# george-gca/sr-pytorch-lightning

Measured on AMD Instinct MI355X. Metric: SR training throughput, LR patches/s (48x48 LR x4, fwd+bwd+Adam), higher is better.
Workload: dtype bf16; 1 GPU; edsr_baseline x4, 48x48 LR patches, batch 256/GPU, train step (L1 + Adam); global_batch=256, parallelism=dp1, hip_graph=full

## Files before the change

### include/srk.h

```cpp
#ifndef SRK_H
#define SRK_H

#include <stdint.h>

#ifdef __cplusplus
extern "C" {
#endif

typedef void* srk_stream_t;

enum { SRK_BF16 = 0, SRK_F16 = 1, SRK_F32 = 2 };

enum {
  SRK_E_BADARG = -1,
  SRK_E_NODEV = -2
};

enum {
  SRK_OUT_NHWC = 0,
  SRK_OUT_NHWC_PS = 1,
  SRK_OUT_PLANAR = 2
};

typedef struct {
  const float* w;
  const float* bias;
  void* wpk;
  float* bias_pk;
  int Cout, Cin, KH, KW;
  int KinP;
  int CoutP;
  int dgrad;
  int ps_r;
  int dtype;
  int rows_layout;
} srk_pack_args;
int srk_pack_conv_weights(const srk_pack_args* a, srk_stream_t stream);
int srk_pack_conv_weights_group(const srk_pack_args* table, int n, srk_stream_t stream);
int srk_pack_group_tiles(const srk_pack_args* host_table, int n, int* tile_begin);
int srk_pack_conv_weights_group_tiled(const srk_pack_args* table, const int* tile_begin, int n, int total_tiles, srk_stream_t stream);

typedef struct {
  const void* x; int x_pitch, x_coff;
  int x_ps;
  int N, H, W;
  int Cin;
  const void* wpk; const float* bias;
  int CoutP;
  int Cout;
  int KH, KW;
  int relu; float scale;
  const void* res; int res_pitch, res_coff;
  const void* mask; int mask_pitch, mask_coff; int mask_from;
  void* out; int out_pitch, out_coff; int out_mode; int ps_r;
  const float* post_add;
  int dtype;
  int cout_real;
  void* relu_bits; const void* mask_bits;
} srk_conv_args;
int srk_conv_bits_ok(const srk_conv_args* a);
int srk_conv2d(const srk_conv_args* a, srk_stream_t stream);
int srk_conv_tile(int Cout);

int srk_conv_trunk_ok(const srk_conv_args* layers_host, int nlayers);
int srk_conv_trunk(const srk_conv_args* layers_host, const void* table_dev, int nlayers, srk_stream_t stream);

typedef struct {
  const void* x; int x_pitch, x_coff;
  int N, H, W;
  const void* w1; const float* b1;
  const void* w2; const float* b2;
  int relu_mid; float scale_mid;
  const void* mask; int mask_pitch, mask_coff;
  void* mid; int mid_pitch, mid_coff;
  float scale_out;
  const void* res; int res_pitch, res_coff; int res_from_x;
  void* out; int out_pitch, out_coff;
  int dtype;
  float* pool; const void* pool_aux; int pool_aux_pitch, pool_aux_coff;
  int ca_mode; int ca_cr;
  const float* ca_gsum; int ca_gsum_rows; const float* ca_sums; int ca_sums_rows;
  const float* ca_s; const float* ca_z; const float* ca_w1; const float* ca_w2;
  float* ca_slots;
  void* xo; int xo_pitch, xo_coff;
  const void* ca_x2; int ca_x2_pitch, ca_x2_coff;
  const float* ca_b1; const float* ca_b2; float* ca_s_out; float* ca_z_out;
} srk_conv_pair_args;
int srk_conv_pair(const srk_conv_pair_args* a, srk_stream_t stream);
int srk_conv_pair_tiles(int N, int H, int W);

typedef struct {
  const float* w1; const float* b1;
  const float* w2; const float* b2;
  int Cin, Chid, Cmid, CoutP;
  void* fwd; void* bwd;
  int dtype;
} srk_pw_pack_args;
int srk_pw_shape_ok(int Cin, int Chid, int CoutP);
long long srk_pw_pack_bytes(int Cin, int Chid, int CoutP, int bwd);
int srk_pw_pack(const srk_pw_pack_args* a, srk_stream_t stream);

typedef struct {
  const float* v; const float* g;
  float* w; float* inv;
  const float* dw;
  float* dv; float* dg;
  int rows, cols, row0, pad_;
} srk_wn_job;
int srk_weight_norm_group(const srk_wn_job* table_dev, int njobs, int total_rows, int backward, srk_stream_t stream);

int srk_pw_pack_group(const srk_pw_pack_args* table_dev, int n, srk_stream_t stream);

typedef struct {
  const void* x; int x_pitch, x_coff;
  long long P;
  int Cin, Chid, CoutP;
  int Cout;
  const void* wpk;
  void* out; int out_pitch, out_coff;
  int dtype;
} srk_pw_args;
int srk_pw_forward(const srk_pw_args* a, srk_stream_t stream);

typedef struct {
  const void* x; int x_pitch, x_coff;
  const void* gz; int gz_pitch, gz_coff; int Cz;
  long long P;
  int Cin, Chid, CoutP;
  const void* wpk;
  const void* res; int res_pitch, res_coff;
  void* gx; int gx_pitch, gx_coff;
  void* h_out; void* gh_out;
  int dtype;
} srk_pw_bwd_args;
int srk_pw_backward(const srk_pw_bwd_args* a, srk_stream_t stream);

typedef struct {
  const void* x; int x_pitch, x_coff;
  const void* gz; int gz_pitch, gz_coff; int Cz;
  long long P;
  int Cin, Chid, Cmid, CoutP;
  const void* wpk;
  float* dw1p; float* dw2p; float* db1p; float* db2p; int nranges;
  float* dw1; float* db1; float* dw2; float* db2;
  int dtype;
} srk_pw_wgrad_args;
int srk_pw_wgrad_ranges(long long P, int Chid);
int srk_pw_wgrad(const srk_pw_wgrad_args* a, srk_stream_t stream);

typedef struct {
  const void* x; int x_pitch, x_coff; int x_ps;
  const void* dy; int dy_pitch, dy_coff; int dy_ps;
  int N, H, W;
  int Cin, Cout;
  int KH, KW;
  float* dwp;
  float* dbp;
  int nslabs;
  int dtype;
  int cout_real;
} srk_wgrad_args;
int srk_conv2d_wgrad(const srk_wgrad_args* a, srk_stream_t stream);
int srk_wgrad_slabs(const srk_wgrad_args* a);
int srk_wgrad_slab_cout(const srk_wgrad_args* a);

typedef struct {
  const float* dwp; const float* dbp;
  int nslabs;
  float* dw; float* db;
  int Cout, Cin, KH, KW;
  int CinP, CoutP;
  int ps_r;
  float scale;
  int accumulate;
} srk_wgrad_fin_args;
int srk_wgrad_finalize(const srk_wgrad_fin_args* a, srk_stream_t stream);

int srk_wgrad_group_ok(const srk_wgrad_args* a);
int srk_wgrad_group_job_bytes(void);
int srk_wgrad_group_plan(srk_wgrad_args* jobs, int n, float* scratch, void* table_host, int* block_job_host,
                         int* nblocks, long long* scratch_floats);
int srk_conv2d_wgrad_group(const void* table_dev, const int* block_job_dev, int nblocks, int dtype, srk_stream_t stream);
int srk_wgrad_finalize_group(const srk_wgrad_fin_args* table_dev, int n, int blocks_per_job, srk_stream_t stream);
int srk_upload_small(void* dst_dev, const void* src_host, long long nbytes, srk_stream_t stream);
int srk_upload_prepare(void);
int srk_upload_eager(void* dst_dev, const void* src_host, long long nbytes);
int srk_upload_fence(void);

typedef struct {
  const float* x;
  const float* sub;
  void* dst; int dst_pitch, dst_coff;
  int N, Cin, H, W, KH, KW;
  int Kstore;
  int dtype;
} srk_unfold_args;
int srk_unfold_nchw(const srk_unfold_args* a, srk_stream_t stream);

typedef struct {
  const float* src; void* dst; int dst_pitch, dst_coff;
  int N, C, H, W;
  int Cstore; int ps_r; float scale; int dtype;
} srk_to_nhwc_args;
int srk_nchw_to_nhwc(const srk_to_nhwc_args* a, srk_stream_t stream);

typedef struct {
  const void* src; int src_pitch, src_coff; float* dst;
  int N, C, H, W; int dtype;
} srk_to_nchw_args;
int srk_nhwc_to_nchw(const srk_to_nchw_args* a, srk_stream_t stream);

int srk_ca_splits(int N, int HW);
typedef struct {
  const void* t; int t_pitch, t_coff;
  const void* u; int u_pitch, u_coff;
  float* sums;
  int N, HW, C; int dtype;
} srk_ca_pool_args;
int srk_ca_pool(const srk_ca_pool_args* a, srk_stream_t stream);

typedef struct {
  const void* t; int t_pitch, t_coff;
  const void* res; int res_pitch, res_coff;
  const float* sums;
  const float* w1; const float* b1; const float* w2; const float* b2;
  float* s_out; float* z_out;
  void* out; int out_pitch, out_coff;
  int N, HW, C, Cr; int dtype;
  int sums_rows;
} srk_ca_apply_args;
int srk_ca_apply(const srk_ca_apply_args* a, srk_stream_t stream);

typedef struct {
  const void* g; int g_pitch, g_coff;
  const float* gsum;
  const float* sums; const float* s; const float* z;
  const float* w1; const float* w2;
  float* dw1; float* db1; float* dw2; float* db2;
  void* gt; int gt_pitch, gt_coff;
  int N, HW, C, Cr; int dtype;
  int sums_rows, gsum_rows;
} srk_ca_bwd_args;
int srk_ca_bwd_apply(const srk_ca_bwd_args* a, srk_stream_t stream);
typedef struct { const float* src; float* dst; int n; int k; } srk_rowsum_job;
int srk_rowsum_group(const srk_rowsum_job* table_dev, int njobs, int max_k, srk_stream_t stream);

typedef struct {
  const uint8_t* lr; const uint8_t* hr;
  int lr_h, lr_w, hr_h, hr_w;
  int top, left;
  int rot;
  int hflip, vflip;
} srk_patch_desc;
typedef struct {
  const srk_patch_desc* table; int N; int C; int patch_lr; int scale;
  float* lr_out;
  float* hr_out;
} srk_patch_args;
int srk_sample_patches(const srk_patch_args* a, srk_stream_t stream);

typedef struct {
  const float* sr; const float* hr;
  int N, C, H, W;
  int luma;
  int shave;
  double* sse;
} srk_sse_args;
int srk_image_sse(const srk_sse_args* a, srk_stream_t stream);

typedef struct srk_l1_args {
  const float* sr;
  const float* hr;
  long long n;
  signed char* sign;
  double* partial;
  const float* gout;
  float scale;
  float* grad;
} srk_l1_args;
int srk_l1_blocks(long long n);
int srk_l1_loss_fwd(const srk_l1_args* a, srk_stream_t stream);
int srk_l1_loss_bwd(const srk_l1_args* a, srk_stream_t stream);
int srk_l1_loss_mean(const double* partial, int nb, long long n, float* out, srk_stream_t stream);

#define SRK_FLIP_TABLE_FLOATS 176
#define SRK_FLIP_ADJ_CHANNELS 7
typedef struct srk_flip_args {
  const float* sr;
  const float* hr;
  int N, H, W;
  const float* table;
  double* partial;
  float* err;
  float* adj;
  const float* gout;
  float scale;
  float* grad;
} srk_flip_args;
int srk_flip_blocks(int N, int H, int W);
int srk_flip_fwd(const srk_flip_args* a, srk_stream_t stream);
int srk_flip_bwd(const srk_flip_args* a, srk_stream_t stream);
int srk_flip_mean(const double* partial, int nb, long long n, float* out, srk_stream_t stream);

typedef struct srk_ssim_args {
  const float* x;
  const float* y;
  int N, C, H, W;
  int pool;
  float sigma, k1, k2;
  double* sums;
} srk_ssim_args;
int srk_image_ssim(const srk_ssim_args* a, srk_stream_t stream);

typedef struct srk_ms_ssim_args {
  const float* x;
  const float* y;
  float* workspace;
  double* partials;
  float* out;
  int N, C, H, W;
  float sigma, k1, k2;
  float w0, w1, w2, w3, w4;
} srk_ms_ssim_args;
long long srk_ms_ssim_workspace_bytes(int N, int C, int H, int W);
int srk_ms_ssim_tiles(int H, int W, int* first);
int srk_ms_ssim(const srk_ms_ssim_args* a, srk_stream_t stream);

typedef struct {
  const void* x; int x_pitch, x_coff;
  void* cols; int cols_pitch;
  int N, H, W, C;
  int K, stride, pad;
  int Ho, Wo;
  int dtype;
} srk_unfold_nhwc_args;
int srk_unfold_nhwc(const srk_unfold_nhwc_args* a, srk_stream_t stream);

typedef struct {
  const void* cols; int cols_pitch;
  const float* bias;
  void* out; int out_pitch, out_coff;
  int N, Hi, Wi, C;
  int K, stride, pad;
  int Ho, Wo;
  int dtype;
} srk_fold_nhwc_args;
int srk_fold_nhwc(const srk_fold_nhwc_args* a, srk_stream_t stream);

typedef struct {
  const void* x; int x_pitch;
  void* out; int out_pitch;
  const void* wpk;
  const float* bias;
  int N, H, W;
  int dtype;
  const float* slope; int slope_stride;
  void* pre; int pre_pitch;
} srk_proj_args;
long long srk_proj_pack_bytes(void);
int srk_proj_pack(const float* w4, void* wpk, int dtype, srk_stream_t stream);
typedef struct { const float* w4; void* wpk; } srk_proj_pack_job;
int srk_proj_pack_group(const srk_proj_pack_job* table_dev, int n, int dtype, srk_stream_t stream);
int srk_proj_down(const srk_proj_args* a, srk_stream_t stream);
int srk_proj_up(const srk_proj_args* a, srk_stream_t stream);
typedef struct {
  const void* xh; int xh_pitch;
  const void* g; int g_pitch;
  float* scratch;
  float* dw;
  int accumulate;
  int N, H, W;
  int dtype;
  float* db;
  int bias_side;
  int db_accumulate;
} srk_proj_wgrad_args;
long long srk_proj_wgrad_scratch_floats(int N, int H, int W);
int srk_proj_wgrad(const srk_proj_wgrad_args* a, srk_stream_t stream);

typedef struct {
  const void* x; int x_pitch, x_coff;
  const void* y; int y_pitch, y_coff;
  long long P; int C;
  int mode;
  float* partial;
  int dtype;
  const float* shift;
  float* shift_out;
  void* gate_out; int gate_pitch;
  const float* slope; int slope_stride;
  const float* gate_a; const float* gate_d;
  float* partial2;
} srk_chan_stats_args;
int srk_chan_stats_blocks(long long P);
int srk_chan_stats(const srk_chan_stats_args* a, srk_stream_t stream);
typedef struct {
  const float* partial; int nblocks; int C; int Creal;
  int mode; int total;
  float M, eps, momentum;
  const float* mean; const float* invstd; const float* gamma;
  const float* weight; const float* bias;
  float* running_mean; float* running_var;
  float* out;
  long long* nbt;
  float* dgamma_acc; float* dbeta_acc;
  const float* partial2; int total2;
  float* dslope_acc;
} srk_chan_finalize_args;
int srk_chan_finalize(const srk_chan_finalize_args* a, srk_stream_t stream);
int srk_chan_stats_finalize(const srk_chan_stats_args* a, const srk_chan_finalize_args* f, int* counter, srk_stream_t stream);

typedef struct {
  const void* x; int x_pitch, x_coff;
  const void* y; int y_pitch, y_coff;
  const void* z; int z_pitch, z_coff;
  const float* a; const float* b; const float* d;
  const float* slope; int slope_stride;
  int post_prelu;
  void* out; int out_pitch, out_coff;
  long long P; int C;
  int dtype;
  const float* gate_a; const float* gate_d;
} srk_chan_apply_args;
int srk_chan_apply(const srk_chan_apply_args* a, srk_stream_t stream);

typedef struct {
  const float* wt; const float* bt;
  const float* wu; const float* bu;
  int O, C, Ci;
  float* weff; float* beff;
  float* wedge; float* bedge; float* wcor; float* bcor;
  const void* x; int x_pitch;
  int N, H, W; int dtype;
  float* out;
  const float* g;
  void* dx; int dx_pitch;
  float* eedge; float* e0; float* ecor; float* k0;
  float* scratch;
  const float* r; const float* r0;
  float* dwt; float* dbt; float* dwu; float* dbu;
} srk_hrtail_args;
int srk_hrtail_collapse(const srk_hrtail_args* a, srk_stream_t stream);
int srk_hrtail_edge_fwd(const srk_hrtail_args* a, srk_stream_t stream);
int srk_hrtail_edge_bwd_x(const srk_hrtail_args* a, srk_stream_t stream);
long long srk_hrtail_scratch_floats(int N, int Ci);
int srk_hrtail_edge_bwd_w(const srk_hrtail_args* a, srk_stream_t stream);
int srk_hrtail_expand(const srk_hrtail_args* a, srk_stream_t stream);

typedef struct { float* p; const float* g; long long state_off; long long n; long long step_idx; } srk_adam_slot;
typedef struct { int slot; int count; long long start; } srk_adam_block;
typedef struct {
  const srk_adam_slot* slots; const srk_adam_block* blocks; int nslots, nblocks;
  float* m; float* v;
  float* steps; unsigned int* ticket;
  float lr, beta1, beta2, eps, weight_decay; int maximize;
  float one_minus_beta1, one_minus_beta2;
} srk_adam_args;
int srk_adam_step(const srk_adam_args* a, srk_stream_t stream);
int srk_adam_step_scaled(const srk_adam_args* a, float* scaler_state, srk_stream_t stream);
int srk_adam_check_scaled(const srk_adam_args* a, float* scaler_state, srk_stream_t stream);
int srk_adam_update_scaled(const srk_adam_args* a, const float* scaler_state, srk_stream_t stream);
int srk_loss_scale_update(float* scaler_state, srk_stream_t stream);

const char* srk_last_error(void);
int srk_version(void);
int srk_device_cus(void);

#ifdef __cplusplus
}
#endif
#endif
```

### sr-pytorch-lightning_amd/_lib.py

```python
import ctypes as C
import os

_HERE = os.path.dirname(os.path.abspath(__file__))
EXACT_RELU = os.environ.get("SRK_EXACT_RELU") == "1"
LIB_PATH = os.environ.get("SRK_LIB_PATH") or os.path.join(_HERE, "libsrk_gfx950_exact.so" if EXACT_RELU else "libsrk_gfx950.so")

SRK_BF16, SRK_F16, SRK_F32 = 0, 1, 2
OUT_NHWC, OUT_NHWC_PS, OUT_PLANAR = 0, 1, 2

_p, _i, _f = C.c_void_p, C.c_int, C.c_float


class PackArgs(C.Structure):
    _fields_ = [("w", _p), ("bias", _p), ("wpk", _p), ("bias_pk", _p),
                ("Cout", _i), ("Cin", _i), ("KH", _i), ("KW", _i),
                ("KinP", _i), ("CoutP", _i), ("dgrad", _i), ("ps_r", _i), ("dtype", _i), ("rows_layout", _i)]


class ConvArgs(C.Structure):
    _fields_ = [("x", _p), ("x_pitch", _i), ("x_coff", _i), ("x_ps", _i),
                ("N", _i), ("H", _i), ("W", _i), ("Cin", _i),
                ("wpk", _p), ("bias", _p), ("CoutP", _i), ("Cout", _i), ("KH", _i), ("KW", _i),
                ("relu", _i), ("scale", _f),
                ("res", _p), ("res_pitch", _i), ("res_coff", _i),
                ("mask", _p), ("mask_pitch", _i), ("mask_coff", _i), ("mask_from", _i),
                ("out", _p), ("out_pitch", _i), ("out_coff", _i), ("out_mode", _i), ("ps_r", _i),
                ("post_add", _p), ("dtype", _i), ("cout_real", _i), ("relu_bits", _p), ("mask_bits", _p)]


class ConvPairArgs(C.Structure):
    _fields_ = [("x", _p), ("x_pitch", _i), ("x_coff", _i), ("N", _i), ("H", _i), ("W", _i),
                ("w1", _p), ("b1", _p), ("w2", _p), ("b2", _p),
                ("relu_mid", _i), ("scale_mid", _f),
                ("mask", _p), ("mask_pitch", _i), ("mask_coff", _i),
                ("mid", _p), ("mid_pitch", _i), ("mid_coff", _i),
                ("scale_out", _f),
                ("res", _p), ("res_pitch", _i), ("res_coff", _i), ("res_from_x", _i),
                ("out", _p), ("out_pitch", _i), ("out_coff", _i), ("dtype", _i),
                ("pool", _p), ("pool_aux", _p), ("pool_aux_pitch", _i), ("pool_aux_coff", _i),
                ("ca_mode", _i), ("ca_cr", _i), ("ca_gsum", _p), ("ca_gsum_rows", _i), ("ca_sums", _p), ("ca_sums_rows", _i),
                ("ca_s", _p), ("ca_z", _p), ("ca_w1", _p), ("ca_w2", _p), ("ca_slots", _p),
                ("xo", _p), ("xo_pitch", _i), ("xo_coff", _i),
                ("ca_x2", _p), ("ca_x2_pitch", _i), ("ca_x2_coff", _i), ("ca_b1", _p), ("ca_b2", _p), ("ca_s_out", _p), ("ca_z_out", _p)]


class PwPackArgs(C.Structure):
    _fields_ = [("w1", _p), ("b1", _p), ("w2", _p), ("b2", _p), ("Cin", _i), ("Chid", _i), ("Cmid", _i), ("CoutP", _i),
                ("fwd", _p), ("bwd", _p), ("dtype", _i)]


class WnJob(C.Structure):
    _fields_ = [("v", _p), ("g", _p), ("w", _p), ("inv", _p), ("dw", _p), ("dv", _p), ("dg", _p),
                ("rows", _i), ("cols", _i), ("row0", _i), ("pad_", _i)]


class PwArgs(C.Structure):
    _fields_ = [("x", _p), ("x_pitch", _i), ("x_coff", _i), ("P", C.c_longlong), ("Cin", _i), ("Chid", _i), ("CoutP", _i), ("Cout", _i),
                ("wpk", _p), ("out", _p), ("out_pitch", _i), ("out_coff", _i), ("dtype", _i)]


class PwBwdArgs(C.Structure):
    _fields_ = [("x", _p), ("x_pitch", _i), ("x_coff", _i), ("gz", _p), ("gz_pitch", _i), ("gz_coff", _i), ("Cz", _i),
                ("P", C.c_longlong), ("Cin", _i), ("Chid", _i), ("CoutP", _i), ("wpk", _p),
                ("res", _p), ("res_pitch", _i), ("res_coff", _i), ("gx", _p), ("gx_pitch", _i), ("gx_coff", _i),
                ("h_out", _p), ("gh_out", _p), ("dtype", _i)]


class PwWgradArgs(C.Structure):
    _fields_ = [("x", _p), ("x_pitch", _i), ("x_coff", _i), ("gz", _p), ("gz_pitch", _i), ("gz_coff", _i), ("Cz", _i),
                ("P", C.c_longlong), ("Cin", _i), ("Chid", _i), ("Cmid", _i), ("CoutP", _i), ("wpk", _p),
                ("dw1p", _p), ("dw2p", _p), ("db1p", _p), ("db2p", _p), ("nranges", _i), ("dw1", _p), ("db1", _p), ("dw2", _p), ("db2", _p),
                ("dtype", _i)]


class ChanFinalizeArgs(C.Structure):
    _fields_ = [("partial", _p), ("nblocks", _i), ("C", _i), ("Creal", _i), ("mode", _i), ("total", _i),
                ("M", _f), ("eps", _f), ("momentum", _f), ("mean", _p), ("invstd", _p), ("gamma", _p),
                ("weight", _p), ("bias", _p), ("running_mean", _p), ("running_var", _p), ("out", _p),
                ("nbt", _p), ("dgamma_acc", _p), ("dbeta_acc", _p), ("partial2", _p), ("total2", _i), ("dslope_acc", _p)]


class RowsumJob(C.Structure):
    _fields_ = [("src", _p), ("dst", _p), ("n", _i), ("k", _i)]


class AdamSlot(C.Structure):
    _fields_ = [("p", _p), ("g", _p), ("state_off", C.c_longlong), ("n", C.c_longlong), ("step_idx", C.c_longlong)]


class AdamBlock(C.Structure):
    _fields_ = [("slot", _i), ("count", _i), ("start", C.c_longlong)]


class AdamArgs(C.Structure):
    _fields_ = [("slots", _p), ("blocks", _p), ("nslots", _i), ("nblocks", _i), ("m", _p), ("v", _p), ("steps", _p), ("ticket", _p),
                ("lr", _f), ("beta1", _f), ("beta2", _f), ("eps", _f), ("weight_decay", _f), ("maximize", _i),
                ("one_minus_beta1", _f), ("one_minus_beta2", _f)]


class WgradArgs(C.Structure):
    _fields_ = [("x", _p), ("x_pitch", _i), ("x_coff", _i), ("x_ps", _i),
                ("dy", _p), ("dy_pitch", _i), ("dy_coff", _i), ("dy_ps", _i),
                ("N", _i), ("H", _i), ("W", _i), ("Cin", _i), ("Cout", _i), ("KH", _i), ("KW", _i),
                ("dwp", _p), ("dbp", _p), ("nslabs", _i), ("dtype", _i), ("cout_real", _i)]


class WgradFinArgs(C.Structure):
    _fields_ = [("dwp", _p), ("dbp", _p), ("nslabs", _i), ("dw", _p), ("db", _p),
                ("Cout", _i), ("Cin", _i), ("KH", _i), ("KW", _i), ("CinP", _i), ("CoutP", _i),
                ("ps_r", _i), ("scale", _f), ("accumulate", _i)]


class ProjArgs(C.Structure):
    _fields_ = [("x", _p), ("x_pitch", _i), ("out", _p), ("out_pitch", _i), ("wpk", _p), ("bias", _p),
                ("N", _i), ("H", _i), ("W", _i), ("dtype", _i), ("slope", _p), ("slope_stride", _i), ("pre", _p), ("pre_pitch", _i)]


class ProjPackJob(C.Structure):
    _fields_ = [("w4", _p), ("wpk", _p)]


class ProjWgradArgs(C.Structure):
    _fields_ = [("xh", _p), ("xh_pitch", _i), ("g", _p), ("g_pitch", _i), ("scratch", _p), ("dw", _p), ("accumulate", _i),
                ("N", _i), ("H", _i), ("W", _i), ("dtype", _i), ("db", _p), ("bias_side", _i), ("db_accumulate", _i)]


class UnfoldArgs(C.Structure):
    _fields_ = [("x", _p), ("sub", _p), ("dst", _p), ("dst_pitch", _i), ("dst_coff", _i),
                ("N", _i), ("Cin", _i), ("H", _i), ("W", _i), ("KH", _i), ("KW", _i), ("Kstore", _i), ("dtype", _i)]


class ToNhwcArgs(C.Structure):
    _fields_ = [("src", _p), ("dst", _p), ("dst_pitch", _i), ("dst_coff", _i),
                ("N", _i), ("C", _i), ("H", _i), ("W", _i), ("Cstore", _i), ("ps_r", _i), ("scale", _f), ("dtype", _i)]


class ToNchwArgs(C.Structure):
    _fields_ = [("src", _p), ("src_pitch", _i), ("src_coff", _i), ("dst", _p),
                ("N", _i), ("C", _i), ("H", _i), ("W", _i), ("dtype", _i)]


class CaPoolArgs(C.Structure):
    _fields_ = [("t", _p), ("t_pitch", _i), ("t_coff", _i), ("u", _p), ("u_pitch", _i), ("u_coff", _i),
                ("sums", _p), ("N", _i), ("HW", _i), ("C", _i), ("dtype", _i)]


class CaApplyArgs(C.Structure):
    _fields_ = [("t", _p), ("t_pitch", _i), ("t_coff", _i), ("res", _p), ("res_pitch", _i), ("res_coff", _i),
                ("sums", _p), ("w1", _p), ("b1", _p), ("w2", _p), ("b2", _p), ("s_out", _p), ("z_out", _p),
                ("out", _p), ("out_pitch", _i), ("out_coff", _i),
                ("N", _i), ("HW", _i), ("C", _i), ("Cr", _i), ("dtype", _i), ("sums_rows", _i)]


class CaBwdArgs(C.Structure):
    _fields_ = [("g", _p), ("g_pitch", _i), ("g_coff", _i), ("gsum", _p), ("sums", _p), ("s", _p), ("z", _p),
                ("w1", _p), ("w2", _p), ("dw1", _p), ("db1", _p), ("dw2", _p), ("db2", _p),
                ("gt", _p), ("gt_pitch", _i), ("gt_coff", _i),
                ("N", _i), ("HW", _i), ("C", _i), ("Cr", _i), ("dtype", _i), ("sums_rows", _i), ("gsum_rows", _i)]


class PatchDesc(C.Structure):
    _fields_ = [("lr", _p), ("hr", _p), ("lr_h", _i), ("lr_w", _i), ("hr_h", _i), ("hr_w", _i),
                ("top", _i), ("left", _i), ("rot", _i), ("hflip", _i), ("vflip", _i)]


class PatchArgs(C.Structure):
    _fields_ = [("table", _p), ("N", _i), ("C", _i), ("patch_lr", _i), ("scale", _i), ("lr_out", _p), ("hr_out", _p)]


class SseArgs(C.Structure):
    _fields_ = [("sr", _p), ("hr", _p), ("N", _i), ("C", _i), ("H", _i), ("W", _i), ("luma", _i), ("shave", _i), ("sse", _p)]


class SsimArgs(C.Structure):
    _fields_ = [("x", _p), ("y", _p), ("N", _i), ("C", _i), ("H", _i), ("W", _i), ("pool", _i),
                ("sigma", _f), ("k1", _f), ("k2", _f), ("sums", _p)]


class MsSsimArgs(C.Structure):
    _fields_ = [("x", _p), ("y", _p), ("workspace", _p), ("partials", _p), ("out", _p), ("N", _i), ("C", _i), ("H", _i), ("W", _i),
                ("sigma", _f), ("k1", _f), ("k2", _f), ("w0", _f), ("w1", _f), ("w2", _f), ("w3", _f), ("w4", _f)]


class L1Args(C.Structure):
    _fields_ = [("sr", _p), ("hr", _p), ("n", C.c_longlong), ("sign", _p), ("partial", _p), ("gout", _p),
                ("scale", _f), ("grad", _p)]


class FlipArgs(C.Structure):
    _fields_ = [("sr", _p), ("hr", _p), ("N", _i), ("H", _i), ("W", _i), ("table", _p), ("partial", _p), ("err", _p), ("adj", _p),
                ("gout", _p), ("scale", _f), ("grad", _p)]


class UnfoldNhwcArgs(C.Structure):
    _fields_ = [("x", _p), ("x_pitch", _i), ("x_coff", _i), ("cols", _p), ("cols_pitch", _i),
                ("N", _i), ("H", _i), ("W", _i), ("C", _i), ("K", _i), ("stride", _i), ("pad", _i), ("Ho", _i), ("Wo", _i), ("dtype", _i)]


class FoldNhwcArgs(C.Structure):
    _fields_ = [("cols", _p), ("cols_pitch", _i), ("bias", _p), ("out", _p), ("out_pitch", _i), ("out_coff", _i),
                ("N", _i), ("Hi", _i), ("Wi", _i), ("C", _i), ("K", _i), ("stride", _i), ("pad", _i), ("Ho", _i), ("Wo", _i), ("dtype", _i)]


class ChanStatsArgs(C.Structure):
    _fields_ = [("x", _p), ("x_pitch", _i), ("x_coff", _i), ("y", _p), ("y_pitch", _i), ("y_coff", _i),
                ("P", C.c_longlong), ("C", _i), ("mode", _i), ("partial", _p), ("dtype", _i), ("shift", _p), ("shift_out", _p),
                ("gate_out", _p), ("gate_pitch", _i), ("slope", _p), ("slope_stride", _i),
                ("gate_a", _p), ("gate_d", _p), ("partial2", _p)]


class ChanApplyArgs(C.Structure):
    _fields_ = [("x", _p), ("x_pitch", _i), ("x_coff", _i), ("y", _p), ("y_pitch", _i), ("y_coff", _i),
                ("z", _p), ("z_pitch", _i), ("z_coff", _i), ("a", _p), ("b", _p), ("d", _p),
                ("slope", _p), ("slope_stride", _i), ("post_prelu", _i), ("out", _p), ("out_pitch", _i), ("out_coff", _i),
                ("P", C.c_longlong), ("C", _i), ("dtype", _i), ("gate_a", _p), ("gate_d", _p)]


class HrTailArgs(C.Structure):
    _fields_ = [("wt", _p), ("bt", _p), ("wu", _p), ("bu", _p), ("O", _i), ("C", _i), ("Ci", _i),
                ("weff", _p), ("beff", _p), ("wedge", _p), ("bedge", _p), ("wcor", _p), ("bcor", _p),
                ("x", _p), ("x_pitch", _i), ("N", _i), ("H", _i), ("W", _i), ("dtype", _i),
                ("out", _p), ("g", _p), ("dx", _p), ("dx_pitch", _i),
                ("eedge", _p), ("e0", _p), ("ecor", _p), ("k0", _p), ("scratch", _p),
                ("r", _p), ("r0", _p), ("dwt", _p), ("dbt", _p), ("dwu", _p), ("dbu", _p)]


LAUNCHERS = {
    "srk_pack_conv_weights": PackArgs,
    "srk_conv2d": ConvArgs,
    "srk_conv_pair": ConvPairArgs,
    "srk_pw_pack": PwPackArgs,
    "srk_pw_forward": PwArgs,
    "srk_pw_backward": PwBwdArgs,
    "srk_pw_wgrad": PwWgradArgs,
    "srk_adam_step": AdamArgs,
    "srk_chan_finalize": ChanFinalizeArgs,
    "srk_conv2d_wgrad": WgradArgs,
    "srk_wgrad_finalize": WgradFinArgs,
    "srk_unfold_nchw": UnfoldArgs,
    "srk_nchw_to_nhwc": ToNhwcArgs,
    "srk_nhwc_to_nchw": ToNchwArgs,
    "srk_ca_pool": CaPoolArgs,
    "srk_ca_apply": CaApplyArgs,
    "srk_ca_bwd_apply": CaBwdArgs,
    "srk_sample_patches": PatchArgs,
    "srk_image_sse": SseArgs,
    "srk_image_ssim": SsimArgs,
    "srk_ms_ssim": MsSsimArgs,
    "srk_l1_loss_fwd": L1Args,
    "srk_l1_loss_bwd": L1Args,
    "srk_flip_fwd": FlipArgs,
    "srk_flip_bwd": FlipArgs,
    "srk_unfold_nhwc": UnfoldNhwcArgs,
    "srk_fold_nhwc": FoldNhwcArgs,
    "srk_chan_stats": ChanStatsArgs,
    "srk_chan_apply": ChanApplyArgs,
    "srk_proj_down": ProjArgs,
    "srk_proj_up": ProjArgs,
    "srk_proj_wgrad": ProjWgradArgs,
    "srk_hrtail_collapse": HrTailArgs,
    "srk_hrtail_edge_fwd": HrTailArgs,
    "srk_hrtail_edge_bwd_x": HrTailArgs,
    "srk_hrtail_edge_bwd_w": HrTailArgs,
    "srk_hrtail_expand": HrTailArgs,
}
OTHER_SYMBOLS = ("srk_conv_tile", "srk_last_error", "srk_version", "srk_device_cus", "srk_wgrad_slabs",
                 "srk_pack_conv_weights_group", "srk_l1_blocks", "srk_wgrad_group_ok", "srk_wgrad_group_job_bytes",
                 "srk_wgrad_group_plan", "srk_conv2d_wgrad_group", "srk_wgrad_finalize_group", "srk_upload_small", "srk_upload_prepare", "srk_upload_eager", "srk_upload_fence", "srk_ca_splits", "srk_chan_stats_blocks",
                 "srk_conv_pair_tiles", "srk_rowsum_group", "srk_pw_shape_ok", "srk_pw_pack_bytes", "srk_pw_pack_group", "srk_weight_norm_group", "srk_pw_wgrad_ranges", "srk_l1_loss_mean", "srk_chan_stats_finalize", "srk_pack_group_tiles", "srk_pack_conv_weights_group_tiled",
                 "srk_proj_pack", "srk_proj_pack_bytes", "srk_proj_wgrad_scratch_floats", "srk_proj_pack_group", "srk_wgrad_slab_cout",
                 "srk_hrtail_scratch_floats", "srk_adam_step_scaled", "srk_adam_check_scaled", "srk_adam_update_scaled", "srk_loss_scale_update", "srk_conv_bits_ok",
                 "srk_conv_trunk", "srk_conv_trunk_ok", "srk_flip_blocks", "srk_flip_mean",
                 "srk_ms_ssim_workspace_bytes", "srk_ms_ssim_tiles")

_lib = None


def load():
    global _lib
    if _lib is not None:
        return _lib
    if not os.path.exists(LIB_PATH):
        raise RuntimeError(
            f"{LIB_PATH} is missing: build it with `python __graft_entry__.py` "
            "(hipcc --offload-arch=gfx950).  There is no CPU fallback for the HIP path.")
    lib = C.CDLL(LIB_PATH)
    older = bool(os.environ.get("SRK_LIB_PATH"))

    class _Absent:
        def __init__(self, name):
            self.name = name
            self.argtypes = self.restype = None

        def __call__(self, *a, **k):
            raise RuntimeError(f"{self.name} is not exported by {LIB_PATH} (an older build loaded through SRK_LIB_PATH)")

    if older:
        for name in list(LAUNCHERS) + list(OTHER_SYMBOLS):
            if not hasattr(lib, name):
                setattr(lib, name, _Absent(name))
    for name, st in LAUNCHERS.items():
        fn = getattr(lib, name)
        fn.argtypes = [C.POINTER(st), C.c_void_p]
        fn.restype = C.c_int
    lib.srk_conv_tile.argtypes = [C.c_int]
    lib.srk_conv_tile.restype = C.c_int
    lib.srk_conv_pair_tiles.argtypes = [C.c_int, C.c_int, C.c_int]
    lib.srk_conv_pair_tiles.restype = C.c_int
    lib.srk_wgrad_slabs.argtypes = [C.POINTER(WgradArgs)]
    lib.srk_wgrad_slabs.restype = C.c_int
    lib.srk_wgrad_slab_cout.argtypes = [C.POINTER(WgradArgs)]
    lib.srk_wgrad_slab_cout.restype = C.c_int
    lib.srk_pack_conv_weights_group.argtypes = [C.c_void_p, C.c_int, C.c_void_p]
    lib.srk_pack_conv_weights_group.restype = C.c_int
    lib.srk_pack_group_tiles.argtypes = [C.c_void_p, C.c_int, C.c_void_p]
    lib.srk_pack_group_tiles.restype = C.c_int
    lib.srk_pack_conv_weights_group_tiled.argtypes = [C.c_void_p, C.c_void_p, C.c_int, C.c_int, C.c_void_p]
    lib.srk_pack_conv_weights_group_tiled.restype = C.c_int
    lib.srk_wgrad_group_ok.argtypes = [C.POINTER(WgradArgs)]
    lib.srk_wgrad_group_ok.restype = C.c_int
    lib.srk_wgrad_group_job_bytes.restype = C.c_int
    lib.srk_wgrad_group_plan.argtypes = [C.POINTER(WgradArgs), C.c_int, C.c_void_p, C.c_void_p, C.c_void_p,
                                         C.POINTER(C.c_int), C.POINTER(C.c_longlong)]
    lib.srk_wgrad_group_plan.restype = C.c_int
    lib.srk_conv2d_wgrad_group.argtypes = [C.c_void_p, C.c_void_p, C.c_int, C.c_int, C.c_void_p]
    lib.srk_conv2d_wgrad_group.restype = C.c_int
    lib.srk_wgrad_finalize_group.argtypes = [C.c_void_p, C.c_int, C.c_int, C.c_void_p]
    lib.srk_wgrad_finalize_group.restype = C.c_int
    lib.srk_rowsum_group.argtypes = [C.c_void_p, C.c_int, C.c_int, C.c_void_p]
    lib.srk_rowsum_group.restype = C.c_int
    lib.srk_upload_small.argtypes = [C.c_void_p, C.c_void_p, C.c_longlong, C.c_void_p]
    lib.srk_upload_small.restype = C.c_int
    if not isinstance(getattr(lib, "srk_upload_eager", None), _Absent):
        lib.srk_upload_prepare.argtypes = []
        lib.srk_upload_prepare.restype = C.c_int
        lib.srk_upload_eager.argtypes = [C.c_void_p, C.c_void_p, C.c_longlong]
        lib.srk_upload_eager.restype = C.c_int
        lib.srk_upload_fence.argtypes = []
        lib.srk_upload_fence.restype = C.c_int
    lib.srk_chan_stats_finalize.argtypes = [C.POINTER(ChanStatsArgs), C.POINTER(ChanFinalizeArgs), C.c_void_p, C.c_void_p]
    lib.srk_chan_stats_finalize.restype = C.c_int
    lib.srk_chan_stats_blocks.argtypes = [C.c_longlong]
    lib.srk_chan_stats_blocks.restype = C.c_int
    lib.srk_ca_splits.argtypes = [C.c_int, C.c_int]
    lib.srk_ca_splits.restype = C.c_int
    lib.srk_l1_loss_mean.argtypes = [C.c_void_p, C.c_int, C.c_longlong, C.c_void_p, C.c_void_p]
    lib.srk_l1_loss_mean.restype = C.c_int
    lib.srk_l1_blocks.argtypes = [C.c_longlong]
    if not isinstance(getattr(lib, "srk_flip_mean", None), _Absent):
        lib.srk_flip_mean.argtypes = [C.c_void_p, C.c_int, C.c_longlong, C.c_void_p, C.c_void_p]
        lib.srk_flip_mean.restype = C.c_int
        lib.srk_flip_blocks.argtypes = [C.c_int, C.c_int, C.c_int]
        lib.srk_flip_blocks.restype = C.c_int
    lib.srk_l1_blocks.restype = C.c_int
    if not isinstance(getattr(lib, "srk_ms_ssim_tiles", None), _Absent):
        lib.srk_ms_ssim_workspace_bytes.argtypes = [C.c_int, C.c_int, C.c_int, C.c_int]
        lib.srk_ms_ssim_workspace_bytes.restype = C.c_longlong
        lib.srk_ms_ssim_tiles.argtypes = [C.c_int, C.c_int, C.c_void_p]
        lib.srk_ms_ssim_tiles.restype = C.c_int
    lib.srk_pw_shape_ok.argtypes = [C.c_int, C.c_int, C.c_int]
    lib.srk_pw_shape_ok.restype = C.c_int
    lib.srk_pw_pack_bytes.argtypes = [C.c_int, C.c_int, C.c_int, C.c_int]
    lib.srk_pw_pack_bytes.restype = C.c_longlong
    lib.srk_pw_wgrad_ranges.argtypes = [C.c_longlong, C.c_int]
    lib.srk_pw_wgrad_ranges.restype = C.c_int
    lib.srk_pw_pack_group.argtypes = [C.c_void_p, C.c_int, C.c_void_p]
    lib.srk_pw_pack_group.restype = C.c_int
    lib.srk_weight_norm_group.argtypes = [C.c_void_p, C.c_int, C.c_int, C.c_int, C.c_void_p]
    lib.srk_weight_norm_group.restype = C.c_int
    lib.srk_proj_pack.argtypes = [C.c_void_p, C.c_void_p, C.c_int, C.c_void_p]
    lib.srk_proj_pack.restype = C.c_int
    lib.srk_proj_pack_group.argtypes = [C.c_void_p, C.c_int, C.c_int, C.c_void_p]
    lib.srk_proj_pack_group.restype = C.c_int
    lib.srk_proj_pack_bytes.restype = C.c_longlong
    lib.srk_proj_wgrad_scratch_floats.argtypes = [C.c_int, C.c_int, C.c_int]
    lib.srk_proj_wgrad_scratch_floats.restype = C.c_longlong
    lib.srk_hrtail_scratch_floats.argtypes = [C.c_int, C.c_int]
    lib.srk_hrtail_scratch_floats.restype = C.c_longlong
    lib.srk_conv_bits_ok.argtypes = [C.POINTER(ConvArgs)]
    lib.srk_conv_bits_ok.restype = C.c_int
    lib.srk_conv_trunk_ok.argtypes = [C.POINTER(ConvArgs), C.c_int]
    lib.srk_conv_trunk_ok.restype = C.c_int
    lib.srk_conv_trunk.argtypes = [C.POINTER(ConvArgs), C.c_void_p, C.c_int, C.c_void_p]
    lib.srk_conv_trunk.restype = C.c_int
    lib.srk_adam_step_scaled.argtypes = [C.POINTER(AdamArgs), C.c_void_p, C.c_void_p]
    lib.srk_adam_step_scaled.restype = C.c_int
    for fn in (lib.srk_adam_check_scaled, lib.srk_adam_update_scaled):
        fn.argtypes = [C.POINTER(AdamArgs), C.c_void_p, C.c_void_p]
        fn.restype = C.c_int
    lib.srk_loss_scale_update.argtypes = [C.c_void_p, C.c_void_p]
    lib.srk_loss_scale_update.restype = C.c_int
    lib.srk_last_error.restype = C.c_char_p
    lib.srk_version.restype = C.c_int
    lib.srk_device_cus.restype = C.c_int
    _lib = lib
    return lib


def call(name, args, stream):
    lib = load()
    if getattr(args, "N", 1) == 0:
        return
    rc = getattr(lib, name)(C.byref(args), C.c_void_p(stream))
    if rc != 0:
        raise RuntimeError(f"{name} failed (rc={rc}): {lib.srk_last_error().decode(errors='replace')}")


def check(rc, what):
    if rc != 0:
        raise RuntimeError(f"{what} failed (rc={rc}): {load().srk_last_error().decode(errors='replace')}")


def conv_tile(cout):
    return load().srk_conv_tile(int(cout))
```

### sr-pytorch-lightning_amd/csrc/hr_tail.hip

```cpp
#include "srk_common.h"

namespace {

SRK_DEV void sub_of(int a, int d, int& i, int& s) {
  const int ap = a + d;
  i = ap & 1;
  s = (ap - i) >> 1;
}

struct Wts {
  const float* wt; const float* bt; const float* wu; const float* bu;
  int O, C, Ci;
};

SRK_DEV float sum16(float v) {
  v += __shfl_xor(v, 8, 64);
  v += __shfl_xor(v, 4, 64);
  v += __shfl_xor(v, 2, 64);
  v += __shfl_xor(v, 1, 64);
  return v;
}

SRK_DEV float collapse_w(const Wts& p, int sub, int o, int a, int b, int ci, int dy0, int dy1, int dx0, int dx1, int fy, int fx) {
  float acc = 0.f;
  for (int dy = dy0; dy <= dy1; ++dy) {
    int i, sy; sub_of(a, dy, i, sy);
    const int ey = fy - sy;
    if (ey < -1 || ey > 1) continue;
    for (int dx = dx0; dx <= dx1; ++dx) {
      int j, sx; sub_of(b, dx, j, sx);
      const int ex = fx - sx;
      if (ex < -1 || ex > 1) continue;
      const float* wt = p.wt + (size_t)o * p.C * 9 + (dy + 1) * 3 + (dx + 1);
      const float* wu = p.wu + ((size_t)(i * 2 + j) * p.Ci + ci) * 9 + (ey + 1) * 3 + (ex + 1);
      for (int c0 = sub; c0 < p.C; c0 += 64) {
        float x[4], y[4];
#pragma unroll
        for (int k = 0; k < 4; ++k) {
          const int c = c0 + 16 * k;
          const bool ok = c < p.C;
          x[k] = ok ? wt[(size_t)c * 9] : 0.f;
          y[k] = ok ? wu[(size_t)c * 4 * p.Ci * 9] : 0.f;
        }
#pragma unroll
        for (int k = 0; k < 4; ++k)
          if (c0 + 16 * k < p.C) acc += x[k] * y[k];
      }
    }
  }
  return sum16(acc);
}
SRK_DEV float collapse_b(const Wts& p, int sub, int o, int a, int b, int dy0, int dy1, int dx0, int dx1) {
  float acc = 0.f;
  if (p.bu) {
    for (int dy = dy0; dy <= dy1; ++dy) {
      int i, sy; sub_of(a, dy, i, sy);
      for (int dx = dx0; dx <= dx1; ++dx) {
        int j, sx; sub_of(b, dx, j, sx);
        const float* wt = p.wt + (size_t)o * p.C * 9 + (dy + 1) * 3 + (dx + 1);
        for (int c = sub; c < p.C; c += 16) acc += wt[(size_t)c * 9] * p.bu[c * 4 + i * 2 + j];
      }
    }
  }
  return sum16(acc);
}

__global__ __launch_bounds__(256) void hrtail_collapse_kernel(const srk_hrtail_args a) {
  const Wts p{a.wt, a.bt, a.wu, a.bu, a.O, a.C, a.Ci};
  const int O = a.O, Ci = a.Ci;
  const int n_eff = 4 * O * Ci * 25, n_edge = 4 * 2 * O * Ci * 5, n_cor = 4 * O * Ci;
  const int n_b = 4 * O + 4 * 2 * O + 4 * O;
  const int sub = threadIdx.x & 15;
  int t = blockIdx.x * 16 + (threadIdx.x >> 4);
  if (t >= n_eff + n_edge + n_cor + n_b) t = n_eff + n_edge + n_cor + n_b;
  float v = 0.f;
  float* dst = nullptr;
  if (t < n_eff) {
    const int f = t % 25, ci = (t / 25) % Ci, k = t / (25 * Ci);
    v = collapse_w(p, sub, k >> 2, (k >> 1) & 1, k & 1, ci, -1, 1, -1, 1, f / 5 - 2, f % 5 - 2);
    dst = a.weff + t;
  } else if (t < n_eff + n_edge) {
    const int u = t - n_eff;
    const int tt = u % 5, ci = (u / 5) % Ci, kk = (u / (5 * Ci)) % (2 * O), ty = u / (5 * Ci * 2 * O);
    const int o = kk >> 1, q = kk & 1;
    if (ty == 0) v = collapse_w(p, sub, o, 0, q, ci, -1, -1, -1, 1, 0, tt - 2);
    else if (ty == 1) v = collapse_w(p, sub, o, 1, q, ci, 1, 1, -1, 1, 0, tt - 2);
    else if (ty == 2) v = collapse_w(p, sub, o, q, 0, ci, -1, 1, -1, -1, tt - 2, 0);
    else v = collapse_w(p, sub, o, q, 1, ci, -1, 1, 1, 1, tt - 2, 0);
    dst = a.wedge + u;
  } else if (t < n_eff + n_edge + n_cor) {
    const int u = t - n_eff - n_edge;
    const int ci = u % Ci, o = (u / Ci) % O, c = u / (Ci * O);
    const int ca = c >> 1, cb = c & 1;
    v = collapse_w(p, sub, o, ca, cb, ci, ca ? 1 : -1, ca ? 1 : -1, cb ? 1 : -1, cb ? 1 : -1, 0, 0);
    dst = a.wcor + u;
  } else if (t < n_eff + n_edge + n_cor + n_b) {
    const int w = t - n_eff - n_edge - n_cor;
    if (w < 4 * O) {
      const int k = w;
      v = (a.bt ? a.bt[k >> 2] : 0.f) + collapse_b(p, sub, k >> 2, (k >> 1) & 1, k & 1, -1, 1, -1, 1);
      dst = a.beff + k;
    } else if (w < 4 * O + 8 * O) {
      const int u = w - 4 * O, kk = u % (2 * O), ty = u / (2 * O), o = kk >> 1, q = kk & 1;
      if (ty == 0) v = collapse_b(p, sub, o, 0, q, -1, -1, -1, 1);
      else if (ty == 1) v = collapse_b(p, sub, o, 1, q, 1, 1, -1, 1);
      else if (ty == 2) v = collapse_b(p, sub, o, q, 0, -1, 1, -1, -1);
      else v = collapse_b(p, sub, o, q, 1, -1, 1, 1, 1);
      dst = a.bedge + u;
    } else {
      const int u = w - 12 * O, o = u % O, c = u / O, ca = c >> 1, cb = c & 1;
      v = collapse_b(p, sub, o, ca, cb, ca ? 1 : -1, ca ? 1 : -1, cb ? 1 : -1, cb ? 1 : -1);
      dst = a.bcor + u;
    }
  }
  if (dst && sub == 0) *dst = v;
}

template <int DT> SRK_DEV float ld_act(const void* base, size_t idx) {
  return DTraits<DT>::to_f32(reinterpret_cast<const typename DTraits<DT>::elem*>(base)[idx]);
}

constexpr int MAXO = 4;
SRK_DEV float wave_total(float v) {
#pragma unroll
  for (int m = 32; m >= 1; m >>= 1) v += __shfl_xor(v, m, 64);
  return v;
}
struct EdgeGeo {
  int ty, len; bool row;
  int fix_lr, fix_hr;
};
SRK_DEV EdgeGeo edge_geo(int ty, int H, int W) {
  EdgeGeo e;
  e.ty = ty; e.row = ty < 2; e.len = e.row ? W : H;
  e.fix_lr = ty == 0 ? 0 : ty == 1 ? H - 1 : ty == 2 ? 0 : W - 1;
  e.fix_hr = ty == 0 ? 0 : ty == 1 ? 2 * H - 1 : ty == 2 ? 0 : 2 * W - 1;
  return e;
}
SRK_DEV void stage_copy256(float* __restrict__ dst, const float* __restrict__ src, int n) {
  int i = threadIdx.x;
  for (; i + 256 * 7 < n; i += 256 * 8) {
    float v[8];
#pragma unroll
    for (int k = 0; k < 8; ++k) v[k] = src[i + 256 * k];
#pragma unroll
    for (int k = 0; k < 8; ++k) dst[i + 256 * k] = v[k];
  }
  float v[8];
#pragma unroll
  for (int k = 0; k < 8; ++k) v[k] = i + 256 * k < n ? src[i + 256 * k] : 0.f;
#pragma unroll
  for (int k = 0; k < 8; ++k)
    if (i + 256 * k < n) dst[i + 256 * k] = v[k];
}
template <int DT>
SRK_DEV void stage_line(const srk_hrtail_args& a, const EdgeGeo& e, int n, float* Xl, int pitch) {
  typedef DTraits<DT> Tr;
  const int Ci = a.Ci;
  if ((Ci & 7) == 0 && (a.x_pitch & 7) == 0) {
    const int nch = Ci >> 3, total = (e.len + 4) * nch;
    for (int i0 = threadIdx.x; i0 < total; i0 += 256 * 4) {
      i32x4 raw[4];
#pragma unroll
      for (int u = 0; u < 4; ++u) {
        const int i = i0 + 256 * u;
        const int sp = i / nch, c8 = i - sp * nch, s = sp - 2;
        raw[u] = i32x4{0, 0, 0, 0};
        if (i < total && s >= 0 && s < e.len) {
          const int yy = e.row ? e.fix_lr : s, xx = e.row ? s : e.fix_lr;
          raw[u] = gload16(reinterpret_cast<const typename Tr::elem*>(a.x) + ((size_t)(n * a.H + yy) * a.W + xx) * a.x_pitch + c8 * 8);
        }
      }
#pragma unroll
      for (int u = 0; u < 4; ++u) {
        const int i = i0 + 256 * u;
        if (i >= total) continue;
        const int sp = i / nch, c8 = i - sp * nch;
        const int w4[4] = {raw[u].x, raw[u].y, raw[u].z, raw[u].w};
        float v[8];
#pragma unroll
        for (int k = 0; k < 4; ++k) unpack2<DT>((uint32_t)w4[k], v[2 * k], v[2 * k + 1]);
#pragma unroll
        for (int k = 0; k < 8; ++k) Xl[sp * pitch + c8 * 8 + k] = v[k];
      }
    }
    return;
  }
  for (int i = threadIdx.x; i < (e.len + 4) * Ci; i += 256) {
    const int s = i / Ci - 2, ci = i % Ci;
    float v = 0.f;
    if (s >= 0 && s < e.len) {
      const int yy = e.row ? e.fix_lr : s, xx = e.row ? s : e.fix_lr;
      v = ld_act<DT>(a.x, ((size_t)(n * a.H + yy) * a.W + xx) * a.x_pitch + ci);
    }
    Xl[(s + 2) * pitch + ci] = v;
  }
}

template <int DT>
__global__ __launch_bounds__(256) void hrtail_edge_fwd_kernel(const srk_hrtail_args a, int phase) {
  const int H = a.H, W = a.W, O = a.O, Ci = a.Ci, H2 = 2 * H, W2 = 2 * W;
  const int n = blockIdx.x;
  const EdgeGeo e = edge_geo(2 * phase + blockIdx.y, H, W);
  extern __shared__ __attribute__((aligned(16))) char smem_raw[];
  const int pitch = Ci + 1;
  float* const Xl = reinterpret_cast<float*>(smem_raw);
  float* const Wl = Xl + (size_t)(e.len + 4) * pitch;
  stage_line<DT>(a, e, n, Xl, pitch);
  stage_copy256(Wl, a.wedge + (size_t)e.ty * 2 * O * Ci * 5, 2 * O * Ci * 5);
  __syncthreads();
  const size_t oplane = (size_t)H2 * W2;
  float* const out = a.out + (size_t)n * O * oplane;
  for (int idx = threadIdx.x + 256 * blockIdx.z; idx < 2 * e.len * O; idx += 256 * gridDim.z) {
    const int p = idx % (2 * e.len), o = idx / (2 * e.len);
    const int s = p >> 1, q = p & 1;
    const float* const w = Wl + (size_t)(o * 2 + q) * Ci * 5;
    const float* const x = Xl + (size_t)s * pitch;
    float a0 = a.bedge[e.ty * 2 * O + o * 2 + q], a1 = 0.f, a2 = 0.f, a3 = 0.f, a4 = 0.f;
    for (int ci = 0; ci < Ci; ++ci) {
      a0 += w[ci * 5 + 0] * x[0 * pitch + ci]; a1 += w[ci * 5 + 1] * x[1 * pitch + ci]; a2 += w[ci * 5 + 2] * x[2 * pitch + ci];
      a3 += w[ci * 5 + 3] * x[3 * pitch + ci]; a4 += w[ci * 5 + 4] * x[4 * pitch + ci];
    }
    float acc = ((a0 + a1) + (a2 + a3)) + a4;
    if (!e.row && (p == 0 || p == 2 * e.len - 1)) {
      const int ca = p == 0 ? 0 : 1, cb = e.ty == 2 ? 0 : 1, c = ca * 2 + cb;
      float cc = a.bcor[c * O + o];
      const float* const xc = Xl + (size_t)(s + 2) * pitch;
      for (int ci = 0; ci < Ci; ++ci) cc += a.wcor[((size_t)c * O + o) * Ci + ci] * xc[ci];
      acc -= cc;
    }
    const size_t at = e.row ? (size_t)e.fix_hr * W2 + p : (size_t)p * W2 + e.fix_hr;
    out[(size_t)o * oplane + at] -= acc;
  }
}

template <int DT>
__global__ __launch_bounds__(256) void hrtail_edge_bwd_x_kernel(const srk_hrtail_args a, int phase) {
  typedef DTraits<DT> Tr;
  const int H = a.H, W = a.W, O = a.O, Ci = a.Ci, H2 = 2 * H, W2 = 2 * W;
  const int n = blockIdx.x;
  const bool shared_line = phase == 0 ? H == 1 : W == 1;
  if (shared_line && blockIdx.y == 1) return;
  extern __shared__ __attribute__((aligned(16))) char smem_raw[];
  const size_t gplane = (size_t)H2 * W2;
  const float* const g = a.g + (size_t)n * O * gplane;
  for (int rep = 0; rep < (shared_line ? 2 : 1); ++rep) {
  const EdgeGeo e = edge_geo(2 * phase + (shared_line ? rep : (int)blockIdx.y), H, W);
  float* const Gl = reinterpret_cast<float*>(smem_raw);
  float* const Wl = Gl + (size_t)2 * O * (e.len + 4);
  __syncthreads();
  for (int i0 = threadIdx.x; i0 < 2 * O * (e.len + 4); i0 += 256 * 4) {
    float v[4];
#pragma unroll
    for (int u = 0; u < 4; ++u) {
      const int i = i0 + 256 * u;
      const int kk = i / (e.len + 4), s = i % (e.len + 4) - 2, o = kk >> 1, q = kk & 1;
      v[u] = 0.f;
      if (i < 2 * O * (e.len + 4) && s >= 0 && s < e.len)
        v[u] = e.row ? g[(size_t)o * gplane + (size_t)e.fix_hr * W2 + 2 * s + q] : g[(size_t)o * gplane + (size_t)(2 * s + q) * W2 + e.fix_hr];
    }
#pragma unroll
    for (int u = 0; u < 4; ++u)
      if (i0 + 256 * u < 2 * O * (e.len + 4)) Gl[i0 + 256 * u] = v[u];
  }
  stage_copy256(Wl, a.wedge + (size_t)e.ty * 2 * O * Ci * 5, 2 * O * Ci * 5);
  __syncthreads();
  const int nch = (Ci + 7) >> 3;
  const bool vec = (Ci & 7) == 0 && (a.dx_pitch & 7) == 0;
  for (int idx = threadIdx.x + 256 * blockIdx.z; idx < e.len * nch; idx += 256 * gridDim.z) {
    const int c8 = idx % nch, s = idx / nch;
    float corr[8];
#pragma unroll
    for (int k = 0; k < 8; ++k) corr[k] = 0.f;
    for (int kk = 0; kk < 2 * O; ++kk) {
      const float* const gl = Gl + (size_t)kk * (e.len + 4) + s + 2;
      float gv[5];
#pragma unroll
      for (int tt = 0; tt < 5; ++tt) gv[tt] = gl[2 - tt];
#pragma unroll
      for (int k = 0; k < 8; ++k) {
        const int ci = c8 * 8 + k;
        if (ci < Ci) {
          const float* const w = Wl + ((size_t)kk * Ci + ci) * 5;
#pragma unroll
          for (int tt = 0; tt < 5; ++tt) corr[k] += w[tt] * gv[tt];
        }
      }
    }
    if (!e.row && (s == 0 || s == e.len - 1)) {
      for (int ca = 0; ca < 2; ++ca) {
        if (!(ca ? s == e.len - 1 : s == 0)) continue;
        const int cb = e.ty == 2 ? 0 : 1, c = ca * 2 + cb;
        const size_t at = (size_t)(ca ? H2 - 1 : 0) * W2 + e.fix_hr;
        for (int o = 0; o < O; ++o) {
          const float gc = g[(size_t)o * gplane + at];
#pragma unroll
          for (int k = 0; k < 8; ++k)
            if (c8 * 8 + k < Ci) corr[k] -= a.wcor[((size_t)c * O + o) * Ci + c8 * 8 + k] * gc;
        }
      }
    }
    const int yy = e.row ? e.fix_lr : s, xx = e.row ? s : e.fix_lr;
    typename Tr::elem* const d = reinterpret_cast<typename Tr::elem*>(a.dx) + ((size_t)(n * H + yy) * W + xx) * a.dx_pitch + c8 * 8;
    if (vec) {
      const i32x4 raw = *reinterpret_cast<const i32x4*>(d);
      const int w4[4] = {raw.x, raw.y, raw.z, raw.w};
      int o4[4];
#pragma unroll
      for (int k = 0; k < 4; ++k) {
        float f0, f1;
        unpack2<DT>((uint32_t)w4[k], f0, f1);
        o4[k] = (int)pack2<DT>(f0 - corr[2 * k], f1 - corr[2 * k + 1]);
      }
      *reinterpret_cast<i32x4*>(d) = i32x4{o4[0], o4[1], o4[2], o4[3]};
    } else {
#pragma unroll
      for (int k = 0; k < 8; ++k)
        if (c8 * 8 + k < Ci) d[k] = Tr::from_f32(Tr::to_f32(d[k]) - corr[k]);
    }
  }
  }
}

constexpr int EW_MAXLEN = 512;
template <int DT>
__global__ __launch_bounds__(256) void hrtail_edge_bwd_w_kernel(const srk_hrtail_args a, int nchunks, int ew_chunk) {
  const int H = a.H, W = a.W, O = a.O, Ci = a.Ci, H2 = 2 * H, W2 = 2 * W;
  const int ty = blockIdx.y, chunk = blockIdx.x;
  const int n0 = chunk * ew_chunk, n1 = min(a.N, n0 + ew_chunk);
  const int ncombo = ty < 4 ? 2 * O * 5 : O;
  const size_t gplane = (size_t)H2 * W2;
  float* const dst = a.scratch + ((size_t)ty * nchunks + chunk) * (size_t)(2 * MAXO * 5) * (Ci + 1);
  extern __shared__ __attribute__((aligned(16))) char smem_raw[];
  float* const Xl = reinterpret_cast<float*>(smem_raw);
  if (ty >= 4) {
    if (blockIdx.z != 0) return;
    const int c = ty - 4, ca = c >> 1, cbb = c & 1;
    const int Py = ca ? H2 - 1 : 0, Px = cbb ? W2 - 1 : 0, yy = ca ? H - 1 : 0, xx = cbb ? W - 1 : 0;
    for (int item = threadIdx.x; item < ncombo * (Ci + 1); item += 256) {
      const int ci = item % (Ci + 1), o = item / (Ci + 1);
      float acc = 0.f;
      for (int n = n0; n < n1; ++n) {
        const float gv = a.g[((size_t)n * O + o) * gplane + (size_t)Py * W2 + Px];
        const float xv = ci < Ci ? ld_act<DT>(a.x, ((size_t)(n * H + yy) * W + xx) * a.x_pitch + ci) : 1.f;
        acc += gv * xv;
      }
      dst[item] = acc;
    }
    return;
  }
  const bool rowedge = ty < 2;
  const int len = rowedge ? W : H;
  float* const Gl = Xl + (size_t)(len + 4) * Ci;
  constexpr int MAXIT = (2 * MAXO * 5 * 65 + 255) / 256;
  const int nitems = ncombo * (Ci + 1);
  const int ipb = (nitems + gridDim.z - 1) / gridDim.z, item0 = blockIdx.z * ipb, item1 = min(nitems, item0 + ipb);
  float acc[MAXIT];
#pragma unroll
  for (int k = 0; k < MAXIT; ++k) acc[k] = 0.f;
  for (int n = n0; n < n1; ++n) {
    __syncthreads();
    stage_line<DT>(a, edge_geo(ty, H, W), n, Xl, Ci);
    for (int i = threadIdx.x; i < 2 * O * len; i += 256) {
      const int kk = i / len, s = i % len, o = kk >> 1, q = kk & 1;
      const float* const g = a.g + ((size_t)n * O + o) * gplane;
      Gl[i] = rowedge ? g[(size_t)(ty == 0 ? 0 : H2 - 1) * W2 + 2 * s + q] : g[(size_t)(2 * s + q) * W2 + (ty == 2 ? 0 : W2 - 1)];
    }
    __syncthreads();
#pragma unroll
    for (int k = 0; k < MAXIT; ++k) {
      const int item = item0 + threadIdx.x + k * 256;
      if (item >= item1) break;
      const int ci = item % (Ci + 1), cb = item / (Ci + 1), tt = cb % 5, kk = cb / 5;
      const float* const gr = Gl + kk * len;
      float t0 = 0.f, t1 = 0.f, t2 = 0.f, t3 = 0.f;
      int p = 0;
      if (ci < Ci) {
        const float* const xr = Xl + (size_t)tt * Ci + ci;
        for (; p + 3 < len; p += 4) {
          t0 += gr[p] * xr[(size_t)p * Ci]; t1 += gr[p + 1] * xr[(size_t)(p + 1) * Ci];
          t2 += gr[p + 2] * xr[(size_t)(p + 2) * Ci]; t3 += gr[p + 3] * xr[(size_t)(p + 3) * Ci];
        }
        for (; p < len; ++p) t0 += gr[p] * xr[(size_t)p * Ci];
      } else if (tt == 2) {
        for (; p + 3 < len; p += 4) { t0 += gr[p]; t1 += gr[p + 1]; t2 += gr[p + 2]; t3 += gr[p + 3]; }
        for (; p < len; ++p) t0 += gr[p];
      }
      acc[k] += (t0 + t1) + (t2 + t3);
    }
  }
#pragma unroll
  for (int k = 0; k < MAXIT; ++k) {
    const int item = item0 + threadIdx.x + k * 256;
    if (item < item1) dst[item] = acc[k];
  }
}

__global__ __launch_bounds__(256) void hrtail_edge_reduce_kernel(const srk_hrtail_args a, int nchunks) {
  const int O = a.O, Ci = a.Ci;
  const int per = 2 * MAXO * 5 * (Ci + 1);
  const int t = blockIdx.x * 256 + threadIdx.x;
  const int n_edge = 4 * 2 * O * 5 * (Ci + 1), n_cor = 4 * O * (Ci + 1);
  if (t >= n_edge + n_cor) return;
  int ty, item;
  if (t < n_edge) { ty = t / (2 * O * 5 * (Ci + 1)); item = t % (2 * O * 5 * (Ci + 1)); }
  else { const int u = t - n_edge; ty = 4 + u / (O * (Ci + 1)); item = u % (O * (Ci + 1)); }
  const float* const src = a.scratch + (size_t)ty * nchunks * per + item;
  float s0 = 0.f, s1 = 0.f, s2 = 0.f, s3 = 0.f;
  int c = 0;
  for (; c + 3 < nchunks; c += 4) {
    s0 += src[(size_t)c * per]; s1 += src[(size_t)(c + 1) * per]; s2 += src[(size_t)(c + 2) * per]; s3 += src[(size_t)(c + 3) * per];
  }
  for (; c < nchunks; ++c) s0 += src[(size_t)c * per];
  const float s = (s0 + s1) + (s2 + s3);
  const int ci = item % (Ci + 1), cb = item / (Ci + 1);
  if (ty < 4) {
    const int tt = cb % 5, kk = cb / 5;
    if (ci < Ci) a.eedge[(((size_t)ty * 2 * O + kk) * Ci + ci) * 5 + tt] = s;
    else if (tt == 2) a.e0[ty * 2 * O + kk] = s;
  } else {
    if (ci < Ci) a.ecor[((size_t)(ty - 4) * O + cb) * Ci + ci] = s;
    else a.k0[(ty - 4) * O + cb] = s;
  }
}

struct Gr {
  const float* r; const float* r0; const float* ee; const float* e0; const float* ec; const float* k0;
  int O, Ci;
};
SRK_DEV int row_type(int a, int dy) { return (a == 0 && dy == -1) ? 0 : ((a == 1 && dy == 1) ? 1 : -1); }
SRK_DEV int col_type(int b, int dx) { return (b == 0 && dx == -1) ? 2 : ((b == 1 && dx == 1) ? 3 : -1); }
SRK_DEV float g_w(const Gr& q, int o, int a, int b, int dy, int dx, int ci, int fy, int fx) {
  float v = q.r[(((size_t)(o * 4 + a * 2 + b)) * q.Ci + ci) * 25 + (fy + 2) * 5 + (fx + 2)];
  const int rt = row_type(a, dy), ct = col_type(b, dx);
  if (rt >= 0 && fy == 0) v -= q.ee[(((size_t)rt * 2 * q.O + o * 2 + b) * q.Ci + ci) * 5 + fx + 2];
  if (ct >= 0 && fx == 0) v -= q.ee[(((size_t)ct * 2 * q.O + o * 2 + a) * q.Ci + ci) * 5 + fy + 2];
  if (rt >= 0 && ct >= 0 && fy == 0 && fx == 0) v += q.ec[((size_t)(a * 2 + b) * q.O + o) * q.Ci + ci];
  return v;
}
SRK_DEV float g_b(const Gr& q, int o, int a, int b, int dy, int dx) {
  float v = q.r0[o * 4 + a * 2 + b];
  const int rt = row_type(a, dy), ct = col_type(b, dx);
  if (rt >= 0) v -= q.e0[rt * 2 * q.O + o * 2 + b];
  if (ct >= 0) v -= q.e0[ct * 2 * q.O + o * 2 + a];
  if (rt >= 0 && ct >= 0) v += q.k0[(a * 2 + b) * q.O + o];
  return v;
}

__global__ __launch_bounds__(256) void hrtail_expand_kernel(const srk_hrtail_args a) {
  const Gr q{a.r, a.r0, a.eedge, a.e0, a.ecor, a.k0, a.O, a.Ci};
  const int O = a.O, C = a.C, Ci = a.Ci;
  const int n_wu = 4 * C * Ci * 9, n_bu = 4 * C, n_bt = O;
  const int nb_thread = (n_wu + n_bu + n_bt + 255) / 256;
  if ((int)blockIdx.x >= nb_thread) {
    const int t = ((int)blockIdx.x - nb_thread) * 4 + (threadIdx.x >> 6), lane = threadIdx.x & 63;
    if (t >= O * C * 9) return;
    const int d = t % 9, c = (t / 9) % C, o = t / (9 * C);
    const int dy = d / 3 - 1, dx = d % 3 - 1;
    float acc = 0.f;
    for (int pa = 0; pa < 2; ++pa) {
      int i, sy; sub_of(pa, dy, i, sy);
      for (int pb = 0; pb < 2; ++pb) {
        int j, sx; sub_of(pb, dx, j, sx);
        const int cu = c * 4 + i * 2 + j;
        if (a.bu && lane == 0) acc += g_b(q, o, pa, pb, dy, dx) * a.bu[cu];
        for (int ci = lane; ci < Ci; ci += 64)
#pragma unroll
          for (int e = 0; e < 9; ++e)
            acc += g_w(q, o, pa, pb, dy, dx, ci, sy + e / 3 - 1, sx + e % 3 - 1) * a.wu[((size_t)cu * Ci + ci) * 9 + e];
      }
    }
    acc = wave_total(acc);
    if (lane == 0) a.dwt[t] = acc;
    return;
  }
  int t = blockIdx.x * 256 + threadIdx.x;
  if (t < n_wu) {
    const int e = t % 9, ci = (t / 9) % Ci, cu = t / (9 * Ci), c = cu >> 2, i = (cu >> 1) & 1, j = cu & 1;
    const int ey = e / 3 - 1, ex = e % 3 - 1;
    float acc = 0.f;
    for (int pa = 0; pa < 2; ++pa)
      for (int dy = -1; dy <= 1; ++dy) {
        int ii, sy; sub_of(pa, dy, ii, sy);
        if (ii != i) continue;
        for (int pb = 0; pb < 2; ++pb)
          for (int dx = -1; dx <= 1; ++dx) {
            int jj, sx; sub_of(pb, dx, jj, sx);
            if (jj != j) continue;
            for (int o = 0; o < O; ++o)
              acc += a.wt[((size_t)o * C + c) * 9 + (dy + 1) * 3 + dx + 1] * g_w(q, o, pa, pb, dy, dx, ci, sy + ey, sx + ex);
          }
      }
    a.dwu[t] = acc;
    return;
  }
  t -= n_wu;
  if (t < n_bu) {
    if (!a.dbu) return;
    const int cu = t, c = cu >> 2, i = (cu >> 1) & 1, j = cu & 1;
    float acc = 0.f;
    for (int pa = 0; pa < 2; ++pa)
      for (int dy = -1; dy <= 1; ++dy) {
        int ii, sy; sub_of(pa, dy, ii, sy);
        if (ii != i) continue;
        for (int pb = 0; pb < 2; ++pb)
          for (int dx = -1; dx <= 1; ++dx) {
            int jj, sx; sub_of(pb, dx, jj, sx);
            if (jj != j) continue;
            for (int o = 0; o < O; ++o) acc += a.wt[((size_t)o * C + c) * 9 + (dy + 1) * 3 + dx + 1] * g_b(q, o, pa, pb, dy, dx);
          }
      }
    a.dbu[cu] = acc;
    return;
  }
  t -= n_bu;
  if (t < n_bt && a.dbt) a.dbt[t] = a.r0[t * 4] + a.r0[t * 4 + 1] + a.r0[t * 4 + 2] + a.r0[t * 4 + 3];
}

int check_common(const srk_hrtail_args* a, const char* who) {
  SRK_CHECK_ARG(a, "%s: null argument", who);
  SRK_CHECK_ARG(a->O >= 1 && a->O <= MAXO && a->C >= 1 && a->Ci >= 1, "%s: O=%d (1..%d) C=%d Ci=%d", who, a->O, MAXO, a->C, a->Ci);
  return 0;
}
int check_act(const srk_hrtail_args* a, const char* who) {
  SRK_CHECK_ARG(a->N > 0 && a->H > 0 && a->W > 0, "%s: bad dims N=%d H=%d W=%d", who, a->N, a->H, a->W);
  SRK_CHECK_ARG(a->dtype == SRK_BF16 || a->dtype == SRK_F16, "%s: 16-bit activations only", who);
  SRK_CHECK_ARG((long long)a->N * a->O * 4 * a->H * a->W < (1ll << 31), "%s: output too large", who);
  return 0;
}

}

extern "C" int srk_hrtail_collapse(const srk_hrtail_args* a, srk_stream_t stream) {
  if (int rc = check_common(a, "srk_hrtail_collapse")) return rc;
  SRK_CHECK_ARG(a->wt && a->wu && a->weff && a->beff && a->wedge && a->bedge && a->wcor && a->bcor, "srk_hrtail_collapse: null pointer");
  const int total = 4 * a->O * a->Ci * 25 + 4 * 2 * a->O * a->Ci * 5 + 4 * a->O * a->Ci + 16 * a->O;
  hipLaunchKernelGGL(hrtail_collapse_kernel, dim3((unsigned)((total + 15) / 16)), dim3(256), 0, reinterpret_cast<hipStream_t>(stream), *a);
  SRK_LAUNCH_CHECK();
  return 0;
}

static unsigned edge_split(int N) {
  const int z = (512 + 2 * N - 1) / (2 * N);
  return (unsigned)(z < 1 ? 1 : (z > 8 ? 8 : z));
}

template <typename K> static int edge_lds_attr(K kernel, const char* who) {
  const hipError_t e = hipFuncSetAttribute(reinterpret_cast<const void*>(kernel), hipFuncAttributeMaxDynamicSharedMemorySize, 160 * 1024);
  if (e != hipSuccess) { srk_set_error("%s: cannot reserve LDS: %s", who, hipGetErrorString(e)); return (int)e; }
  return 0;
}

extern "C" int srk_hrtail_edge_fwd(const srk_hrtail_args* a, srk_stream_t stream) {
  if (int rc = check_common(a, "srk_hrtail_edge_fwd")) return rc;
  if (int rc = check_act(a, "srk_hrtail_edge_fwd")) return rc;
  SRK_CHECK_ARG(a->x && a->out && a->wedge && a->bedge && a->wcor && a->bcor, "srk_hrtail_edge_fwd: null pointer");
  const int len = a->H > a->W ? a->H : a->W;
  const size_t lds = ((size_t)(len + 4) * (a->Ci + 1) + (size_t)2 * a->O * a->Ci * 5) * 4;
  SRK_CHECK_ARG(lds <= 160 * 1024, "srk_hrtail_edge_fwd: edge of %d pixels x %d channels does not fit the LDS", len, a->Ci);
  static const int rc0 = edge_lds_attr(&hrtail_edge_fwd_kernel<SRK_BF16>, "srk_hrtail_edge_fwd");
  static const int rc1 = edge_lds_attr(&hrtail_edge_fwd_kernel<SRK_F16>, "srk_hrtail_edge_fwd");
  if (rc0 || rc1) return rc0 ? rc0 : rc1;
  hipStream_t st = reinterpret_cast<hipStream_t>(stream);
  for (int phase = 0; phase < 2; ++phase) {
    if (a->dtype == SRK_BF16) hipLaunchKernelGGL(hrtail_edge_fwd_kernel<SRK_BF16>, dim3((unsigned)a->N, 2, edge_split(a->N)), dim3(256), lds, st, *a, phase);
    else hipLaunchKernelGGL(hrtail_edge_fwd_kernel<SRK_F16>, dim3((unsigned)a->N, 2, edge_split(a->N)), dim3(256), lds, st, *a, phase);
    SRK_LAUNCH_CHECK();
  }
  return 0;
}

extern "C" int srk_hrtail_edge_bwd_x(const srk_hrtail_args* a, srk_stream_t stream) {
  if (int rc = check_common(a, "srk_hrtail_edge_bwd_x")) return rc;
  if (int rc = check_act(a, "srk_hrtail_edge_bwd_x")) return rc;
  SRK_CHECK_ARG(a->g && a->dx && a->wedge && a->wcor, "srk_hrtail_edge_bwd_x: null pointer");
  const int len = a->H > a->W ? a->H : a->W;
  const size_t lds = ((size_t)2 * a->O * (len + 4) + (size_t)2 * a->O * a->Ci * 5) * 4;
  SRK_CHECK_ARG(lds <= 160 * 1024, "srk_hrtail_edge_bwd_x: edge of %d pixels does not fit the LDS", len);
  static const int rc0 = edge_lds_attr(&hrtail_edge_bwd_x_kernel<SRK_BF16>, "srk_hrtail_edge_bwd_x");
  static const int rc1 = edge_lds_attr(&hrtail_edge_bwd_x_kernel<SRK_F16>, "srk_hrtail_edge_bwd_x");
  if (rc0 || rc1) return rc0 ? rc0 : rc1;
  hipStream_t st = reinterpret_cast<hipStream_t>(stream);
  for (int phase = 0; phase < 2; ++phase) {
    if (a->dtype == SRK_BF16) hipLaunchKernelGGL(hrtail_edge_bwd_x_kernel<SRK_BF16>, dim3((unsigned)a->N, 2, edge_split(a->N)), dim3(256), lds, st, *a, phase);
    else hipLaunchKernelGGL(hrtail_edge_bwd_x_kernel<SRK_F16>, dim3((unsigned)a->N, 2, edge_split(a->N)), dim3(256), lds, st, *a, phase);
    SRK_LAUNCH_CHECK();
  }
  return 0;
}

static int ew_chunk_of(int N) { return N <= 64 ? 1 : (N + 63) / 64; }

extern "C" long long srk_hrtail_scratch_floats(int N, int Ci) {
  const int ewc = ew_chunk_of(N);
  const long long nchunks = (N + ewc - 1) / ewc;
  return 8 * nchunks * (long long)(2 * MAXO * 5) * (Ci + 1);
}

extern "C" int srk_hrtail_edge_bwd_w(const srk_hrtail_args* a, srk_stream_t stream) {
  if (int rc = check_common(a, "srk_hrtail_edge_bwd_w")) return rc;
  if (int rc = check_act(a, "srk_hrtail_edge_bwd_w")) return rc;
  SRK_CHECK_ARG(a->x && a->g && a->scratch && a->eedge && a->e0 && a->ecor && a->k0, "srk_hrtail_edge_bwd_w: null pointer");
  const int ewc = ew_chunk_of(a->N);
  const int nchunks = (a->N + ewc - 1) / ewc;
  const unsigned nz = nchunks * 8 >= 512 ? 2 : (nchunks * 8 >= 256 ? 4 : 8);
  const int len = a->H > a->W ? a->H : a->W;
  SRK_CHECK_ARG(a->Ci <= 64 && len <= EW_MAXLEN, "srk_hrtail_edge_bwd_w: Ci=%d (<= 64) edge length %d (<= %d)", a->Ci, len, EW_MAXLEN);
  const size_t lds = ((size_t)(len + 4) * a->Ci + (size_t)2 * a->O * len) * 4;
  hipStream_t st = reinterpret_cast<hipStream_t>(stream);
  static const hipError_t attr0 = hipFuncSetAttribute(reinterpret_cast<const void*>(&hrtail_edge_bwd_w_kernel<SRK_BF16>), hipFuncAttributeMaxDynamicSharedMemorySize, 160 * 1024);
  static const hipError_t attr1 = hipFuncSetAttribute(reinterpret_cast<const void*>(&hrtail_edge_bwd_w_kernel<SRK_F16>), hipFuncAttributeMaxDynamicSharedMemorySize, 160 * 1024);
  if (attr0 != hipSuccess || attr1 != hipSuccess) { srk_set_error("srk_hrtail_edge_bwd_w: cannot reserve LDS"); return (int)(attr0 != hipSuccess ? attr0 : attr1); }
  if (a->dtype == SRK_BF16) hipLaunchKernelGGL(hrtail_edge_bwd_w_kernel<SRK_BF16>, dim3((unsigned)nchunks, 8, nz), dim3(256), lds, st, *a, nchunks, ewc);
  else hipLaunchKernelGGL(hrtail_edge_bwd_w_kernel<SRK_F16>, dim3((unsigned)nchunks, 8, nz), dim3(256), lds, st, *a, nchunks, ewc);
  SRK_LAUNCH_CHECK();
  const int total = (4 * 2 * a->O * 5 + 4 * a->O) * (a->Ci + 1);
  hipLaunchKernelGGL(hrtail_edge_reduce_kernel, dim3((unsigned)((total + 255) / 256)), dim3(256), 0, st, *a, nchunks);
  SRK_LAUNCH_CHECK();
  return 0;
}

extern "C" int srk_hrtail_expand(const srk_hrtail_args* a, srk_stream_t stream) {
  if (int rc = check_common(a, "srk_hrtail_expand")) return rc;
  SRK_CHECK_ARG(a->wt && a->wu && a->r && a->r0 && a->eedge && a->e0 && a->ecor && a->k0 && a->dwt && a->dwu, "srk_hrtail_expand: null pointer");
  const int per_thread = 4 * a->C * a->Ci * 9 + 4 * a->C + a->O, per_wave = a->O * a->C * 9;
  const int nblocks = (per_thread + 255) / 256 + (per_wave + 3) / 4;
  hipLaunchKernelGGL(hrtail_expand_kernel, dim3((unsigned)nblocks), dim3(256), 0, reinterpret_cast<hipStream_t>(stream), *a);
  SRK_LAUNCH_CHECK();
  return 0;
}
```

### sr-pytorch-lightning_amd/ops.py

```python
import weakref

import torch

from . import _lib as L
from .packing import *
from .packing import _DT, _TLS, _f32c, _group_for, _knob, _need_gpu, _ptr, _roundup, _stream, _tok


def _pitch(t):
    n, h, w, c = t.shape
    p = t.stride(2) if w > 1 else (t.stride(1) if h > 1 else (t.stride(0) if n > 1 else c))
    if w > 1 and h > 1:
        assert t.stride(1) == w * p, "NHWC view must be dense in W"
    if h > 1 and n > 1:
        assert t.stride(0) == h * w * p, "NHWC view must be dense in H"
    assert c == 1 or t.stride(3) == 1, "channels must be innermost"
    return p


_ADDR_LIMIT = 0x7fff0000


def _batch_chunks(n, *tensors):
    worst = 0
    for t in tensors:
        if t is not None and t.dim() > 0 and t.shape[0] > 0:
            worst = max(worst, t.shape[0] * t.stride(0) * t.element_size())
    if worst < _ADDR_LIMIT or n <= 1:
        return 1
    return min(n, -(-worst // (_ADDR_LIMIT // 2)))


_SIGN_BITS = _knob("SRK_NO_SIGN_BITS") != "1"


def _conv_args(x, pk, out, *, res=None, mask=None, post_add=None, relu_bits=None, mask_bits=None, use_bias=True, **fields):
    n, h, w, c = x.shape
    planar = fields.get("out_mode") == L.OUT_PLANAR
    a = dict(x=x.data_ptr(), x_pitch=_pitch(x), N=n, H=h, W=w, Cin=c, scale=1.0,
             res=_ptr(res), res_pitch=0 if (res is None or planar) else _pitch(res),
             mask=_ptr(mask), mask_pitch=0 if mask is None else _pitch(mask),
             out=out.data_ptr(), out_pitch=0 if planar else _pitch(out), post_add=_ptr(post_add), dtype=_DT[x.dtype],
             relu_bits=_ptr(relu_bits), mask_bits=_ptr(mask_bits))
    if pk is not None:
        a.update(wpk=pk.wpk.data_ptr(), bias=_ptr(pk.bias) if use_bias else 0, CoutP=pk.CoutP, KH=pk.k, KW=pk.k,
                 cout_real=getattr(pk, "cr", 0) or 0)
    a.update(fields)
    args = L.ConvArgs(**a)
    args.pk = pk
    return args


def conv_raw(x, pk, *, N, H, W, Cin, Cout, out, out_mode=L.OUT_NHWC, ps_r=0, relu=False, scale=1.0,
             res=None, mask=None, mask_from=0, post_add=None, x_ps=0, use_bias=True, relu_bits=None, mask_bits=None):
    _need_gpu(x)
    if relu_bits is not None or mask_bits is not None:
        ok = _SIGN_BITS and _batch_chunks(N, x, out, res, mask) == 1 and mask_from == 0 and out_mode == L.OUT_NHWC and int(ps_r) <= 1 and post_add is None
        bits_t = None
        if ok:
            bits_t = mask_bits if mask_bits is not None else torch.empty((N * H * W, 2), dtype=torch.int32, device=x.device)
            a = _conv_args(x, pk, out, N=N, H=H, W=W, Cin=Cin, Cout=Cout, x_ps=int(x_ps), relu=int(relu), scale=float(scale), res=res,
                           out_mode=out_mode, ps_r=int(ps_r), relu_bits=bits_t if relu_bits is not None else None,
                           mask_bits=bits_t if mask_bits is not None else None, bias=0, cout_real=0)
            ok = bool(L.load().srk_conv_bits_ok(a))
        if not ok:
            conv_raw(x, pk, N=N, H=H, W=W, Cin=Cin, Cout=Cout, out=out, out_mode=out_mode, ps_r=ps_r, relu=relu, scale=scale, res=res, mask=mask,
                     mask_from=mask_from, post_add=post_add, x_ps=x_ps, use_bias=use_bias)
            out.__dict__["_srk_bits"] = None
            return out
        a.bias = _ptr(pk.bias) if use_bias else 0
        a.cout_real = getattr(pk, "cr", 0) or 0
        L.call("srk_conv2d", a, _stream())
        out.__dict__["_srk_bits"] = bits_t if relu_bits is not None else None
        return out
    nck = _batch_chunks(N, x, out, res, mask)
    if nck > 1:
        step = -(-N // nck)
        for n0 in range(0, N, step):
            n1 = min(N, n0 + step)
            conv_raw(x[n0:n1], pk, N=n1 - n0, H=H, W=W, Cin=Cin, Cout=Cout, out=out[n0:n1], out_mode=out_mode, ps_r=ps_r,
                     relu=relu, scale=scale, res=None if res is None else res[n0:n1], mask=None if mask is None else mask[n0:n1],
                     mask_from=mask_from, post_add=post_add, x_ps=x_ps, use_bias=use_bias)
        return out
    a = _conv_args(x, pk, out, N=N, H=H, W=W, Cin=Cin, Cout=Cout, x_ps=int(x_ps), relu=int(relu), scale=float(scale), res=res, mask=mask,
                   mask_from=int(mask_from), out_mode=out_mode, ps_r=int(ps_r), post_add=post_add, use_bias=use_bias)
    L.call("srk_conv2d", a, _stream())
    return out


_PAIR_OFF = _knob("SRK_NO_PAIR", "0") == "1"
_CA_UNFUSED = _knob("SRK_CA_UNFUSED", "0") == "1"
_PAIR_MAX_TILES = int(_knob("SRK_PAIR_MAX_TILES", "0"))


def pair_ok(x, w1, w2):
    if _PAIR_OFF or x.dtype not in (torch.bfloat16, torch.float16) or x.shape[3] != 64:
        return False
    if tuple(w1.shape) != (64, 64, 3, 3) or tuple(w2.shape) != (64, 64, 3, 3):
        return False
    n, h, wd, _ = x.shape
    if n == 0 or x.numel() * 2 >= _ADDR_LIMIT:
        return False
    lim = _PAIR_MAX_TILES or 2 * L.load().srk_device_cus()
    return L.load().srk_conv_pair_tiles(n, h, wd) <= lim


def conv_pair_raw(x, pk1, pk2, *, out, relu_mid=False, scale_mid=1.0, mask=None, mid=None, scale_out=1.0, res=None,
                  use_bias=True, pool=None, pool_aux=None, ca_bwd=None, ca_fwd=None, xo=None):
    _need_gpu(x)
    n, h, wd, _ = x.shape
    from_x = res is not None and res.data_ptr() == x.data_ptr() and _pitch(res) == _pitch(x) and ca_bwd is None and ca_fwd is None
    ca = ca_bwd or ca_fwd or {}
    x2 = ca.get("x2")
    a = L.ConvPairArgs(
        x=x.data_ptr(), x_pitch=_pitch(x), x_coff=0, N=n, H=h, W=wd,
        w1=pk1.wpk.data_ptr(), b1=_ptr(pk1.bias) if use_bias else 0, w2=pk2.wpk.data_ptr(), b2=_ptr(pk2.bias) if use_bias else 0,
        relu_mid=int(relu_mid), scale_mid=float(scale_mid),
        mask=_ptr(mask), mask_pitch=0 if mask is None else _pitch(mask), mask_coff=0,
        mid=_ptr(mid), mid_pitch=0 if mid is None else _pitch(mid), mid_coff=0,
        scale_out=float(scale_out),
        res=_ptr(res), res_pitch=0 if res is None else _pitch(res), res_coff=0, res_from_x=int(from_x),
        out=out.data_ptr(), out_pitch=_pitch(out), out_coff=0, dtype=_DT[x.dtype],
        pool=_ptr(pool), pool_aux=_ptr(pool_aux), pool_aux_pitch=0 if pool_aux is None else _pitch(pool_aux), pool_aux_coff=0,
        ca_mode=1 if ca_bwd is not None else (2 if ca_fwd is not None else 0), ca_cr=ca["w1"].shape[0] if ca else 0,
        ca_gsum=_ptr(ca.get("gsum")), ca_gsum_rows=ca["gsum"].shape[1] if ca_bwd else 0,
        ca_sums=_ptr(ca.get("sums")), ca_sums_rows=ca["sums"].shape[1] if ca else 0,
        ca_s=_ptr(ca.get("s")), ca_z=_ptr(ca.get("z")), ca_w1=_ptr(ca.get("w1")), ca_w2=_ptr(ca.get("w2")), ca_slots=_ptr(ca.get("slots")),
        xo=_ptr(xo), xo_pitch=0 if xo is None else _pitch(xo), xo_coff=0,
        ca_x2=_ptr(x2), ca_x2_pitch=0 if x2 is None else _pitch(x2), ca_x2_coff=0,
        ca_b1=_ptr(ca.get("b1")), ca_b2=_ptr(ca.get("b2")), ca_s_out=_ptr(ca.get("s_out")), ca_z_out=_ptr(ca.get("z_out")))
    L.call("srk_conv_pair", a, _stream())
    PAIR_LAUNCHES[a.ca_mode] += 1
    return out


_ONES = {}


def backward(loss):
    key = (loss.device, loss.dtype)
    one = _ONES.get(key)
    if one is None:
        if loss.is_cuda and torch.cuda.is_current_stream_capturing():
            loss.backward()
            return
        one = _ONES[key] = torch.ones((), dtype=loss.dtype, device=loss.device)
    loss.backward(gradient=one if loss.dim() == 0 else one.expand_as(loss))


def unfold_raw(x, sub, k, dtype):
    _need_gpu(x)
    n, c, h, w = x.shape
    xs = x.detach()
    if xs.dtype != torch.float32 or not xs.is_contiguous():
        xs = xs.float().contiguous()
    ks = pad16(c * k * k)
    dst = torch.empty((n, h, w, ks), dtype=dtype, device=x.device)
    a = L.UnfoldArgs(x=xs.data_ptr(), sub=_ptr(sub), dst=dst.data_ptr(), dst_pitch=ks, dst_coff=0,
                     N=n, Cin=c, H=h, W=w, KH=k, KW=k, Kstore=ks, dtype=_DT[dtype])
    L.call("srk_unfold_nchw", a, _stream())
    return dst


def to_nhwc(src, dtype, *, ps_r=0, scale=1.0):
    _need_gpu(src)
    r = ps_r if ps_r > 1 else 1
    n, cs, hs, ws = src.shape
    c, h, w = cs * r * r, hs // r, ws // r
    s = src.detach()
    if s.dtype != torch.float32 or not s.is_contiguous():
        s = s.float().contiguous()
    dst = torch.empty((n, h, w, pad16(c)), dtype=dtype, device=src.device)
    a = L.ToNhwcArgs(src=s.data_ptr(), dst=dst.data_ptr(), dst_pitch=dst.shape[3], dst_coff=0,
                     N=n, C=c, H=h, W=w, Cstore=dst.shape[3], ps_r=int(ps_r), scale=float(scale), dtype=_DT[dtype])
    L.call("srk_nchw_to_nhwc", a, _stream())
    return dst


def to_nchw(src, C=None):
    _need_gpu(src)
    n, h, w, cp = src.shape
    C = cp if C is None else C
    dst = torch.empty((n, C, h, w), dtype=torch.float32, device=src.device)
    a = L.ToNchwArgs(src=src.data_ptr(), src_pitch=_pitch(src), src_coff=0, dst=dst.data_ptr(),
                     N=n, C=C, H=h, W=w, dtype=_DT[src.dtype])
    L.call("srk_nhwc_to_nchw", a, _stream())
    return dst


class ToNhwcFn(torch.autograd.Function):

    @staticmethod
    def forward(ctx, x, dtype):
        ctx.c = x.shape[1]
        return to_nhwc(x, dtype)

    @staticmethod
    def backward(ctx, g):
        return to_nchw(g.contiguous(), ctx.c), None


class ToNchwFn(torch.autograd.Function):

    @staticmethod
    def forward(ctx, x, C):
        ctx.dt = x.dtype
        return to_nchw(x, C)

    @staticmethod
    def backward(ctx, g):
        return to_nhwc(g, ctx.dt), None


def nchw_to_nhwc(x, dtype):
    return ToNhwcFn.apply(x, dtype)


def nhwc_to_nchw(x, C):
    return ToNchwFn.apply(x, int(C))


_RES_LINK = _knob("SRK_NO_RES_LINK", "0") != "1"


class ResLink:
    __slots__ = ("armed", "g")

    def __init__(self):
        self.armed, self.g = False, None


class ConvFn(torch.autograd.Function):

    @staticmethod
    def forward(ctx, x, w, b, res, scale, ps_r, link=None):
        _need_gpu(x)
        n, h, wd, cinp = x.shape
        cout, cin, k, _ = w.shape
        assert cinp == pad16(cin), f"input has {cinp} channels, conv expects pad16({cin})"
        ctx.link = link
        if link is not None:
            link.armed = bool(ctx.needs_input_grad[0]) and int(ps_r) <= 1
        pk = pack_conv(w, b, x.dtype, ps_r=ps_r)
        if ps_r > 1:
            c = cout // (ps_r * ps_r)
            assert c % 16 == 0, "fused PixelShuffle store needs C % 16 == 0"
            out = torch.empty((n, h * ps_r, wd * ps_r, c), dtype=x.dtype, device=x.device)
            conv_raw(x, pk, N=n, H=h, W=wd, Cin=cinp, Cout=cout, out=out, out_mode=L.OUT_NHWC_PS, ps_r=ps_r,
                     scale=scale, res=res)
        else:
            out = torch.empty((n, h, wd, pad16(cout)), dtype=x.dtype, device=x.device)
            conv_raw(x, pk, N=n, H=h, W=wd, Cin=cinp, Cout=out.shape[3], out=out, scale=scale, res=res)
        ctx.save_for_backward(x, w)
        ctx.cfg = (scale, ps_r, b is not None, res is not None)
        ctx.wb = (w, b)
        ctx.pg = _tok()
        ctx.gacc = x.__dict__.get("_srk_gacc")
        return out

    @staticmethod
    def backward(ctx, g):
        x, w = ctx.saved_tensors
        scale, ps_r, has_b, has_res = ctx.cfg
        g = g.contiguous()
        n, h, wd, cinp = x.shape
        cout, cin, k, _ = w.shape
        coutp = pad16(cout)
        gx = gw = gb = None
        if ctx.needs_input_grad[0]:
            pkd = pack_conv(w, None, x.dtype, dgrad=True, ps_r=ps_r, token=ctx.pg)
            if ctx.gacc is not None and ps_r <= 1:
                gx, add = ctx.gacc[0].grad_dest(ctx.gacc[1])
                conv_raw(g, pkd, N=n, H=h, W=wd, Cin=coutp, Cout=cinp, out=gx, scale=scale, use_bias=False, res=gx if add else None)
            else:
                gx = torch.empty_like(x)
                parked = None
                if ctx.link is not None and ctx.link.g is not None:
                    parked, ctx.link.g = ctx.link.g, None
                conv_raw(g, pkd, N=n, H=h, W=wd, Cin=coutp, Cout=cinp, out=gx, scale=scale, x_ps=ps_r, use_bias=False, res=parked)
        if ctx.needs_input_grad[1] or ctx.needs_input_grad[2]:
            gw, gb = wgrad(x, g, wparam=ctx.wb[0], bparam=ctx.wb[1], N=n, H=h, W=wd, Cin=cinp, Cout=coutp, k=k,
                           w_shape=tuple(w.shape), ps_r=ps_r, scale=scale, dy_ps=ps_r, want_bias=has_b)
            gw = gw if ctx.needs_input_grad[1] else None
        return gx, gw, gb, (g if has_res else None), None, None, None


def conv(x, w, b, *, res=None, scale=1.0, ps_r=0, link=None):
    return ConvFn.apply(x, w, b, res, float(scale), int(ps_r), link)


class HeadConvFn(torch.autograd.Function):

    @staticmethod
    def forward(ctx, x, w, b, sub, dtype):
        _need_gpu(x)
        cout, cin, k, _ = w.shape
        n, c, h, wd = x.shape
        assert c == cin
        xu = unfold_raw(x, sub, k, dtype)
        pk = _pack_head(w, b, dtype)
        out = torch.empty((n, h, wd, pad16(cout)), dtype=dtype, device=x.device)
        conv_raw(xu, pk, N=n, H=h, W=wd, Cin=xu.shape[3], Cout=out.shape[3], out=out)
        ctx.save_for_backward(xu, w)
        ctx.has_b = b is not None
        return out

    @staticmethod
    def backward(ctx, g):
        xu, w = ctx.saved_tensors
        g = g.contiguous()
        n, h, wd, kp = xu.shape
        gw = gb = None
        if ctx.needs_input_grad[1] or ctx.needs_input_grad[2]:
            gw, gb = wgrad_raw(xu, g, N=n, H=h, W=wd, Cin=kp, Cout=g.shape[3], k=1, w_shape=tuple(w.shape),
                               want_bias=ctx.has_b)
            gw = gw if ctx.needs_input_grad[1] else None
        return None, gw, gb, None, None


def _pack_head(w, b, dtype):
    return pack_conv(w, b, dtype, as_1x1=True)


def head_conv(x, w, b, sub, dtype):
    return HeadConvFn.apply(x, w, b, sub, dtype)


class TailConvFn(torch.autograd.Function):

    @staticmethod
    def forward(ctx, x, w, b, res, post_add, ps_r):
        _need_gpu(x)
        n, h, wd, cinp = x.shape
        cout, cin, k, _ = w.shape
        r = ps_r if ps_r > 1 else 1
        pk = pack_conv(w, b, x.dtype)
        out = torch.empty((n, cout // (r * r), h * r, wd * r), dtype=torch.float32, device=x.device)
        resc = None if res is None else _f32c(res)
        conv_raw(x, pk, N=n, H=h, W=wd, Cin=cinp, Cout=cout, out=out, out_mode=L.OUT_PLANAR, ps_r=ps_r,
                 res=resc, post_add=post_add)
        ctx.save_for_backward(x, w)
        ctx.cfg = (ps_r, b is not None, res is not None)
        ctx.wb = (w, b)
        ctx.pg = _tok()
        return out

    @staticmethod
    def backward(ctx, g):
        x, w = ctx.saved_tensors
        ps_r, has_b, has_res = ctx.cfg
        n, h, wd, cinp = x.shape
        cout, cin, k, _ = w.shape
        dy = to_nhwc(g, x.dtype, ps_r=ps_r)
        gx = gw = gb = None
        if ctx.needs_input_grad[0]:
            pkd = pack_conv(w, None, x.dtype, dgrad=True, token=ctx.pg)
            gx = torch.empty_like(x)
            conv_raw(dy, pkd, N=n, H=h, W=wd, Cin=dy.shape[3], Cout=cinp, out=gx, use_bias=False)
        if ctx.needs_input_grad[1] or ctx.needs_input_grad[2]:
            gw, gb = wgrad(x, dy, wparam=ctx.wb[0], bparam=ctx.wb[1], N=n, H=h, W=wd, Cin=cinp, Cout=dy.shape[3], k=k,
                           w_shape=tuple(w.shape), want_bias=has_b)
            gw = gw if ctx.needs_input_grad[1] else None
        return gx, gw, gb, (g if has_res else None), None, None


def tail_conv(x, w, b, *, res=None, post_add=None, ps_r=0):
    return TailConvFn.apply(x, w, b, res, post_add, int(ps_r))


class SkipConvFn(torch.autograd.Function):

    @staticmethod
    def forward(ctx, x, w, b, sub, ps_r, dtype):
        _need_gpu(x)
        cout, cin, k, _ = w.shape
        n, c, h, wd = x.shape
        r = ps_r if ps_r > 1 else 1
        xu = unfold_raw(x, sub, k, dtype)
        pk = _pack_head(w, b, dtype)
        out = torch.empty((n, cout // (r * r), h * r, wd * r), dtype=torch.float32, device=x.device)
        conv_raw(xu, pk, N=n, H=h, W=wd, Cin=xu.shape[3], Cout=cout, out=out, out_mode=L.OUT_PLANAR, ps_r=ps_r)
        ctx.save_for_backward(xu, w)
        ctx.cfg = (ps_r, b is not None)
        return out

    @staticmethod
    def backward(ctx, g):
        xu, w = ctx.saved_tensors
        ps_r, has_b = ctx.cfg
        n, h, wd, kp = xu.shape
        gw = gb = None
        if ctx.needs_input_grad[1] or ctx.needs_input_grad[2]:
            dy = to_nhwc(g, xu.dtype, ps_r=ps_r)
            gw, gb = wgrad_raw(xu, dy, N=n, H=h, W=wd, Cin=kp, Cout=dy.shape[3], k=1, w_shape=tuple(w.shape),
                               want_bias=has_b)
            gw = gw if ctx.needs_input_grad[1] else None
        return None, gw, gb, None, None, None


def skip_conv(x, w, b, sub, ps_r, dtype):
    return SkipConvFn.apply(x, w, b, sub, int(ps_r), dtype)


_HR_COLLAPSE = _knob("SRK_NO_HR_COLLAPSE", "0") != "1"


def hr_tail_ok(x, wu, wt, ps_r):
    if not _HR_COLLAPSE or int(ps_r) != 2 or x.dtype not in (torch.bfloat16, torch.float16):
        return False
    cu, ci, ku, _ = wu.shape
    o, c, kt, _ = wt.shape
    if ku != 3 or kt != 3 or cu != 4 * c or ci != 64 or x.shape[3] != 64 or not 1 <= o <= 4:
        return False
    n, h, w, _ = x.shape
    return n > 0 and max(h, w) <= 512 and x.numel() * 2 < _ADDR_LIMIT and n * o * 4 * h * w < (1 << 31)


def _hr_bufs(o, ci, dev):
    f32 = torch.float32
    return dict(weff=torch.empty((4 * o, ci, 5, 5), dtype=f32, device=dev), beff=torch.empty(4 * o, dtype=f32, device=dev),
                wedge=torch.empty((4, 2 * o, ci, 5), dtype=f32, device=dev), bedge=torch.empty((4, 2 * o), dtype=f32, device=dev),
                wcor=torch.empty((4, o, ci), dtype=f32, device=dev), bcor=torch.empty((4, o), dtype=f32, device=dev))


class HrTailFn(torch.autograd.Function):

    @staticmethod
    def _args(x, wu, bu, wt, bt, bufs, **kw):
        n, h, w, _ = x.shape
        o, c = wt.shape[0], wt.shape[1]
        return L.HrTailArgs(wt=wt.data_ptr(), bt=_ptr(bt), wu=wu.data_ptr(), bu=_ptr(bu), O=o, C=c, Ci=wu.shape[1],
                            weff=bufs["weff"].data_ptr(), beff=bufs["beff"].data_ptr(), wedge=bufs["wedge"].data_ptr(),
                            bedge=bufs["bedge"].data_ptr(), wcor=bufs["wcor"].data_ptr(), bcor=bufs["bcor"].data_ptr(),
                            x=x.data_ptr(), x_pitch=_pitch(x), N=n, H=h, W=w, dtype=_DT[x.dtype], **kw)

    @staticmethod
    def forward(ctx, x, wu, bu, wt, bt, post_add):
        _need_gpu(x)
        n, h, w, ci = x.shape
        o = wt.shape[0]
        dev, f32 = x.device, torch.float32
        wu_, wt_ = _f32c(wu), _f32c(wt)
        bu_, bt_ = (None if bu is None else _f32c(bu)), (None if bt is None else _f32c(bt))
        bufs = _hr_bufs(o, ci, dev)
        L.call("srk_hrtail_collapse", HrTailFn._args(x, wu_, bu_, wt_, bt_, bufs), _stream())
        pk = pack_conv(bufs["weff"], bufs["beff"], x.dtype, cache=False)
        out = torch.empty((n, o, 2 * h, 2 * w), dtype=f32, device=dev)
        conv_raw(x, pk, N=n, H=h, W=w, Cin=ci, Cout=4 * o, out=out, out_mode=L.OUT_PLANAR, ps_r=2, post_add=post_add)
        L.call("srk_hrtail_edge_fwd", HrTailFn._args(x, wu_, bu_, wt_, bt_, bufs, out=out.data_ptr()), _stream())
        ctx.save_for_backward(x, wu_, wt_, *( [bu_] if bu_ is not None else []))
        ctx.has = (bu is not None, bt is not None)
        ctx.bufs = bufs
        ctx.wb = (wu, bu, wt, bt)
        return out

    @staticmethod
    def backward(ctx, g):
        x, wu_, wt_ = ctx.saved_tensors[:3]
        has_bu, has_bt = ctx.has
        bu_ = ctx.saved_tensors[3] if has_bu else None
        bufs = ctx.bufs
        n, h, w, ci = x.shape
        o, c = wt_.shape[0], wt_.shape[1]
        dev, f32 = x.device, torch.float32
        g = _f32c(g)
        st = _stream()
        g12 = to_nhwc(g, x.dtype, ps_r=2)
        need_x = ctx.needs_input_grad[0]
        need_w = any(ctx.needs_input_grad[1:5])
        gx = None
        if need_x:
            pkd = pack_conv(bufs["weff"], None, x.dtype, dgrad=True, cache=False)
            gx = torch.empty_like(x)
            conv_raw(g12, pkd, N=n, H=h, W=w, Cin=g12.shape[3], Cout=ci, out=gx, use_bias=False)
            L.call("srk_hrtail_edge_bwd_x", HrTailFn._args(x, wu_, bu_, wt_, None, bufs, g=g.data_ptr(), dx=gx.data_ptr(), dx_pitch=_pitch(gx)), st)
        gwu = gbu = gwt = gbt = None
        if need_w:
            r, r0 = wgrad_raw(x, g12, N=n, H=h, W=w, Cin=ci, Cout=g12.shape[3], k=5, w_shape=(4 * o, ci, 5, 5), want_bias=True)
            red = dict(eedge=torch.empty((4, 2 * o, ci, 5), dtype=f32, device=dev), e0=torch.empty((4, 2 * o), dtype=f32, device=dev),
                       ecor=torch.empty((4, o, ci), dtype=f32, device=dev), k0=torch.empty((4, o), dtype=f32, device=dev))
            scratch = torch.empty(int(L.load().srk_hrtail_scratch_floats(n, ci)), dtype=f32, device=dev)
            ptrs = {k: v.data_ptr() for k, v in red.items()}
            L.call("srk_hrtail_edge_bwd_w", HrTailFn._args(x, wu_, bu_, wt_, None, bufs, g=g.data_ptr(), scratch=scratch.data_ptr(), **ptrs), st)
            pu, pbu, pt, pbt = ctx.wb
            gwu, gwt = (route(p, shape, dev, slice=p.dtype == f32, buffer=True).out for p, shape in ((pu, tuple(wu_.shape)), (pt, tuple(wt_.shape))))
            gbu = route(pbu, (4 * c,), dev, slice=pbu.dtype == f32, buffer=True).out if has_bu else None
            gbt = route(pbt, (o,), dev, slice=pbt.dtype == f32, buffer=True).out if has_bt else None
            L.call("srk_hrtail_expand", HrTailFn._args(x, wu_, bu_, wt_, None, bufs, r=r.data_ptr(), r0=r0.data_ptr(), dwt=gwt.data_ptr(),
                                                       dbt=_ptr(gbt), dwu=gwu.data_ptr(), dbu=_ptr(gbu), **ptrs), st)
        return gx, gwu, gbu, gwt, gbt, None


def hr_tail(x, wu, bu, wt, bt, *, post_add=None):
    return HrTailFn.apply(x, wu, bu, wt, bt, post_add)


class ConvChainFn(torch.autograd.Function):

    @staticmethod
    def forward(ctx, x, scale, relus, *params):
        _need_gpu(x)
        L_ = len(relus)
        ws, bs = params[0::2], params[1::2]
        n, h, wd, _ = x.shape
        acts = [x]
        bits = []
        a = x
        paired = L_ == 2 and tuple(relus) == (True, False) and pair_ok(x, ws[0], ws[1])
        if paired:
            y1 = torch.empty_like(x)
            a = conv_pair_raw(x, pack_conv(ws[0], bs[0], x.dtype), pack_conv(ws[1], bs[1], x.dtype), out=torch.empty_like(x),
                              relu_mid=True, mid=y1, scale_out=scale, res=x)
            acts.append(y1)
        for i in range(0 if paired else L_):
            w = ws[i]
            cout, cin, k, _ = w.shape
            pk = pack_conv(w, bs[i], x.dtype)
            out = torch.empty((n, h, wd, pad16(cout)), dtype=x.dtype, device=x.device)
            last = i == L_ - 1
            conv_raw(a, pk, N=n, H=h, W=wd, Cin=a.shape[3], Cout=out.shape[3], out=out, relu=relus[i],
                     scale=scale if last else 1.0, res=x if last else None,
                     relu_bits="want" if (relus[i] and not last and ctx.needs_input_grad[0]) else None)
            a = out
            if not last:
                acts.append(a)
                bits.append(out.__dict__.pop("_srk_bits", None))
        ctx.bits = bits
        ctx.save_for_backward(*acts, *ws)
        ctx.cfg = (scale, tuple(relus), tuple(b is not None for b in bs))
        ctx.wb = (tuple(ws), tuple(bs))
        ctx.pg = _tok()
        return a

    @staticmethod
    def backward(ctx, g):
        scale, relus, has_b = ctx.cfg
        L_ = len(relus)
        acts, ws = ctx.saved_tensors[:L_], ctx.saved_tensors[L_:]
        g = g.contiguous()
        n, h, wd, _ = g.shape
        grads = [None] * (2 * L_)
        dy = g
        paired = L_ == 2 and relus == (True, False) and pair_ok(g, ws[0], ws[1])
        if paired:
            x, y1 = acts
            g1 = torch.empty_like(g)
            gx = conv_pair_raw(g, pack_conv(ws[1], None, g.dtype, dgrad=True, token=ctx.pg),
                               pack_conv(ws[0], None, g.dtype, dgrad=True, token=ctx.pg), out=torch.empty_like(g),
                               scale_mid=scale, mask=y1, mid=g1, res=g, use_bias=False)
            for i, (a_in, d, sc) in enumerate(((x, g1, 1.0), (y1, g, scale))):
                if ctx.needs_input_grad[3 + 2 * i] or ctx.needs_input_grad[4 + 2 * i]:
                    gw, grads[2 * i + 1] = wgrad(
                        a_in, d, wparam=ctx.wb[0][i], bparam=ctx.wb[1][i], N=n, H=h, W=wd, Cin=64, Cout=64, k=3,
                        w_shape=tuple(ws[i].shape), scale=sc, want_bias=has_b[i])
                    grads[2 * i] = gw if ctx.needs_input_grad[3 + 2 * i] else None
            return (gx, None, None, *grads)
        for i in range(L_ - 1, -1, -1):
            w = ws[i]
            a_in = acts[i]
            k = w.shape[2]
            sc = scale if i == L_ - 1 else 1.0
            if ctx.needs_input_grad[3 + 2 * i] or ctx.needs_input_grad[4 + 2 * i]:
                gw, gb = wgrad(a_in, dy, wparam=ctx.wb[0][i], bparam=ctx.wb[1][i], N=n, H=h, W=wd, Cin=a_in.shape[3],
                               Cout=dy.shape[3], k=k, w_shape=tuple(w.shape), scale=sc, want_bias=has_b[i])
                grads[2 * i], grads[2 * i + 1] = (gw if ctx.needs_input_grad[3 + 2 * i] else None), gb
            pkd = pack_conv(w, None, g.dtype, dgrad=True, token=ctx.pg)
            gin = torch.empty_like(a_in)
            mk = a_in if (i > 0 and relus[i - 1]) else None
            mb = ctx.bits[i - 1] if (mk is not None and i - 1 < len(ctx.bits)) else None
            conv_raw(dy, pkd, N=n, H=h, W=wd, Cin=dy.shape[3], Cout=a_in.shape[3], out=gin, scale=sc,
                     res=g if i == 0 else None, mask=mk, mask_bits=mb, use_bias=False)
            dy = gin
        return (dy, None, None, *grads)


def conv_chain(x, convs, relus, scale=1.0):
    flat = []
    for w, b in convs:
        flat += [w, b]
    return ConvChainFn.apply(x, float(scale), tuple(bool(r) for r in relus), *flat)


_TRUNK_OFF = _knob("SRK_NO_TRUNK", "0") == "1"


def _trunk_layer(x, pk, out, *, relu=False, scale=1.0, res=None, relu_bits=None, mask_bits=None, use_bias=True):
    return _conv_args(x, pk, out, Cin=64, Cout=64, relu=int(relu), scale=float(scale), res=res, relu_bits=relu_bits, mask_bits=mask_bits,
                      use_bias=use_bias)


def _trunk_add_layer(x, res, out):
    return _conv_args(x, None, out, res=res, CoutP=64, Cout=64)


def _trunk_launch(layers, dev):
    import ctypes as C
    nl = len(layers)
    host = (L.ConvArgs * nl)(*layers)
    lib = L.load()
    if not lib.srk_conv_trunk_ok(host, nl):
        return False
    st = _stream()
    nbytes = C.sizeof(L.ConvArgs) * nl
    table = _upload_table(C.addressof(host), nbytes, _roundup(nbytes, 16), dev, st)
    L.check(lib.srk_conv_trunk(host, table.data_ptr(), nl, st), "srk_conv_trunk")
    return True


def res_trunk_ok(x, blocks, tail):
    if _TRUNK_OFF or not _SIGN_BITS or getattr(_TLS, "seg", None) is not None or not x.is_cuda or x.dtype not in (torch.bfloat16, torch.float16):
        return False
    if x.dim() != 4 or x.shape[3] != 64 or not x.is_contiguous() or not blocks:
        return False
    cus = L.load().srk_device_cus()
    if cus <= 0 or x.shape[0] < cus or x.shape[0] % cus != 0 or _batch_chunks(x.shape[0], x) != 1:
        return False
    ws = [w for blk in blocks for (w, _b) in blk] + [tail[0]]
    return all(len(blk) == 2 for blk in blocks) and all(tuple(w.shape) == (64, 64, 3, 3) for w in ws)


class ResTrunkFn(torch.autograd.Function):

    @staticmethod
    def forward(ctx, x, scale, nb, *params):
        _need_gpu(x)
        dt, dev = x.dtype, x.device
        n, h, wd, _ = x.shape
        ws, bs = params[0::2], params[1::2]
        train = any(ctx.needs_input_grad)
        xs, hs, bits, layers = [x], [], [], []
        spare = []

        def take():
            return spare.pop() if spare else torch.empty_like(x)
        cur = x
        for b in range(nb):
            hb, xo = take(), take()
            bt = torch.empty((n * h * wd, 2), dtype=torch.int32, device=dev) if train else None
            layers.append(_trunk_layer(cur, pack_conv(ws[2 * b], bs[2 * b], dt), hb, relu=True, relu_bits=bt))
            layers.append(_trunk_layer(hb, pack_conv(ws[2 * b + 1], bs[2 * b + 1], dt), xo, scale=scale, res=cur))
            if train:
                xs.append(xo)
                hs.append(hb)
                bits.append(bt)
            else:
                spare.append(hb)
                if cur is not x:
                    spare.append(cur)
            cur = xo
        out = take()
        layers.append(_trunk_layer(cur, pack_conv(ws[2 * nb], bs[2 * nb], dt), out, res=x))
        if not _trunk_launch(layers, dev):
            raise RuntimeError("ResTrunkFn: srk_conv_trunk_ok refused a table res_trunk_ok had accepted")
        if train:
            ctx.save_for_backward(*xs, *hs, *ws)
            ctx.bits = bits
            ctx.cfg = (float(scale), int(nb), tuple(b is not None for b in bs))
            ctx.wb = (tuple(ws), tuple(bs))
            ctx.pg = _tok()
        return out

    @staticmethod
    def backward(ctx, g):
        scale, nb, has_b = ctx.cfg
        sv = ctx.saved_tensors
        xs, hs, ws = sv[:nb + 1], sv[nb + 1:2 * nb + 1], sv[2 * nb + 1:]
        g = g.contiguous()
        dt, dev = g.dtype, g.device
        n, h, wd, _ = g.shape
        need_x = bool(ctx.needs_input_grad[0])

        def pkd(w):
            return pack_conv(w, None, dt, dgrad=True, token=ctx.pg)
        gxs = [None] * (nb + 1)
        ghs = [None] * nb
        gxs[nb] = torch.empty_like(g)
        layers = [_trunk_layer(g, pkd(ws[2 * nb]), gxs[nb], use_bias=False)]
        for b in range(nb - 1, -1, -1):
            ghs[b] = torch.empty_like(g)
            layers.append(_trunk_layer(gxs[b + 1], pkd(ws[2 * b + 1]), ghs[b], scale=scale, mask_bits=ctx.bits[b], use_bias=False))
            if b > 0 or need_x:
                gxs[b] = torch.empty_like(g)
                layers.append(_trunk_layer(ghs[b], pkd(ws[2 * b]), gxs[b], res=gxs[b + 1], use_bias=False))
        gx = None
        if need_x:
            gx = torch.empty_like(g)
            layers.append(_trunk_add_layer(gxs[0], g, gx))
        if not _trunk_launch(layers, dev):
            raise RuntimeError("ResTrunkFn.backward: srk_conv_trunk_ok refused the data-gradient table")
        grads = [None] * (2 * (2 * nb + 1))
        jobs = [(2 * nb, xs[nb], g, 1.0)]
        for b in range(nb - 1, -1, -1):
            jobs += [(2 * b + 1, hs[b], gxs[b + 1], scale), (2 * b, xs[b], ghs[b], 1.0)]
        for i, a_in, dy, sc in jobs:
            if ctx.needs_input_grad[3 + 2 * i] or ctx.needs_input_grad[4 + 2 * i]:
                gw, grads[2 * i + 1] = wgrad(a_in, dy, wparam=ctx.wb[0][i], bparam=ctx.wb[1][i], N=n, H=h, W=wd, Cin=64, Cout=64, k=3,
                                             w_shape=(64, 64, 3, 3), scale=sc, want_bias=has_b[i])
                grads[2 * i] = gw if ctx.needs_input_grad[3 + 2 * i] else None
        return (gx, None, None, *grads)


def res_trunk(x, blocks, tail, scale=1.0):
    flat = []
    for blk in blocks:
        for w, b in blk:
            flat += [w, b]
    flat += [tail[0], tail[1]]
    return ResTrunkFn.apply(x, float(scale), len(blocks), *flat)


class record_segments:

    def __init__(self, every=1, limit=None):
        self.every, self.count, self.cuts, self.limit, self.taken, self.keeps = max(1, int(every)), 0, [], limit, 0, 0

    def __enter__(self):
        self.prev = getattr(_TLS, "seg", None)
        _TLS.seg = self
        return self

    def __exit__(self, *exc):
        _TLS.seg = self.prev


def cut(*ts, keep=False):
    rec = getattr(_TLS, "seg", None)
    out = ts
    if rec is not None:
        if not keep:
            rec.count += 1
        else:
            rec.keeps += 1
        take = keep or (rec.count % rec.every == 0 and (rec.limit is None or rec.taken < rec.limit))
        if take and any(t.requires_grad for t in ts):
            if not keep:
                rec.taken += 1
            out = tuple(t.detach().requires_grad_(True) if t.requires_grad else t for t in ts)
            rec.cuts.append([(o, l) for o, l in zip(ts, out) if l is not o])
    return out[0] if len(out) == 1 else out


def backward_segments(loss, cuts, after=None):
    loss.backward()
    if after is not None:
        after(0)
    for k, pairs in enumerate(reversed(cuts), 1):
        roots = [o for o, l in pairs if l.grad is not None]
        grads = [l.grad for o, l in pairs if l.grad is not None]
        if roots:
            torch.autograd.backward(roots, grads)
        if after is not None:
            after(k)


class _WnFn(torch.autograd.Function):
    @staticmethod
    def forward(ctx, grp, *params):
        grp._launch(params, backward=False)
        ctx.grp = grp
        ctx.save_for_backward(*params)
        return tuple(grp.flat[o:o + n].view(shape) for (o, n, shape, _, _) in grp.layout)

    @staticmethod
    def backward(ctx, *grads):
        grp, params = ctx.grp, ctx.saved_tensors
        flush_wgrads()
        dev = params[0].device
        dflat = torch.empty(grp.total, dtype=torch.float32, device=dev)
        dg = torch.empty(grp.rows, dtype=torch.float32, device=dev)
        gs = []
        for gr, (off, n, shape, r0, rows) in zip(grads, grp.layout):
            if gr is None:
                gr = torch.zeros(shape, dtype=torch.float32, device=dev)
            elif gr.dtype != torch.float32 or not gr.is_contiguous():
                gr = gr.float().contiguous()
            gs.append(gr)
        grp._launch(params, backward=True, dws=gs, dv=dflat, dg=dg)
        out = [None]
        for (off, n, shape, r0, rows) in grp.layout:
            out += [dflat[off:off + n].view(shape), dg[r0:r0 + rows].view(rows, *([1] * (len(shape) - 1)))]
        return tuple(out)


class WeightNormGroup:

    def __init__(self, convs):
        self.convs = list(convs)
        self.flat = self.inv = None
        self.layout = []
        self.total = self.rows = 0
        self.key = None

    def _build(self, params):
        dev = params[0].device
        off = r0 = 0
        self.layout = []
        for v in params[0::2]:
            n, rows = v.numel(), v.shape[0]
            self.layout.append((off, n, tuple(v.shape), r0, rows))
            off += _roundup(n, 4)
            r0 += rows
        self.total, self.rows = off, r0
        self.flat = torch.empty(off, dtype=torch.float32, device=dev)
        self.inv = torch.empty(r0, dtype=torch.float32, device=dev)

    def _launch(self, params, backward, dws=None, dv=None, dg=None):
        import ctypes as C
        key = tuple(p.data_ptr() for p in params)
        if self.flat is None or self.key != key or self.flat.device != params[0].device:
            for p in params:
                if p.dtype != torch.float32 or not p.is_contiguous() or not p.is_cuda:
                    raise RuntimeError("WeightNormGroup needs contiguous fp32 weight_v / weight_g on the GPU")
            if self.flat is None or self.flat.device != params[0].device or [tuple(v.shape) for v in params[0::2]] != [l[2] for l in self.layout]:
                self._build(params)
            self.key = key
        n = len(self.layout)
        host = (L.WnJob * n)()
        for i, (off, cnt, shape, r0, rows) in enumerate(self.layout):
            v, g = params[2 * i], params[2 * i + 1]
            j = host[i]
            j.v, j.g, j.w, j.inv = v.data_ptr(), g.data_ptr(), self.flat.data_ptr() + 4 * off, self.inv.data_ptr() + 4 * r0
            j.rows, j.cols, j.row0 = rows, cnt // rows, r0
            if backward:
                j.dw, j.dv, j.dg = dws[i].data_ptr(), dv.data_ptr() + 4 * off, dg.data_ptr() + 4 * r0
        nbytes = C.sizeof(L.WnJob) * n
        st = _stream()
        table = _upload_table(C.addressof(host), nbytes, _roundup(nbytes, 16), params[0].device, st)
        L.check(L.load().srk_weight_norm_group(table.data_ptr(), n, self.rows, 1 if backward else 0, st), "srk_weight_norm_group")

    def weights(self):
        params = []
        for c in self.convs:
            params += [c.weight_v, c.weight_g]
        _need_gpu(params[0])
        ws = _WnFn.apply(self, *params)
        for w, c in zip(ws, self.convs):
            mark_proxy(w)
            w.__dict__["_srk_pack_key"] = ("wn", id(c.weight_v))
        return list(ws)


_PW_OFF = _knob("SRK_NO_PW", "0") == "1"


def pw_ok(x, w1, w2):
    if _PW_OFF or x.dtype not in (torch.bfloat16, torch.float16) or x.numel() == 0:
        return False
    if w1.shape[2] != 1 or w2.shape[2] != 1 or w1.shape[1] != x.shape[3] or w2.shape[1] != w1.shape[0]:
        return False
    if x.numel() // x.shape[3] * max(x.shape[3], _roundup(w2.shape[0], 64)) * 2 >= _ADDR_LIMIT:
        return False
    return bool(L.load().srk_pw_shape_ok(int(w1.shape[1]), int(w1.shape[0]), _roundup(int(w2.shape[0]), 64)))


def pw_forward_raw(x, pk, out):
    n, h, wd, _ = x.shape
    L.call("srk_pw_forward", L.PwArgs(x=x.data_ptr(), x_pitch=_pitch(x), x_coff=0, P=n * h * wd, Cin=pk.cin, Chid=pk.chid, CoutP=pk.coutp,
                                      Cout=out.shape[3], wpk=pk.fwd.data_ptr(), out=out.data_ptr(), out_pitch=_pitch(out), out_coff=0,
                                      dtype=_DT[x.dtype]), _stream())
    return out


def pw_backward_raw(x, gz, pk, gx, *, res=None, h_out=None, gh_out=None):
    n, h, wd, _ = x.shape
    L.call("srk_pw_backward", L.PwBwdArgs(
        x=x.data_ptr(), x_pitch=_pitch(x), x_coff=0, gz=gz.data_ptr(), gz_pitch=_pitch(gz), gz_coff=0, Cz=gz.shape[3], P=n * h * wd,
        Cin=pk.cin, Chid=pk.chid, CoutP=pk.coutp, wpk=pk.bwd.data_ptr(), res=_ptr(res), res_pitch=0 if res is None else _pitch(res), res_coff=0,
        gx=gx.data_ptr(), gx_pitch=_pitch(gx), gx_coff=0, h_out=_ptr(h_out), gh_out=_ptr(gh_out), dtype=_DT[x.dtype]), _stream())
    return gx


def pw_wgrad_raw(x, gz, pk, w1_shape, w2_shape, want_b1=True, want_b2=True):
    n, h, wd, _ = x.shape
    P = n * h * wd
    dev = x.device
    nr = L.load().srk_pw_wgrad_ranges(P, pk.chid)
    scratch = torch.empty(nr * (pk.chid * (pk.cin + pk.coutp + 1) + pk.coutp), dtype=torch.float32, device=dev)
    dw1 = torch.empty(w1_shape, dtype=torch.float32, device=dev)
    dw2 = torch.empty(w2_shape, dtype=torch.float32, device=dev)
    db1 = torch.empty(pk.chid, dtype=torch.float32, device=dev) if want_b1 else None
    db2 = torch.empty(pk.cmid, dtype=torch.float32, device=dev) if want_b2 else None
    o2 = nr * pk.chid * pk.cin
    o3 = o2 + nr * pk.chid * pk.coutp
    o4 = o3 + nr * pk.chid
    a = L.PwWgradArgs(
        x=x.data_ptr(), x_pitch=_pitch(x), x_coff=0, gz=gz.data_ptr(), gz_pitch=_pitch(gz), gz_coff=0, Cz=gz.shape[3], P=P,
        Cin=pk.cin, Chid=pk.chid, Cmid=pk.cmid, CoutP=pk.coutp, wpk=pk.bwd.data_ptr(),
        dw1p=scratch.data_ptr(), dw2p=scratch.data_ptr() + 4 * o2, db1p=scratch.data_ptr() + 4 * o3,
        db2p=(scratch.data_ptr() + 4 * o4) if want_b2 else 0, nranges=nr,
        dw1=dw1.data_ptr(), db1=_ptr(db1), dw2=dw2.data_ptr(), db2=_ptr(db2), dtype=_DT[x.dtype])
    L.call("srk_pw_wgrad", a, _stream())
    return dw1, db1, dw2, db2


class WdsrBlockBFn(torch.autograd.Function):

    @staticmethod
    def forward(ctx, x, scale, w1, b1, w2, b2, w3, b3):
        _need_gpu(x)
        n, h, wd, cp = x.shape
        dt = x.dtype
        pk = pw_pack(w1, b1, w2, b2, dt)
        ctx.pg = _tok()
        z = torch.empty((n, h, wd, pad16(w2.shape[0])), dtype=dt, device=x.device)
        pw_forward_raw(x, pk, z)
        out = torch.empty_like(x)
        conv_raw(z, pack_conv(w3, b3, dt), N=n, H=h, W=wd, Cin=z.shape[3], Cout=cp, out=out, scale=scale, res=x)
        ctx.save_for_backward(x, z, w1, w2, w3)
        ctx.pk, ctx.scale = pk, scale
        ctx.wb = (w1, b1, w2, b2, w3, b3)
        ctx.pg = _tok()
        return out

    @staticmethod
    def backward(ctx, g):
        x, z, w1, w2, w3 = ctx.saved_tensors
        scale = ctx.scale
        _, b1, _, b2, _, b3 = ctx.wb
        g = g.contiguous()
        n, h, wd, cp = x.shape
        dt = x.dtype
        pk = ctx.pk if ctx.pg is None else pw_pack(ctx.wb[0], b1, ctx.wb[2], b2, dt, token=ctx.pg)
        gz = torch.empty_like(z)
        conv_raw(g, pack_conv(w3, None, dt, dgrad=True, token=ctx.pg), N=n, H=h, W=wd, Cin=cp, Cout=z.shape[3], out=gz, scale=scale, use_bias=False)
        gw3, gb3 = wgrad(z, g, wparam=ctx.wb[4], bparam=b3, N=n, H=h, W=wd, Cin=z.shape[3], Cout=cp, k=3, w_shape=tuple(w3.shape),
                         scale=scale, want_bias=b3 is not None)
        gx = torch.empty_like(x)
        pw_backward_raw(x, gz, pk, gx, res=g)
        gw1, gb1, gw2, gb2 = pw_wgrad_raw(x, gz, pk, tuple(w1.shape), tuple(w2.shape), want_b1=b1 is not None, want_b2=b2 is not None)
        return gx, None, gw1, gb1, gw2, gb2, gw3, gb3


def wdsr_block_b(x, convs, scale=1.0):
    (w1, b1), (w2, b2), (w3, b3) = convs
    if pw_ok(x, w1, w2) and w3.shape[2] == 3 and w3.shape[0] == x.shape[3]:
        return WdsrBlockBFn.apply(x, float(scale), w1, b1, w2, b2, w3, b3)
    return conv_chain(x, convs, [True, False, False], scale=scale)



class _CAHint:
    __slots__ = ("t", "out_ref", "gsum", "g_ptr", "g_ver", "__weakref__")

    def __init__(self, t, out):
        self.t, self.out_ref = t, weakref.ref(out)
        self.gsum = self.g_ptr = self.g_ver = None


class _LazyApply:
    __slots__ = ("t", "x", "sums", "w", "s", "z", "out")

    def __init__(self, t, x, sums, w, s, z, out):
        self.t, self.x, self.sums, self.w, self.s, self.z, self.out = t, x, sums, w, s, z, out


def _fwd_state():
    st = _TLS
    if not hasattr(st, "ca_hint"):
        st.ca_hint = st.lazy = None
    return st


PAIR_LAUNCHES = [0, 0, 0]


class RCABFn(torch.autograd.Function):

    @staticmethod
    def forward(ctx, x, w1, b1, w2, b2, cw1, cb1, cw2, cb2, lazy_in=None, lazy_out=False):
        _need_gpu(x)
        n, h, wd, cp = x.shape
        dt = x.dtype
        c = w2.shape[0]
        cr = cw1.shape[0]
        y1 = torch.empty_like(x)
        t = torch.empty_like(x)
        paired = pair_ok(x, w1, w2)
        assert paired or (lazy_in is None and not lazy_out), "the lazy channel-attention protocol is for the paired launches"
        if paired:
            ns = L.load().srk_conv_pair_tiles(1, h, wd)
            sums = torch.empty((n, ns, cp), dtype=torch.float32, device=x.device)
            if lazy_in is None:
                conv_pair_raw(x, pack_conv(w1, b1, dt), pack_conv(w2, b2, dt), out=t, relu_mid=True, mid=y1, pool=sums)
            else:
                conv_pair_raw(lazy_in.t, pack_conv(w1, b1, dt), pack_conv(w2, b2, dt), out=t, relu_mid=True, mid=y1, pool=sums,
                              ca_fwd=dict(x2=lazy_in.x, sums=lazy_in.sums, w1=lazy_in.w[0], b1=lazy_in.w[1], w2=lazy_in.w[2],
                                          b2=lazy_in.w[3], s_out=lazy_in.s, z_out=lazy_in.z), xo=x)
        else:
            conv_raw(x, pack_conv(w1, b1, dt), N=n, H=h, W=wd, Cin=cp, Cout=cp, out=y1, relu=True, relu_bits="want")
            ctx.bits = y1.__dict__.pop("_srk_bits", None)
            conv_raw(y1, pack_conv(w2, b2, dt), N=n, H=h, W=wd, Cin=cp, Cout=cp, out=t)
            ns = L.load().srk_ca_splits(n, h * wd)
            sums = torch.empty((n, ns, cp), dtype=torch.float32, device=x.device)
            L.call("srk_ca_pool", L.CaPoolArgs(t=t.data_ptr(), t_pitch=cp, t_coff=0, u=0, u_pitch=0, u_coff=0,
                                               sums=sums.data_ptr(), N=n, HW=h * wd, C=cp, dtype=_DT[dt]), _stream())
        s = torch.empty((n, cp), dtype=torch.float32, device=x.device)
        z = torch.empty((n, cr), dtype=torch.float32, device=x.device)
        out = torch.empty_like(x)
        w1f, b1f, w2f, b2f = _ca_params(cw1, cb1, cw2, cb2, cp)
        fst = _fwd_state()
        fst.lazy = None
        if lazy_out:
            fst.lazy = _LazyApply(t, x, sums, (w1f, b1f, w2f, b2f), s, z, out)
        else:
            L.call("srk_ca_apply", L.CaApplyArgs(
                t=t.data_ptr(), t_pitch=cp, t_coff=0, res=x.data_ptr(), res_pitch=cp, res_coff=0, sums=sums.data_ptr(),
                w1=w1f.data_ptr(), b1=b1f.data_ptr(), w2=w2f.data_ptr(), b2=b2f.data_ptr(),
                s_out=s.data_ptr(), z_out=z.data_ptr(), out=out.data_ptr(), out_pitch=cp, out_coff=0,
                N=n, HW=h * wd, C=cp, Cr=cr, dtype=_DT[dt], sums_rows=ns), _stream())
        ctx.save_for_backward(x, y1, t, sums, s, z, w1, w2, cw1, cw2)
        ctx.wb = (w1, b1, w2, b2)
        ctx.ca = (cw1, cb1, cw2, cb2)
        ctx.pg = _tok()
        prev, ctx.hint_in, ctx.hint_out = fst.ca_hint, None, None
        if paired:
            if prev is not None and prev.out_ref() is x and prev.t.shape == x.shape:
                ctx.hint_in = prev
            ctx.hint_out = fst.ca_hint = _CAHint(t, out)
        else:
            fst.ca_hint = None
        return out

    @staticmethod
    def backward(ctx, g):
        x, y1, t, sums, s, z, w1, w2, cw1, cw2 = ctx.saved_tensors
        g = g.contiguous()
        n, h, wd, cp = x.shape
        dt = x.dtype
        c, cr = w2.shape[0], cw1.shape[0]
        dev = x.device
        ho = ctx.hint_out
        if ho is not None and ho.gsum is not None and ho.g_ptr == g.data_ptr() and ho.g_ver == g._version and ho.gsum.shape[0] == n:
            gsum = ho.gsum
            gs_rows = gsum.shape[1]
        else:
            gs_rows = L.load().srk_ca_splits(n, h * wd)
            gsum = torch.empty((n, gs_rows, cp), dtype=torch.float32, device=dev)
            L.call("srk_ca_pool", L.CaPoolArgs(t=t.data_ptr(), t_pitch=cp, t_coff=0, u=g.data_ptr(), u_pitch=_pitch(g), u_coff=0,
                                               sums=gsum.data_ptr(), N=n, HW=h * wd, C=cp, dtype=_DT[dt]), _stream())
        w1f, _, w2f, _ = _ca_params(cw1, None, cw2, None, cp)
        per = torch.empty((max(n, 1), 2 * cr * cp + cr + cp), dtype=torch.float32, device=dev)
        if n == 0:
            per.zero_()
        dw1, db1 = per[0, :cr * cp], per[0, cr * cp:cr * cp + cr]
        dw2, db2 = per[0, cr * cp + cr:2 * cr * cp + cr], per[0, 2 * cr * cp + cr:]
        gt = torch.empty_like(x)
        paired = pair_ok(g, w1, w2)
        fuse_ca = paired and cp == 64 and cr <= 8 and gs_rows <= 64 and sums.shape[1] <= 64 and not _CA_UNFUSED
        if not fuse_ca:
            L.call("srk_ca_bwd_apply", L.CaBwdArgs(
                g=g.data_ptr(), g_pitch=_pitch(g), g_coff=0, gsum=gsum.data_ptr(), sums=sums.data_ptr(), s=s.data_ptr(),
                z=z.data_ptr(), w1=w1f.data_ptr(), w2=w2f.data_ptr(), dw1=dw1.data_ptr(), db1=db1.data_ptr(),
                dw2=dw2.data_ptr(), db2=db2.data_ptr(), gt=gt.data_ptr(), gt_pitch=cp, gt_coff=0,
                N=n, HW=h * wd, C=cp, Cr=cr, dtype=_DT[dt], sums_rows=sums.shape[1], gsum_rows=gs_rows), _stream())
        g1 = torch.empty_like(x)
        gx = torch.empty_like(x)
        if paired:
            hi = ctx.hint_in
            pool = None
            if hi is not None and hi.t.shape == gx.shape and hi.t.dtype == dt:
                pool = torch.empty((n, L.load().srk_conv_pair_tiles(1, h, wd), cp), dtype=torch.float32, device=dev)
            conv_pair_raw(g if fuse_ca else gt, pack_conv(w2, None, dt, dgrad=True, token=ctx.pg),
                          pack_conv(w1, None, dt, dgrad=True, token=ctx.pg),
                          out=gx, mask=y1, mid=g1, res=g, use_bias=False, pool=pool, pool_aux=None if pool is None else hi.t,
                          ca_bwd=dict(gsum=gsum, sums=sums, s=s, z=z, w1=w1f, w2=w2f, slots=per) if fuse_ca else None,
                          xo=gt if fuse_ca else None)
            if pool is not None:
                hi.gsum, hi.g_ptr, hi.g_ver = pool, gx.data_ptr(), gx._version
        else:
            conv_raw(gt, pack_conv(w2, None, dt, dgrad=True, token=ctx.pg), N=n, H=h, W=wd, Cin=cp, Cout=cp, out=g1, mask=y1,
                     mask_bits=getattr(ctx, "bits", None), use_bias=False)
        gw2, gb2 = wgrad(y1, gt, wparam=ctx.wb[2], bparam=ctx.wb[3], N=n, H=h, W=wd, Cin=cp, Cout=cp, k=w2.shape[2],
                         w_shape=tuple(w2.shape), want_bias=ctx.wb[3] is not None)
        gw1, gb1 = wgrad(x, g1, wparam=ctx.wb[0], bparam=ctx.wb[1], N=n, H=h, W=wd, Cin=cp, Cout=cp, k=w1.shape[2],
                         w_shape=tuple(w1.shape), want_bias=ctx.wb[1] is not None)
        if not paired:
            conv_raw(g1, pack_conv(w1, None, dt, dgrad=True, token=ctx.pg), N=n, H=h, W=wd, Cin=cp, Cout=cp, out=gx, res=g, use_bias=False)
        if c == cp:
            o1, o2, o3 = cr * cp, cr * cp + cr, 2 * cr * cp + cr
            outs = defer_rowsum(per, (ctx.ca[0], ctx.ca[1], ctx.ca[2], ctx.ca[3]),
                                (((cr, c, 1, 1), 0), ((cr,), o1), ((c, cr, 1, 1), o2), ((c,), o3)))
            if outs is not None:
                return (gx, gw1, gb1, gw2, gb2, *outs, None, None)
        tot = per.sum(0)
        dw1, db1 = tot[:cr * cp], tot[cr * cp:cr * cp + cr]
        dw2, db2 = tot[cr * cp + cr:2 * cr * cp + cr], tot[2 * cr * cp + cr:]
        gcw1 = dw1.view(cr, cp)[:, :c].reshape(cr, c, 1, 1)
        gcw2 = dw2.view(cp, cr)[:c].reshape(c, cr, 1, 1)
        return gx, gw1, gb1, gw2, gb2, gcw1, db1, gcw2, db2[:c], None, None


def _ca_params(cw1, cb1, cw2, cb2, cp):
    cr, c = cw1.shape[0], cw1.shape[1]
    w1 = _f32c(cw1).view(cr, c)
    w2 = _f32c(cw2).view(c, cr)
    b1 = None if cb1 is None else _f32c(cb1)
    b2 = None if cb2 is None else _f32c(cb2)
    if cp != c:
        w1 = torch.nn.functional.pad(w1, (0, cp - c)).contiguous()
        w2 = torch.nn.functional.pad(w2, (0, 0, 0, cp - c)).contiguous()
        if b2 is not None:
            b2 = torch.nn.functional.pad(b2, (0, cp - c)).contiguous()
    return w1, b1, w2, b2


def rcab(x, w1, b1, w2, b2, cw1, cb1, cw2, cb2):
    return RCABFn.apply(x, w1, b1, w2, b2, cw1, cb1, cw2, cb2)


def rcab_chain(x, blocks):
    if not blocks:
        return x
    fst = _fwd_state()
    w1, w2 = blocks[0][0], blocks[0][2]
    lazy_ok = (not _CA_UNFUSED and pair_ok(x, w1, w2) and x.shape[3] == 64 and L.load().srk_conv_pair_tiles(1, x.shape[1], x.shape[2]) <= 64
               and all(tuple(b[0].shape) == (64, 64, 3, 3) and tuple(b[2].shape) == (64, 64, 3, 3) and b[5] is not None and b[7] is not None
                       and b[4].shape[1] == 64 and b[4].shape[0] <= 8 for b in blocks))
    lazy = None
    for i, b in enumerate(blocks):
        last = i == len(blocks) - 1
        x = RCABFn.apply(x, *b, lazy, lazy_ok and not last)
        lazy = fst.lazy if (lazy_ok and not last) else None
        fst.lazy = None
    return x


class RDBFn(torch.autograd.Function):

    @staticmethod
    def forward(ctx, x, dest, *params):
        _need_gpu(x)
        n, h, wd, g0 = x.shape
        nconv = (len(params) - 2) // 2
        ws, bs = params[0:2 * nconv:2], params[1:2 * nconv:2]
        wl, bl = params[-2], params[-1]
        g = ws[0].shape[0]
        assert g0 % 16 == 0 and g % 16 == 0, "dense-block widths must be multiples of 16"
        ctot = g0 + nconv * g
        feat = torch.empty((n, h, wd, ctot), dtype=x.dtype, device=x.device)
        feat[..., :g0].copy_(x)
        for c in range(nconv):
            cin = g0 + c * g
            conv_raw(feat[..., :cin], pack_conv(ws[c], bs[c], x.dtype), N=n, H=h, W=wd, Cin=cin, Cout=g,
                     out=feat[..., cin:cin + g], relu=True)
        out = torch.empty_like(x) if dest is None else dest[0].slice(dest[1], x)
        conv_raw(feat, pack_conv(wl, bl, x.dtype), N=n, H=h, W=wd, Cin=ctot, Cout=g0, out=out, res=x)
        ctx.save_for_backward(feat, *ws, wl)
        ctx.cfg = (nconv, g0, g)
        ctx.wb = (tuple(ws), tuple(bs))
        ctx.pg = _tok()
        return out

    @staticmethod
    def backward(ctx, gout):
        nconv, g0, g = ctx.cfg
        feat = ctx.saved_tensors[0]
        ws, wl = ctx.saved_tensors[1:1 + nconv], ctx.saved_tensors[-1]
        gout = gout.contiguous()
        n, h, wd, ctot = feat.shape
        dt = feat.dtype
        grads = [None] * (2 * nconv + 2)
        gwl, gbl = wgrad_raw(feat, gout, N=n, H=h, W=wd, Cin=ctot, Cout=g0, k=1, w_shape=tuple(wl.shape))
        grads[-2], grads[-1] = gwl, gbl
        gfeat = torch.empty_like(feat)
        conv_raw(gout, pack_conv(wl, None, dt, dgrad=True, token=ctx.pg), N=n, H=h, W=wd, Cin=g0, Cout=ctot, out=gfeat,
                 mask=feat, mask_from=ctot - g, use_bias=False)
        for c in range(nconv - 1, -1, -1):
            cin = g0 + c * g
            dy = gfeat[..., cin:cin + g]
            gw, gb = wgrad(feat[..., :cin], dy, wparam=ctx.wb[0][c], bparam=ctx.wb[1][c], N=n, H=h, W=wd, Cin=cin, Cout=g,
                           k=ws[c].shape[2], w_shape=tuple(ws[c].shape), want_bias=ctx.wb[1][c] is not None)
            grads[2 * c], grads[2 * c + 1] = gw, gb
            pref = gfeat[..., :cin]
            conv_raw(dy, pack_conv(ws[c], None, dt, dgrad=True, token=ctx.pg), N=n, H=h, W=wd, Cin=g, Cout=cin, out=pref, res=pref,
                     mask=feat[..., :cin] if c > 0 else None, mask_from=cin - g if c > 0 else 0, use_bias=False)
        gx = gfeat[..., :g0] + gout
        return (gx, None, *grads)


_SLICE_GACC = _knob("SRK_NO_SLICE_GACC", "0") != "1"


class SliceBuffer:

    def __init__(self, count, accumulate_grads=False):
        self.count, self.buf = int(count), None
        self.accumulate = bool(accumulate_grads) and _SLICE_GACC
        self.ks = []
        self.gbuf, self.last_k = None, None

    def alloc(self, n, h, w, c, dtype, device):
        self.buf = torch.empty((n, h, w, self.count * c), dtype=dtype, device=device)
        self.c = c
        return self

    def slice(self, i, like=None):
        if self.buf is None:
            n, h, w, c = like.shape
            self.alloc(n, h, w, c, like.dtype, like.device)
        c = self.c if like is None else like.shape[3]
        return self.buf[..., i * c:(i + 1) * c]

    def grad_dest(self, k):
        if self.gbuf is None:
            if k != max(self.ks):
                raise RuntimeError(f"SliceBuffer: the consumer of prefix {k} runs its backward before the one of prefix {max(self.ks)}")
            self.gbuf = torch.empty_like(self.buf)
            self.last_k = None
            first = True
        else:
            first = False
        return self.gbuf[..., :k * self.c], not first

    def deliver(self, k, g):
        c = self.c
        if self.gbuf is not None and g.data_ptr() == self.gbuf.data_ptr():
            pass
        elif self.gbuf is None:
            if k != max(self.ks):
                raise RuntimeError(f"SliceBuffer: the consumer of prefix {k} runs its backward before the one of prefix {max(self.ks)}")
            if k == self.count and g.is_contiguous():
                self.gbuf = g
            else:
                self.gbuf = torch.zeros_like(self.buf)
                self.gbuf[..., :k * c].copy_(g)
            self.last_k = None
        else:
            self.gbuf[..., :k * c].add_(g)
        if self.last_k is not None and k >= self.last_k:
            raise RuntimeError(f"SliceBuffer: consumers must run their backward longest prefix first (prefix {k} after {self.last_k})")
        self.last_k = k
        below = [q for q in self.ks if q < k]
        lo = max(below) if below else 0
        out = [self.gbuf[..., i * c:(i + 1) * c] if i >= lo else None for i in range(k)]
        if not below:
            self.gbuf, self.last_k = None, None
        return out


class ConcatSlicesFn(torch.autograd.Function):
    @staticmethod
    def forward(ctx, holder, *parts):
        ctx.c = c = parts[0].shape[3]
        ctx.holder, ctx.k = holder, len(parts)
        for i, p_ in enumerate(parts):
            assert p_.numel() == 0 or p_.data_ptr() == holder.buf.data_ptr() + i * ctx.c * p_.element_size(), \
                "part %d is not slice %d of the buffer" % (i, i)
        if holder.accumulate and len(parts) not in holder.ks:
            holder.ks.append(len(parts))
        if len(parts) == holder.count:
            out = holder.buf.view(holder.buf.shape)
        else:
            out = holder.buf[..., :len(parts) * c]
        return out

    @staticmethod
    def backward(ctx, g):
        c = ctx.c
        if ctx.holder.accumulate:
            return (None, *ctx.holder.deliver(ctx.k, g))
        return (None, *[g[..., i * c:(i + 1) * c] for i in range(g.shape[3] // c)])


def concat_slices(holder, parts):
    out = ConcatSlicesFn.apply(holder, *parts)
    if holder.accumulate:
        out.__dict__["_srk_gacc"] = (holder, len(parts))
    return out


class AddIntoFn(torch.autograd.Function):

    @staticmethod
    def forward(ctx, a, b, holder, index):
        return chan_apply(a.contiguous(), y=b.contiguous(), out=holder.slice(index, a))

    @staticmethod
    def backward(ctx, g):
        return g, g, None, None


def add_into(a, b, dest):
    return AddIntoFn.apply(a, b, dest[0], dest[1]) if dest is not None else a.add(b)


def rdb(x, convs, lff, dest=None):
    flat = []
    for w, b in convs:
        flat += [w, b]
    return RDBFn.apply(x, dest, *flat, lff[0], lff[1])


from .grads import *
from .grads import _WQ, _upload_table
from .ops_norm import *
from .ops_proj import *
from .ops_proj import _proj_launch
from .ops_metrics import *
from .flip import *
```

Before: 47700 LR patches/s.

## Fuse HR-tail gradient layout pass and restructure edge kernels into single launches

Replaces the generic pixel-shuffle NHWC conversion of the output gradient with a dedicated kernel that writes the g12 tensor and also a compact buffer of border-line gradients, which the edge backward kernels read instead of doing strided reads of the full HR gradient. The edge forward kernel is templated on output channels, computes all 2*O outputs per position in registers with weights laid out for vector loads, splits each edge across z-blocks, and handles corners in one launch instead of two phases. Edge backward-x also merges its phases into a single launch with a dedicated corner role. This adds extra LDS use, more template instantiations and more complex corner logic, which carries some risk to correctness.

```diff
diff --git a/include/srk.h b/include/srk.h
--- a/include/srk.h
+++ b/include/srk.h
@@ -439,6 +439,8 @@
   float* scratch;
   const float* r; const float* r0;
   float* dwt; float* dbt; float* dwu; float* dbu;
+  void* g12;
+  float* gb;
 } srk_hrtail_args;
 int srk_hrtail_collapse(const srk_hrtail_args* a, srk_stream_t stream);
 int srk_hrtail_edge_fwd(const srk_hrtail_args* a, srk_stream_t stream);
@@ -446,6 +448,8 @@
 long long srk_hrtail_scratch_floats(int N, int Ci);
 int srk_hrtail_edge_bwd_w(const srk_hrtail_args* a, srk_stream_t stream);
 int srk_hrtail_expand(const srk_hrtail_args* a, srk_stream_t stream);
+long long srk_hrtail_gb_floats(int N, int O, int H, int W);
+int srk_hrtail_grad_layout(const srk_hrtail_args* a, srk_stream_t stream);
 
 typedef struct { float* p; const float* g; long long state_off; long long n; long long step_idx; } srk_adam_slot;
 typedef struct { int slot; int count; long long start; } srk_adam_block;
diff --git a/sr-pytorch-lightning_amd/_lib.py b/sr-pytorch-lightning_amd/_lib.py
--- a/sr-pytorch-lightning_amd/_lib.py
+++ b/sr-pytorch-lightning_amd/_lib.py
@@ -222,7 +222,8 @@
                 ("x", _p), ("x_pitch", _i), ("N", _i), ("H", _i), ("W", _i), ("dtype", _i),
                 ("out", _p), ("g", _p), ("dx", _p), ("dx_pitch", _i),
                 ("eedge", _p), ("e0", _p), ("ecor", _p), ("k0", _p), ("scratch", _p),
-                ("r", _p), ("r0", _p), ("dwt", _p), ("dbt", _p), ("dwu", _p), ("dbu", _p)]
+                ("r", _p), ("r0", _p), ("dwt", _p), ("dbt", _p), ("dwu", _p), ("dbu", _p),
+                ("g12", _p), ("gb", _p)]
 
 
 LAUNCHERS = {
@@ -263,13 +264,14 @@
     "srk_hrtail_edge_bwd_x": HrTailArgs,
     "srk_hrtail_edge_bwd_w": HrTailArgs,
     "srk_hrtail_expand": HrTailArgs,
+    "srk_hrtail_grad_layout": HrTailArgs,
 }
 OTHER_SYMBOLS = ("srk_conv_tile", "srk_last_error", "srk_version", "srk_device_cus", "srk_wgrad_slabs",
                  "srk_pack_conv_weights_group", "srk_l1_blocks", "srk_wgrad_group_ok", "srk_wgrad_group_job_bytes",
                  "srk_wgrad_group_plan", "srk_conv2d_wgrad_group", "srk_wgrad_finalize_group", "srk_upload_small", "srk_upload_prepare", "srk_upload_eager", "srk_upload_fence", "srk_ca_splits", "srk_chan_stats_blocks",
                  "srk_conv_pair_tiles", "srk_rowsum_group", "srk_pw_shape_ok", "srk_pw_pack_bytes", "srk_pw_pack_group", "srk_weight_norm_group", "srk_pw_wgrad_ranges", "srk_l1_loss_mean", "srk_chan_stats_finalize", "srk_pack_group_tiles", "srk_pack_conv_weights_group_tiled",
                  "srk_proj_pack", "srk_proj_pack_bytes", "srk_proj_wgrad_scratch_floats", "srk_proj_pack_group", "srk_wgrad_slab_cout",
-                 "srk_hrtail_scratch_floats", "srk_adam_step_scaled", "srk_adam_check_scaled", "srk_adam_update_scaled", "srk_loss_scale_update", "srk_conv_bits_ok",
+                 "srk_hrtail_scratch_floats", "srk_hrtail_gb_floats", "srk_adam_step_scaled", "srk_adam_check_scaled", "srk_adam_update_scaled", "srk_loss_scale_update", "srk_conv_bits_ok",
                  "srk_conv_trunk", "srk_conv_trunk_ok", "srk_flip_blocks", "srk_flip_mean",
                  "srk_ms_ssim_workspace_bytes", "srk_ms_ssim_tiles")
 
@@ -377,6 +379,8 @@
     lib.srk_proj_wgrad_scratch_floats.restype = C.c_longlong
     lib.srk_hrtail_scratch_floats.argtypes = [C.c_int, C.c_int]
     lib.srk_hrtail_scratch_floats.restype = C.c_longlong
+    lib.srk_hrtail_gb_floats.argtypes = [C.c_int, C.c_int, C.c_int, C.c_int]
+    lib.srk_hrtail_gb_floats.restype = C.c_longlong
     lib.srk_conv_bits_ok.argtypes = [C.POINTER(ConvArgs)]
     lib.srk_conv_bits_ok.restype = C.c_int
     lib.srk_conv_trunk_ok.argtypes = [C.POINTER(ConvArgs), C.c_int]
diff --git a/sr-pytorch-lightning_amd/csrc/hr_tail.hip b/sr-pytorch-lightning_amd/csrc/hr_tail.hip
--- a/sr-pytorch-lightning_amd/csrc/hr_tail.hip
+++ b/sr-pytorch-lightning_amd/csrc/hr_tail.hip
@@ -154,17 +154,17 @@
     if (i + 256 * k < n) dst[i + 256 * k] = v[k];
 }
 template <int DT>
-SRK_DEV void stage_line(const srk_hrtail_args& a, const EdgeGeo& e, int n, float* Xl, int pitch) {
+SRK_DEV void stage_span(const srk_hrtail_args& a, const EdgeGeo& e, int n, float* Xl, int pitch, int sbeg, int cnt) {
   typedef DTraits<DT> Tr;
   const int Ci = a.Ci;
   if ((Ci & 7) == 0 && (a.x_pitch & 7) == 0) {
-    const int nch = Ci >> 3, total = (e.len + 4) * nch;
+    const int nch = Ci >> 3, total = cnt * nch;
     for (int i0 = threadIdx.x; i0 < total; i0 += 256 * 4) {
       i32x4 raw[4];
 #pragma unroll
       for (int u = 0; u < 4; ++u) {
         const int i = i0 + 256 * u;
-        const int sp = i / nch, c8 = i - sp * nch, s = sp - 2;
+        const int sp = i / nch, c8 = i - sp * nch, s = sp + sbeg;
         raw[u] = i32x4{0, 0, 0, 0};
         if (i < total && s >= 0 && s < e.len) {
           const int yy = e.row ? e.fix_lr : s, xx = e.row ? s : e.fix_lr;
@@ -186,162 +186,265 @@
     }
     return;
   }
-  for (int i = threadIdx.x; i < (e.len + 4) * Ci; i += 256) {
-    const int s = i / Ci - 2, ci = i % Ci;
+  for (int i = threadIdx.x; i < cnt * Ci; i += 256) {
+    const int sp = i / Ci, s = sp + sbeg, ci = i % Ci;
     float v = 0.f;
     if (s >= 0 && s < e.len) {
       const int yy = e.row ? e.fix_lr : s, xx = e.row ? s : e.fix_lr;
       v = ld_act<DT>(a.x, ((size_t)(n * a.H + yy) * a.W + xx) * a.x_pitch + ci);
     }
-    Xl[(s + 2) * pitch + ci] = v;
-  }
-}
-
+    Xl[sp * pitch + ci] = v;
+  }
+}
 template <int DT>
-__global__ __launch_bounds__(256) void hrtail_edge_fwd_kernel(const srk_hrtail_args a, int phase) {
-  const int H = a.H, W = a.W, O = a.O, Ci = a.Ci, H2 = 2 * H, W2 = 2 * W;
+SRK_DEV void stage_line(const srk_hrtail_args& a, const EdgeGeo& e, int n, float* Xl, int pitch) { stage_span<DT>(a, e, n, Xl, pitch, -2, e.len + 4); }
+
+SRK_DEV size_t gb_edge_off(int ty, int O, int H, int W) {
+  return ty == 0 ? 0 : ty == 1 ? (size_t)2 * O * W : ty == 2 ? (size_t)4 * O * W : (size_t)4 * O * W + (size_t)2 * O * H;
+}
+SRK_DEV float g_line(const srk_hrtail_args& a, const EdgeGeo& e, int n, int kk, int s) {
+  if (a.gb) return a.gb[(size_t)n * 4 * a.O * (a.H + a.W) + gb_edge_off(e.ty, a.O, a.H, a.W) + (size_t)kk * e.len + s];
+  const int o = kk >> 1, q = kk & 1, W2 = 2 * a.W;
+  const float* const g = a.g + ((size_t)n * a.O + o) * (size_t)(2 * a.H) * W2;
+  return e.row ? g[(size_t)e.fix_hr * W2 + 2 * s + q] : g[(size_t)(2 * s + q) * W2 + e.fix_hr];
+}
+
+template <int O> SRK_DEV void edge_chains(const float* __restrict__ x, int pitch, const float* __restrict__ Wl, int Ci, float (&acc)[2 * O][5]) {
+  constexpr int WS = (10 * O + 3) & ~3;
+  for (int ci = 0; ci < Ci; ++ci) {
+    float xv[5];
+#pragma unroll
+    for (int tt = 0; tt < 5; ++tt) xv[tt] = x[tt * pitch + ci];
+    float w[WS];
+#pragma unroll
+    for (int v = 0; v < WS / 4; ++v) {
+      const float4 w4 = reinterpret_cast<const float4*>(Wl + (size_t)ci * WS)[v];
+      w[4 * v] = w4.x; w[4 * v + 1] = w4.y; w[4 * v + 2] = w4.z; w[4 * v + 3] = w4.w;
+    }
+#pragma unroll
+    for (int kk = 0; kk < 2 * O; ++kk)
+#pragma unroll
+      for (int tt = 0; tt < 5; ++tt) acc[kk][tt] += w[kk * 5 + tt] * xv[tt];
+  }
+}
+template <int DT, int O>
+__global__ __launch_bounds__(256) void hrtail_edge_fwd_kernel(const srk_hrtail_args a) {
+  constexpr int K2 = 2 * O, WS = (10 * O + 3) & ~3;
+  const int H = a.H, W = a.W, Ci = a.Ci, H2 = 2 * H, W2 = 2 * W;
   const int n = blockIdx.x;
-  const EdgeGeo e = edge_geo(2 * phase + blockIdx.y, H, W);
+  const EdgeGeo e = edge_geo(blockIdx.y, H, W);
+  const int per = ((H > W ? H : W) + gridDim.z - 1) / gridDim.z;
+  const int s0 = blockIdx.z * per, s1 = min(e.len, s0 + per);
+  if (s0 >= s1) return;
+  const int pitch = Ci + 1;
   extern __shared__ __attribute__((aligned(16))) char smem_raw[];
-  const int pitch = Ci + 1;
   float* const Xl = reinterpret_cast<float*>(smem_raw);
-  float* const Wl = Xl + (size_t)(e.len + 4) * pitch;
-  stage_line<DT>(a, e, n, Xl, pitch);
-  stage_copy256(Wl, a.wedge + (size_t)e.ty * 2 * O * Ci * 5, 2 * O * Ci * 5);
+  float* const Wl = Xl + (((size_t)(per + 4) * pitch + 3) & ~(size_t)3);
+  float* const Xr = Wl + (size_t)Ci * WS;
+  float* const Wr = Xr + (size_t)10 * Ci;
+  float* const Wc = Wr + (size_t)10 * O * Ci;
+  const int cb = e.ty == 3 ? 1 : 0;
+  const bool corners = !e.row && (s0 == 0 || s1 == e.len);
+  stage_span<DT>(a, e, n, Xl, pitch, s0 - 2, s1 - s0 + 4);
+  {
+    const float* const src = a.wedge + (size_t)e.ty * K2 * Ci * 5;
+    for (int i = threadIdx.x; i < K2 * Ci * 5; i += 256) {
+      const int kk = i / (Ci * 5), r = i - kk * Ci * 5, ci = r / 5, tt = r - ci * 5;
+      Wl[ci * WS + kk * 5 + tt] = src[i];
+    }
+  }
+  if (corners) {
+    const int sr = cb ? W - 1 : 0;
+    for (int ca = 0; ca < 2; ++ca) stage_span<DT>(a, edge_geo(ca, H, W), n, Xr + ca * 5 * Ci, Ci, sr - 2, 5);
+    for (int i = threadIdx.x; i < 2 * O * Ci * 5; i += 256) {
+      const int ca = i / (O * Ci * 5), r = i - ca * O * Ci * 5, o = r / (Ci * 5), rest = r - o * Ci * 5;
+      Wr[i] = a.wedge[((size_t)ca * K2 + o * 2 + cb) * Ci * 5 + rest];
+    }
+    for (int i = threadIdx.x; i < 2 * O * Ci; i += 256) {
+      const int ca = i / (O * Ci), r = i - ca * O * Ci;
+      Wc[i] = a.wcor[(size_t)(ca * 2 + cb) * O * Ci + r];
+    }
+  }
   __syncthreads();
   const size_t oplane = (size_t)H2 * W2;
   float* const out = a.out + (size_t)n * O * oplane;
-  for (int idx = threadIdx.x + 256 * blockIdx.z; idx < 2 * e.len * O; idx += 256 * gridDim.z) {
-    const int p = idx % (2 * e.len), o = idx / (2 * e.len);
-    const int s = p >> 1, q = p & 1;
-    const float* const w = Wl + (size_t)(o * 2 + q) * Ci * 5;
-    const float* const x = Xl + (size_t)s * pitch;
-    float a0 = a.bedge[e.ty * 2 * O + o * 2 + q], a1 = 0.f, a2 = 0.f, a3 = 0.f, a4 = 0.f;
-    for (int ci = 0; ci < Ci; ++ci) {
-      a0 += w[ci * 5 + 0] * x[0 * pitch + ci]; a1 += w[ci * 5 + 1] * x[1 * pitch + ci]; a2 += w[ci * 5 + 2] * x[2 * pitch + ci];
-      a3 += w[ci * 5 + 3] * x[3 * pitch + ci]; a4 += w[ci * 5 + 4] * x[4 * pitch + ci];
-    }
-    float acc = ((a0 + a1) + (a2 + a3)) + a4;
-    if (!e.row && (p == 0 || p == 2 * e.len - 1)) {
-      const int ca = p == 0 ? 0 : 1, cb = e.ty == 2 ? 0 : 1, c = ca * 2 + cb;
+  for (int s = s0 + (int)threadIdx.x; s < s1; s += 256) {
+    float acc[K2][5];
+#pragma unroll
+    for (int kk = 0; kk < K2; ++kk) {
+      acc[kk][0] = a.bedge[e.ty * K2 + kk];
+#pragma unroll
+      for (int tt = 1; tt < 5; ++tt) acc[kk][tt] = 0.f;
+    }
+    edge_chains<O>(Xl + (size_t)(s - s0) * pitch, pitch, Wl, Ci, acc);
+#pragma unroll
+    for (int kk = 0; kk < K2; ++kk) {
+      const int o = kk >> 1, q = kk & 1, p = 2 * s + q;
+      const float tot = ((acc[kk][0] + acc[kk][1]) + (acc[kk][2] + acc[kk][3])) + acc[kk][4];
+      const size_t at = (size_t)o * oplane + (e.row ? (size_t)e.fix_hr * W2 + p : (size_t)p * W2 + e.fix_hr);
+      const bool corner = p == 0 || p == 2 * e.len - 1;
+      if (!corner) { out[at] -= tot; continue; }
+      if (e.row) continue;
+      const int ca = p == 0 ? 0 : 1;
+      const float* const xr = Xr + ca * 5 * Ci;
+      const float* const wr = Wr + ((size_t)ca * O + o) * Ci * 5;
+      float r0 = a.bedge[ca * K2 + o * 2 + cb], r1 = 0.f, r2 = 0.f, r3 = 0.f, r4 = 0.f;
+      for (int ci = 0; ci < Ci; ++ci) {
+        r0 += wr[ci * 5 + 0] * xr[0 * Ci + ci]; r1 += wr[ci * 5 + 1] * xr[1 * Ci + ci]; r2 += wr[ci * 5 + 2] * xr[2 * Ci + ci];
+        r3 += wr[ci * 5 + 3] * xr[3 * Ci + ci]; r4 += wr[ci * 5 + 4] * xr[4 * Ci + ci];
+      }
+      const float rowt = ((r0 + r1) + (r2 + r3)) + r4;
+      const int c = ca * 2 + cb;
       float cc = a.bcor[c * O + o];
-      const float* const xc = Xl + (size_t)(s + 2) * pitch;
-      for (int ci = 0; ci < Ci; ++ci) cc += a.wcor[((size_t)c * O + o) * Ci + ci] * xc[ci];
-      acc -= cc;
-    }
-    const size_t at = e.row ? (size_t)e.fix_hr * W2 + p : (size_t)p * W2 + e.fix_hr;
-    out[(size_t)o * oplane + at] -= acc;
-  }
-}
-
+      const float* const xc = Xl + (size_t)(s - s0 + 2) * pitch;
+      const float* const wc = Wc + ((size_t)ca * O + o) * Ci;
+      for (int ci = 0; ci < Ci; ++ci) cc += wc[ci] * xc[ci];
+      float v = out[at];
+      v -= rowt;
+      v -= tot - cc;
+      out[at] = v;
+    }
+  }
+}
+
+struct EdgeSet {
+  float* G[4]; float* Wt[4]; int slot[4];
+};
+SRK_DEV void edge_corr(const srk_hrtail_args& a, const EdgeGeo& e, const float* Gl, const float* Wl, int s, int c8, float (&corr)[8]) {
+  const int O = a.O, Ci = a.Ci;
+#pragma unroll
+  for (int k = 0; k < 8; ++k) corr[k] = 0.f;
+  for (int kk = 0; kk < 2 * O; ++kk) {
+    const float* const gl = Gl + (size_t)kk * (e.len + 4) + s + 2;
+    float gv[5];
+#pragma unroll
+    for (int tt = 0; tt < 5; ++tt) gv[tt] = gl[2 - tt];
+#pragma unroll
+    for (int k = 0; k < 8; ++k) {
+      const int ci = c8 * 8 + k;
+      if (ci < Ci) {
+        const float* const w = Wl + ((size_t)kk * Ci + ci) * 5;
+#pragma unroll
+        for (int tt = 0; tt < 5; ++tt) corr[k] += w[tt] * gv[tt];
+      }
+    }
+  }
+  if (!e.row && (s == 0 || s == e.len - 1)) {
+    for (int ca = 0; ca < 2; ++ca) {
+      if (!(ca ? s == e.len - 1 : s == 0)) continue;
+      const int cb = e.ty == 2 ? 0 : 1, c = ca * 2 + cb;
+      for (int o = 0; o < O; ++o) {
+        const float gc = Gl[(size_t)(o * 2 + ca) * (e.len + 4) + (ca ? e.len - 1 : 0) + 2];
+#pragma unroll
+        for (int k = 0; k < 8; ++k)
+          if (c8 * 8 + k < Ci) corr[k] -= a.wcor[((size_t)c * O + o) * Ci + c8 * 8 + k] * gc;
+      }
+    }
+  }
+}
 template <int DT>
-__global__ __launch_bounds__(256) void hrtail_edge_bwd_x_kernel(const srk_hrtail_args a, int phase) {
+__global__ __launch_bounds__(256) void hrtail_edge_bwd_x_kernel(const srk_hrtail_args a) {
   typedef DTraits<DT> Tr;
-  const int H = a.H, W = a.W, O = a.O, Ci = a.Ci, H2 = 2 * H, W2 = 2 * W;
-  const int n = blockIdx.x;
-  const bool shared_line = phase == 0 ? H == 1 : W == 1;
-  if (shared_line && blockIdx.y == 1) return;
+  const int H = a.H, W = a.W, O = a.O, Ci = a.Ci;
+  const int n = blockIdx.x, role = blockIdx.y;
+  if ((role == 1 && H == 1) || (role == 3 && W == 1) || (role == 4 && blockIdx.z != 0)) return;
+  int ned = 0, edl[4];
+  if (role == 4) { ned = 4; edl[0] = 0; edl[1] = 1; edl[2] = 2; edl[3] = 3; }
+  else {
+    edl[ned++] = role;
+    if ((role == 0 && H == 1) || (role == 2 && W == 1)) edl[ned++] = role + 1;
+  }
+  const int maxlen = H > W ? H : W;
+  const size_t per_edge = (size_t)2 * O * (maxlen + 4) + (size_t)2 * O * Ci * 5;
   extern __shared__ __attribute__((aligned(16))) char smem_raw[];
-  const size_t gplane = (size_t)H2 * W2;
-  const float* const g = a.g + (size_t)n * O * gplane;
-  for (int rep = 0; rep < (shared_line ? 2 : 1); ++rep) {
-  const EdgeGeo e = edge_geo(2 * phase + (shared_line ? rep : (int)blockIdx.y), H, W);
-  float* const Gl = reinterpret_cast<float*>(smem_raw);
-  float* const Wl = Gl + (size_t)2 * O * (e.len + 4);
-  __syncthreads();
-  for (int i0 = threadIdx.x; i0 < 2 * O * (e.len + 4); i0 += 256 * 4) {
-    float v[4];
-#pragma unroll
-    for (int u = 0; u < 4; ++u) {
-      const int i = i0 + 256 * u;
-      const int kk = i / (e.len + 4), s = i % (e.len + 4) - 2, o = kk >> 1, q = kk & 1;
-      v[u] = 0.f;
-      if (i < 2 * O * (e.len + 4) && s >= 0 && s < e.len)
-        v[u] = e.row ? g[(size_t)o * gplane + (size_t)e.fix_hr * W2 + 2 * s + q] : g[(size_t)o * gplane + (size_t)(2 * s + q) * W2 + e.fix_hr];
-    }
-#pragma unroll
-    for (int u = 0; u < 4; ++u)
-      if (i0 + 256 * u < 2 * O * (e.len + 4)) Gl[i0 + 256 * u] = v[u];
-  }
-  stage_copy256(Wl, a.wedge + (size_t)e.ty * 2 * O * Ci * 5, 2 * O * Ci * 5);
+  float* const base = reinterpret_cast<float*>(smem_raw);
+  for (int i = 0; i < ned; ++i) {
+    const EdgeGeo e = edge_geo(edl[i], H, W);
+    float* const Gl = base + i * per_edge;
+    float* const Wl = Gl + (size_t)2 * O * (maxlen + 4);
+    for (int i0 = threadIdx.x; i0 < 2 * O * (e.len + 4); i0 += 256 * 4) {
+      float v[4];
+#pragma unroll
+      for (int u = 0; u < 4; ++u) {
+        const int j = i0 + 256 * u;
+        const int kk = j / (e.len + 4), s = j % (e.len + 4) - 2;
+        v[u] = 0.f;
+        if (j < 2 * O * (e.len + 4) && s >= 0 && s < e.len) v[u] = g_line(a, e, n, kk, s);
+      }
+#pragma unroll
+      for (int u = 0; u < 4; ++u)
+        if (i0 + 256 * u < 2 * O * (e.len + 4)) Gl[i0 + 256 * u] = v[u];
+    }
+    stage_copy256(Wl, a.wedge + (size_t)e.ty * 2 * O * Ci * 5, 2 * O * Ci * 5);
+  }
   __syncthreads();
   const int nch = (Ci + 7) >> 3;
   const bool vec = (Ci & 7) == 0 && (a.dx_pitch & 7) == 0;
-  for (int idx = threadIdx.x + 256 * blockIdx.z; idx < e.len * nch; idx += 256 * gridDim.z) {
-    const int c8 = idx % nch, s = idx / nch;
-    float corr[8];
-#pragma unroll
-    for (int k = 0; k < 8; ++k) corr[k] = 0.f;
-    for (int kk = 0; kk < 2 * O; ++kk) {
-      const float* const gl = Gl + (size_t)kk * (e.len + 4) + s + 2;
-      float gv[5];
-#pragma unroll
-      for (int tt = 0; tt < 5; ++tt) gv[tt] = gl[2 - tt];
-#pragma unroll
-      for (int k = 0; k < 8; ++k) {
-        const int ci = c8 * 8 + k;
-        if (ci < Ci) {
-          const float* const w = Wl + ((size_t)kk * Ci + ci) * 5;
-#pragma unroll
-          for (int tt = 0; tt < 5; ++tt) corr[k] += w[tt] * gv[tt];
-        }
-      }
-    }
-    if (!e.row && (s == 0 || s == e.len - 1)) {
-      for (int ca = 0; ca < 2; ++ca) {
-        if (!(ca ? s == e.len - 1 : s == 0)) continue;
-        const int cb = e.ty == 2 ? 0 : 1, c = ca * 2 + cb;
-        const size_t at = (size_t)(ca ? H2 - 1 : 0) * W2 + e.fix_hr;
-        for (int o = 0; o < O; ++o) {
-          const float gc = g[(size_t)o * gplane + at];
-#pragma unroll
-          for (int k = 0; k < 8; ++k)
-            if (c8 * 8 + k < Ci) corr[k] -= a.wcor[((size_t)c * O + o) * Ci + c8 * 8 + k] * gc;
-        }
-      }
-    }
-    const int yy = e.row ? e.fix_lr : s, xx = e.row ? s : e.fix_lr;
+  const int len = role == 4 ? 0 : edge_geo(role, H, W).len;
+  const int nitems = role == 4 ? 4 * nch : (len > 2 ? len - 2 : 0) * nch;
+  for (int idx = threadIdx.x + 256 * blockIdx.z; idx < nitems; idx += 256 * gridDim.z) {
+    const int c8 = idx % nch, u = idx / nch;
+    int yy, xx;
+    if (role == 4) {
+      const int ca = u >> 1, cb = u & 1;
+      if ((ca && H == 1) || (cb && W == 1)) continue;
+      yy = ca ? H - 1 : 0; xx = cb ? W - 1 : 0;
+    } else {
+      const EdgeGeo e = edge_geo(role, H, W);
+      yy = e.row ? e.fix_lr : u + 1; xx = e.row ? u + 1 : e.fix_lr;
+    }
     typename Tr::elem* const d = reinterpret_cast<typename Tr::elem*>(a.dx) + ((size_t)(n * H + yy) * W + xx) * a.dx_pitch + c8 * 8;
+    float val[8];
     if (vec) {
       const i32x4 raw = *reinterpret_cast<const i32x4*>(d);
-      const int w4[4] = {raw.x, raw.y, raw.z, raw.w};
-      int o4[4];
-#pragma unroll
-      for (int k = 0; k < 4; ++k) {
-        float f0, f1;
-        unpack2<DT>((uint32_t)w4[k], f0, f1);
-        o4[k] = (int)pack2<DT>(f0 - corr[2 * k], f1 - corr[2 * k + 1]);
-      }
-      *reinterpret_cast<i32x4*>(d) = i32x4{o4[0], o4[1], o4[2], o4[3]};
+      unpack2<DT>((uint32_t)raw.x, val[0], val[1]); unpack2<DT>((uint32_t)raw.y, val[2], val[3]);
+      unpack2<DT>((uint32_t)raw.z, val[4], val[5]); unpack2<DT>((uint32_t)raw.w, val[6], val[7]);
     } else {
 #pragma unroll
+      for (int k = 0; k < 8; ++k) val[k] = c8 * 8 + k < Ci ? Tr::to_f32(d[k]) : 0.f;
+    }
+    for (int i = 0; i < ned; ++i) {
+      const int ty = edl[i];
+      const bool on = ty == 0 ? yy == 0 : ty == 1 ? yy == H - 1 : ty == 2 ? xx == 0 : xx == W - 1;
+      if (!on) continue;
+      const EdgeGeo e = edge_geo(ty, H, W);
+      const float* const Gl = base + i * per_edge;
+      float corr[8];
+      edge_corr(a, e, Gl, Gl + (size_t)2 * O * (maxlen + 4), e.row ? xx : yy, c8, corr);
+#pragma unroll
+      for (int k = 0; k < 8; ++k) val[k] = Tr::to_f32(Tr::from_f32(val[k] - corr[k]));
+    }
+    if (vec) {
+      *reinterpret_cast<i32x4*>(d) = i32x4{(int)pack2<DT>(val[0], val[1]), (int)pack2<DT>(val[2], val[3]),
+                                           (int)pack2<DT>(val[4], val[5]), (int)pack2<DT>(val[6], val[7])};
+    } else {
+#pragma unroll
       for (int k = 0; k < 8; ++k)
-        if (c8 * 8 + k < Ci) d[k] = Tr::from_f32(Tr::to_f32(d[k]) - corr[k]);
-    }
-  }
+        if (c8 * 8 + k < Ci) d[k] = Tr::from_f32(val[k]);
+    }
   }
 }
 
 constexpr int EW_MAXLEN = 512;
 template <int DT>
 __global__ __launch_bounds__(256) void hrtail_edge_bwd_w_kernel(const srk_hrtail_args a, int nchunks, int ew_chunk) {
-  const int H = a.H, W = a.W, O = a.O, Ci = a.Ci, H2 = 2 * H, W2 = 2 * W;
+  const int H = a.H, W = a.W, O = a.O, Ci = a.Ci;
   const int ty = blockIdx.y, chunk = blockIdx.x;
   const int n0 = chunk * ew_chunk, n1 = min(a.N, n0 + ew_chunk);
   const int ncombo = ty < 4 ? 2 * O * 5 : O;
-  const size_t gplane = (size_t)H2 * W2;
   float* const dst = a.scratch + ((size_t)ty * nchunks + chunk) * (size_t)(2 * MAXO * 5) * (Ci + 1);
   extern __shared__ __attribute__((aligned(16))) char smem_raw[];
   float* const Xl = reinterpret_cast<float*>(smem_raw);
   if (ty >= 4) {
     if (blockIdx.z != 0) return;
     const int c = ty - 4, ca = c >> 1, cbb = c & 1;
-    const int Py = ca ? H2 - 1 : 0, Px = cbb ? W2 - 1 : 0, yy = ca ? H - 1 : 0, xx = cbb ? W - 1 : 0;
+    const int yy = ca ? H - 1 : 0, xx = cbb ? W - 1 : 0;
+    const EdgeGeo er = edge_geo(ca, H, W);
     for (int item = threadIdx.x; item < ncombo * (Ci + 1); item += 256) {
       const int ci = item % (Ci + 1), o = item / (Ci + 1);
       float acc = 0.f;
       for (int n = n0; n < n1; ++n) {
-        const float gv = a.g[((size_t)n * O + o) * gplane + (size_t)Py * W2 + Px];
+        const float gv = g_line(a, er, n, o * 2 + cbb, xx);
         const float xv = ci < Ci ? ld_act<DT>(a.x, ((size_t)(n * H + yy) * W + xx) * a.x_pitch + ci) : 1.f;
         acc += gv * xv;
       }
@@ -351,48 +454,61 @@
   }
   const bool rowedge = ty < 2;
   const int len = rowedge ? W : H;
+  const EdgeGeo eg = edge_geo(ty, H, W);
   float* const Gl = Xl + (size_t)(len + 4) * Ci;
-  constexpr int MAXIT = (2 * MAXO * 5 * 65 + 255) / 256;
-  const int nitems = ncombo * (Ci + 1);
-  const int ipb = (nitems + gridDim.z - 1) / gridDim.z, item0 = blockIdx.z * ipb, item1 = min(nitems, item0 + ipb);
-  float acc[MAXIT];
-#pragma unroll
-  for (int k = 0; k < MAXIT; ++k) acc[k] = 0.f;
+  constexpr int MAXG = (2 * MAXO * 65 + 2 * 256 - 1) / (2 * 256);
+  const int ngroups = 2 * O * (Ci + 1);
+  const int gpb = (ngroups + gridDim.z - 1) / gridDim.z, gr0 = blockIdx.z * gpb, gr1 = min(ngroups, gr0 + gpb);
+  float acc[MAXG][5];
+#pragma unroll
+  for (int k = 0; k < MAXG; ++k)
+#pragma unroll
+    for (int tt = 0; tt < 5; ++tt) acc[k][tt] = 0.f;
   for (int n = n0; n < n1; ++n) {
     __syncthreads();
-    stage_line<DT>(a, edge_geo(ty, H, W), n, Xl, Ci);
-    for (int i = threadIdx.x; i < 2 * O * len; i += 256) {
-      const int kk = i / len, s = i % len, o = kk >> 1, q = kk & 1;
-      const float* const g = a.g + ((size_t)n * O + o) * gplane;
-      Gl[i] = rowedge ? g[(size_t)(ty == 0 ? 0 : H2 - 1) * W2 + 2 * s + q] : g[(size_t)(2 * s + q) * W2 + (ty == 2 ? 0 : W2 - 1)];
-    }
+    stage_line<DT>(a, eg, n, Xl, Ci);
+    for (int i = threadIdx.x; i < 2 * O * len; i += 256) Gl[i] = g_line(a, eg, n, i / len, i % len);
     __syncthreads();
 #pragma unroll
-    for (int k = 0; k < MAXIT; ++k) {
-      const int item = item0 + threadIdx.x + k * 256;
-      if (item >= item1) break;
-      const int ci = item % (Ci + 1), cb = item / (Ci + 1), tt = cb % 5, kk = cb / 5;
+    for (int k = 0; k < MAXG; ++k) {
+      const int grp = gr0 + threadIdx.x + k * 256;
+      if (grp >= gr1) break;
+      const int ci = grp % (Ci + 1), kk = grp / (Ci + 1);
       const float* const gr = Gl + kk * len;
-      float t0 = 0.f, t1 = 0.f, t2 = 0.f, t3 = 0.f;
+      float t[5][4];
+#pragma unroll
+      for (int tt = 0; tt < 5; ++tt) t[tt][0] = t[tt][1] = t[tt][2] = t[tt][3] = 0.f;
       int p = 0;
       if (ci < Ci) {
-        const float* const xr = Xl + (size_t)tt * Ci + ci;
+        const float* const xr = Xl + ci;
         for (; p + 3 < len; p += 4) {
-          t0 += gr[p] * xr[(size_t)p * Ci]; t1 += gr[p + 1] * xr[(size_t)(p + 1) * Ci];
-          t2 += gr[p + 2] * xr[(size_t)(p + 2) * Ci]; t3 += gr[p + 3] * xr[(size_t)(p + 3) * Ci];
+          float xv[8];
+#pragma unroll
+          for (int j = 0; j < 8; ++j) xv[j] = xr[(size_t)(p + j) * Ci];
+          const float g0 = gr[p], g1 = gr[p + 1], g2 = gr[p + 2], g3 = gr[p + 3];
+#pragma unroll
+          for (int tt = 0; tt < 5; ++tt) {
+            t[tt][0] += g0 * xv[tt]; t[tt][1] += g1 * xv[tt + 1]; t[tt][2] += g2 * xv[tt + 2]; t[tt][3] += g3 * xv[tt + 3];
+          }
         }
-        for (; p < len; ++p) t0 += gr[p] * xr[(size_t)p * Ci];
-      } else if (tt == 2) {
-        for (; p + 3 < len; p += 4) { t0 += gr[p]; t1 += gr[p + 1]; t2 += gr[p + 2]; t3 += gr[p + 3]; }
-        for (; p < len; ++p) t0 += gr[p];
-      }
-      acc[k] += (t0 + t1) + (t2 + t3);
-    }
-  }
-#pragma unroll
-  for (int k = 0; k < MAXIT; ++k) {
-    const int item = item0 + threadIdx.x + k * 256;
-    if (item < item1) dst[item] = acc[k];
+        for (; p < len; ++p)
+#pragma unroll
+          for (int tt = 0; tt < 5; ++tt) t[tt][0] += gr[p] * xr[(size_t)(p + tt) * Ci];
+      } else {
+        for (; p + 3 < len; p += 4) { t[2][0] += gr[p]; t[2][1] += gr[p + 1]; t[2][2] += gr[p + 2]; t[2][3] += gr[p + 3]; }
+        for (; p < len; ++p) t[2][0] += gr[p];
+      }
+#pragma unroll
+      for (int tt = 0; tt < 5; ++tt) acc[k][tt] += (t[tt][0] + t[tt][1]) + (t[tt][2] + t[tt][3]);
+    }
+  }
+#pragma unroll
+  for (int k = 0; k < MAXG; ++k) {
+    const int grp = gr0 + threadIdx.x + k * 256;
+    if (grp >= gr1) break;
+    const int ci = grp % (Ci + 1), kk = grp / (Ci + 1);
+#pragma unroll
+    for (int tt = 0; tt < 5; ++tt) dst[(size_t)(kk * 5 + tt) * (Ci + 1) + ci] = acc[k][tt];
   }
 }
 
@@ -421,6 +537,78 @@
   } else {
     if (ci < Ci) a.ecor[((size_t)(ty - 4) * O + cb) * Ci + ci] = s;
     else a.k0[(ty - 4) * O + cb] = s;
+  }
+}
+
+template <int DT>
+__global__ __launch_bounds__(256) void hrtail_grad_layout_kernel(const srk_hrtail_args a) {
+  typedef DTraits<DT> Tr;
+  const int H = a.H, W = a.W, O = a.O, W2 = 2 * W;
+  const bool pair = (W & 1) == 0;
+  const int P = pair ? 2 : 1, Wp = W / P;
+  const long long total = (long long)a.N * H * Wp;
+  const size_t plane = (size_t)4 * H * W;
+  for (long long idx = (long long)blockIdx.x * 256 + threadIdx.x; idx < total; idx += (long long)gridDim.x * 256) {
+    const int xp = (int)(idx % Wp);
+    const long long q = idx / Wp;
+    const int y = (int)(q % H), n = (int)(q / H), x0 = xp * P;
+    const float* const gp = a.g + (size_t)n * O * plane + (size_t)(2 * y) * W2 + 2 * x0;
+    float v[2][16];
+#pragma unroll
+    for (int u = 0; u < 2; ++u)
+#pragma unroll
+      for (int c = 0; c < 16; ++c) v[u][c] = 0.f;
+    if (pair) {
+#pragma unroll
+      for (int o = 0; o < MAXO; ++o)
+#pragma unroll
+        for (int r = 0; r < 2; ++r)
+          if (o < O) {
+            const float4 f = *reinterpret_cast<const float4*>(gp + o * plane + (size_t)r * W2);
+            v[0][o * 4 + r * 2] = f.x; v[0][o * 4 + r * 2 + 1] = f.y; v[1][o * 4 + r * 2] = f.z; v[1][o * 4 + r * 2 + 1] = f.w;
+          }
+    } else {
+#pragma unroll
+      for (int o = 0; o < MAXO; ++o)
+#pragma unroll
+        for (int r = 0; r < 2; ++r)
+          if (o < O) {
+            const float2 f = *reinterpret_cast<const float2*>(gp + o * plane + (size_t)r * W2);
+            v[0][o * 4 + r * 2] = f.x; v[0][o * 4 + r * 2 + 1] = f.y;
+          }
+    }
+    typename Tr::elem* const d = reinterpret_cast<typename Tr::elem*>(a.g12) + ((size_t)(n * H + y) * W + x0) * 16;
+#pragma unroll
+    for (int u = 0; u < 2; ++u) {
+      if (u >= P) break;
+#pragma unroll
+      for (int h = 0; h < 2; ++h) {
+        const float* const w = v[u] + 8 * h;
+        *reinterpret_cast<i32x4*>(d + u * 16 + 8 * h) = i32x4{(int)pack2<DT>(w[0], w[1]), (int)pack2<DT>(w[2], w[3]),
+                                                              (int)pack2<DT>(w[4], w[5]), (int)pack2<DT>(w[6], w[7])};
+      }
+    }
+    if (a.gb && (y == 0 || y == H - 1 || x0 == 0 || x0 + P - 1 == W - 1)) {
+      float* const gb = a.gb + (size_t)n * 4 * O * (H + W);
+#pragma unroll
+      for (int u = 0; u < 2; ++u) {
+        if (u >= P) break;
+        const int x = x0 + u;
+#pragma unroll
+        for (int o = 0; o < MAXO; ++o)
+#pragma unroll
+          for (int r = 0; r < 2; ++r)
+#pragma unroll
+            for (int b = 0; b < 2; ++b) {
+              if (o >= O) continue;
+              const float val = v[u][o * 4 + r * 2 + b];
+              if (y == 0 && r == 0) gb[gb_edge_off(0, O, H, W) + (size_t)(o * 2 + b) * W + x] = val;
+              if (y == H - 1 && r == 1) gb[gb_edge_off(1, O, H, W) + (size_t)(o * 2 + b) * W + x] = val;
+              if (x == 0 && b == 0) gb[gb_edge_off(2, O, H, W) + (size_t)(o * 2 + r) * H + y] = val;
+              if (x == W - 1 && b == 1) gb[gb_edge_off(3, O, H, W) + (size_t)(o * 2 + r) * H + y] = val;
+            }
+      }
+    }
   }
 }
 
@@ -540,15 +728,34 @@
   return 0;
 }
 
-static unsigned edge_split(int N) {
-  const int z = (512 + 2 * N - 1) / (2 * N);
-  return (unsigned)(z < 1 ? 1 : (z > 8 ? 8 : z));
-}
-
 template <typename K> static int edge_lds_attr(K kernel, const char* who) {
   const hipError_t e = hipFuncSetAttribute(reinterpret_cast<const void*>(kernel), hipFuncAttributeMaxDynamicSharedMemorySize, 160 * 1024);
   if (e != hipSuccess) { srk_set_error("%s: cannot reserve LDS: %s", who, hipGetErrorString(e)); return (int)e; }
   return 0;
+}
+
+static unsigned edge_split(int N, int maxlen, int cap) {
+  int z = (1024 + 4 * N - 1) / (4 * N);
+  z = z < 1 ? 1 : (z > cap ? cap : z);
+  const int zmin = (maxlen + 255) / 256;
+  if (z < zmin) z = zmin;
+  return (unsigned)(z > maxlen ? maxlen : z);
+}
+
+template <int DT, int O> static int edge_fwd_launch(const srk_hrtail_args* a, unsigned z, size_t lds, hipStream_t st) {
+  static const int rc = edge_lds_attr(&hrtail_edge_fwd_kernel<DT, O>, "srk_hrtail_edge_fwd");
+  if (rc) return rc;
+  hipLaunchKernelGGL((hrtail_edge_fwd_kernel<DT, O>), dim3((unsigned)a->N, 4, z), dim3(256), lds, st, *a);
+  SRK_LAUNCH_CHECK();
+  return 0;
+}
+template <int DT> static int edge_fwd_o(const srk_hrtail_args* a, unsigned z, size_t lds, hipStream_t st) {
+  switch (a->O) {
+    case 1: return edge_fwd_launch<DT, 1>(a, z, lds, st);
+    case 2: return edge_fwd_launch<DT, 2>(a, z, lds, st);
+    case 3: return edge_fwd_launch<DT, 3>(a, z, lds, st);
+    default: return edge_fwd_launch<DT, 4>(a, z, lds, st);
+  }
 }
 
 extern "C" int srk_hrtail_edge_fwd(const srk_hrtail_args* a, srk_stream_t stream) {
@@ -556,36 +763,30 @@
   if (int rc = check_act(a, "srk_hrtail_edge_fwd")) return rc;
   SRK_CHECK_ARG(a->x && a->out && a->wedge && a->bedge && a->wcor && a->bcor, "srk_hrtail_edge_fwd: null pointer");
   const int len = a->H > a->W ? a->H : a->W;
-  const size_t lds = ((size_t)(len + 4) * (a->Ci + 1) + (size_t)2 * a->O * a->Ci * 5) * 4;
+  const unsigned z = edge_split(a->N, len, 16);
+  const int per = (len + (int)z - 1) / (int)z, ws = (10 * a->O + 3) & ~3;
+  const size_t lds = ((((size_t)(per + 4) * (a->Ci + 1) + 3) & ~(size_t)3) + (size_t)a->Ci * ws + (size_t)10 * a->Ci +
+                      (size_t)10 * a->O * a->Ci + (size_t)2 * a->O * a->Ci) * 4;
   SRK_CHECK_ARG(lds <= 160 * 1024, "srk_hrtail_edge_fwd: edge of %d pixels x %d channels does not fit the LDS", len, a->Ci);
-  static const int rc0 = edge_lds_attr(&hrtail_edge_fwd_kernel<SRK_BF16>, "srk_hrtail_edge_fwd");
-  static const int rc1 = edge_lds_attr(&hrtail_edge_fwd_kernel<SRK_F16>, "srk_hrtail_edge_fwd");
-  if (rc0 || rc1) return rc0 ? rc0 : rc1;
   hipStream_t st = reinterpret_cast<hipStream_t>(stream);
-  for (int phase = 0; phase < 2; ++phase) {
-    if (a->dtype == SRK_BF16) hipLaunchKernelGGL(hrtail_edge_fwd_kernel<SRK_BF16>, dim3((unsigned)a->N, 2, edge_split(a->N)), dim3(256), lds, st, *a, phase);
-    else hipLaunchKernelGGL(hrtail_edge_fwd_kernel<SRK_F16>, dim3((unsigned)a->N, 2, edge_split(a->N)), dim3(256), lds, st, *a, phase);
-    SRK_LAUNCH_CHECK();
-  }
-  return 0;
+  return a->dtype == SRK_BF16 ? edge_fwd_o<SRK_BF16>(a, z, lds, st) : edge_fwd_o<SRK_F16>(a, z, lds, st);
 }
 
 extern "C" int srk_hrtail_edge_bwd_x(const srk_hrtail_args* a, srk_stream_t stream) {
   if (int rc = check_common(a, "srk_hrtail_edge_bwd_x")) return rc;
   if (int rc = check_act(a, "srk_hrtail_edge_bwd_x")) return rc;
-  SRK_CHECK_ARG(a->g && a->dx && a->wedge && a->wcor, "srk_hrtail_edge_bwd_x: null pointer");
+  SRK_CHECK_ARG((a->g || a->gb) && a->dx && a->wedge && a->wcor, "srk_hrtail_edge_bwd_x: null pointer");
   const int len = a->H > a->W ? a->H : a->W;
-  const size_t lds = ((size_t)2 * a->O * (len + 4) + (size_t)2 * a->O * a->Ci * 5) * 4;
+  const size_t lds = 4 * ((size_t)2 * a->O * (len + 4) + (size_t)2 * a->O * a->Ci * 5) * 4;
   SRK_CHECK_ARG(lds <= 160 * 1024, "srk_hrtail_edge_bwd_x: edge of %d pixels does not fit the LDS", len);
   static const int rc0 = edge_lds_attr(&hrtail_edge_bwd_x_kernel<SRK_BF16>, "srk_hrtail_edge_bwd_x");
   static const int rc1 = edge_lds_attr(&hrtail_edge_bwd_x_kernel<SRK_F16>, "srk_hrtail_edge_bwd_x");
   if (rc0 || rc1) return rc0 ? rc0 : rc1;
   hipStream_t st = reinterpret_cast<hipStream_t>(stream);
-  for (int phase = 0; phase < 2; ++phase) {
-    if (a->dtype == SRK_BF16) hipLaunchKernelGGL(hrtail_edge_bwd_x_kernel<SRK_BF16>, dim3((unsigned)a->N, 2, edge_split(a->N)), dim3(256), lds, st, *a, phase);
-    else hipLaunchKernelGGL(hrtail_edge_bwd_x_kernel<SRK_F16>, dim3((unsigned)a->N, 2, edge_split(a->N)), dim3(256), lds, st, *a, phase);
-    SRK_LAUNCH_CHECK();
-  }
+  const dim3 grid((unsigned)a->N, 5, edge_split(a->N, len, 8));
+  if (a->dtype == SRK_BF16) hipLaunchKernelGGL(hrtail_edge_bwd_x_kernel<SRK_BF16>, grid, dim3(256), lds, st, *a);
+  else hipLaunchKernelGGL(hrtail_edge_bwd_x_kernel<SRK_F16>, grid, dim3(256), lds, st, *a);
+  SRK_LAUNCH_CHECK();
   return 0;
 }
 
@@ -600,7 +801,7 @@
 extern "C" int srk_hrtail_edge_bwd_w(const srk_hrtail_args* a, srk_stream_t stream) {
   if (int rc = check_common(a, "srk_hrtail_edge_bwd_w")) return rc;
   if (int rc = check_act(a, "srk_hrtail_edge_bwd_w")) return rc;
-  SRK_CHECK_ARG(a->x && a->g && a->scratch && a->eedge && a->e0 && a->ecor && a->k0, "srk_hrtail_edge_bwd_w: null pointer");
+  SRK_CHECK_ARG(a->x && (a->g || a->gb) && a->scratch && a->eedge && a->e0 && a->ecor && a->k0, "srk_hrtail_edge_bwd_w: null pointer");
   const int ewc = ew_chunk_of(a->N);
   const int nchunks = (a->N + ewc - 1) / ewc;
   const unsigned nz = nchunks * 8 >= 512 ? 2 : (nchunks * 8 >= 256 ? 4 : 8);
@@ -629,3 +830,19 @@
   SRK_LAUNCH_CHECK();
   return 0;
 }
+
+extern "C" long long srk_hrtail_gb_floats(int N, int O, int H, int W) { return (long long)N * 4 * O * (H + W); }
+
+extern "C" int srk_hrtail_grad_layout(const srk_hrtail_args* a, srk_stream_t stream) {
+  if (int rc = check_common(a, "srk_hrtail_grad_layout")) return rc;
+  if (int rc = check_act(a, "srk_hrtail_grad_layout")) return rc;
+  SRK_CHECK_ARG(a->g && a->g12, "srk_hrtail_grad_layout: null pointer");
+  SRK_CHECK_ARG(((uintptr_t)a->g & 15) == 0 && ((uintptr_t)a->g12 & 15) == 0, "srk_hrtail_grad_layout: g / g12 not 16-byte aligned");
+  const long long items = (long long)a->N * a->H * (a->W % 2 == 0 ? a->W / 2 : a->W);
+  const unsigned grid = (unsigned)((items + 255) / 256 > 16384 ? 16384 : (items + 255) / 256);
+  hipStream_t st = reinterpret_cast<hipStream_t>(stream);
+  if (a->dtype == SRK_BF16) hipLaunchKernelGGL(hrtail_grad_layout_kernel<SRK_BF16>, dim3(grid), dim3(256), 0, st, *a);
+  else hipLaunchKernelGGL(hrtail_grad_layout_kernel<SRK_F16>, dim3(grid), dim3(256), 0, st, *a);
+  SRK_LAUNCH_CHECK();
+  return 0;
+}
diff --git a/sr-pytorch-lightning_amd/ops.py b/sr-pytorch-lightning_amd/ops.py
--- a/sr-pytorch-lightning_amd/ops.py
+++ b/sr-pytorch-lightning_amd/ops.py
@@ -465,7 +465,9 @@
         dev, f32 = x.device, torch.float32
         g = _f32c(g)
         st = _stream()
-        g12 = to_nhwc(g, x.dtype, ps_r=2)
+        g12 = torch.empty((n, h, w, 16), dtype=x.dtype, device=dev)
+        gb = torch.empty(int(L.load().srk_hrtail_gb_floats(n, o, h, w)), dtype=f32, device=dev)
+        L.call("srk_hrtail_grad_layout", HrTailFn._args(x, wu_, bu_, wt_, None, bufs, g=g.data_ptr(), g12=g12.data_ptr(), gb=gb.data_ptr()), st)
         need_x = ctx.needs_input_grad[0]
         need_w = any(ctx.needs_input_grad[1:5])
         gx = None
@@ -473,7 +475,7 @@
             pkd = pack_conv(bufs["weff"], None, x.dtype, dgrad=True, cache=False)
             gx = torch.empty_like(x)
             conv_raw(g12, pkd, N=n, H=h, W=w, Cin=g12.shape[3], Cout=ci, out=gx, use_bias=False)
-            L.call("srk_hrtail_edge_bwd_x", HrTailFn._args(x, wu_, bu_, wt_, None, bufs, g=g.data_ptr(), dx=gx.data_ptr(), dx_pitch=_pitch(gx)), st)
+            L.call("srk_hrtail_edge_bwd_x", HrTailFn._args(x, wu_, bu_, wt_, None, bufs, g=g.data_ptr(), gb=gb.data_ptr(), dx=gx.data_ptr(), dx_pitch=_pitch(gx)), st)
         gwu = gbu = gwt = gbt = None
         if need_w:
             r, r0 = wgrad_raw(x, g12, N=n, H=h, W=w, Cin=ci, Cout=g12.shape[3], k=5, w_shape=(4 * o, ci, 5, 5), want_bias=True)
@@ -481,7 +483,7 @@
                        ecor=torch.empty((4, o, ci), dtype=f32, device=dev), k0=torch.empty((4, o), dtype=f32, device=dev))
             scratch = torch.empty(int(L.load().srk_hrtail_scratch_floats(n, ci)), dtype=f32, device=dev)
             ptrs = {k: v.data_ptr() for k, v in red.items()}
-            L.call("srk_hrtail_edge_bwd_w", HrTailFn._args(x, wu_, bu_, wt_, None, bufs, g=g.data_ptr(), scratch=scratch.data_ptr(), **ptrs), st)
+            L.call("srk_hrtail_edge_bwd_w", HrTailFn._args(x, wu_, bu_, wt_, None, bufs, g=g.data_ptr(), gb=gb.data_ptr(), scratch=scratch.data_ptr(), **ptrs), st)
             pu, pbu, pt, pbt = ctx.wb
             gwu, gwt = (route(p, shape, dev, slice=p.dtype == f32, buffer=True).out for p, shape in ((pu, tuple(wu_.shape)), (pt, tuple(wt_.shape))))
             gbu = route(pbu, (4 * c,), dev, slice=pbu.dtype == f32, buffer=True).out if has_bu else None
```

Result: no change. 47910 LR patches/s (median of 6 runs) (+0.4%).
